# stella-cv/stella_vslam

Measured on AMD Instinct MI355X. Metric: frames/s ORB-extract+match @640x480,2k kpts, higher is better.
Workload: dtype u8

## Files before the change

include/svgpu.h:

```cpp
#ifndef SVGPU_H
#define SVGPU_H

#include <stddef.h>
#include <stdint.h>

#ifdef __cplusplus
extern "C" {
#endif

#define SVGPU_ABI_VERSION 1

typedef enum svgpu_status {
    SVGPU_OK = 0,
    SVGPU_ERR_INVALID = 1,
    SVGPU_ERR_HIP = 2,
    SVGPU_ERR_CAPACITY = 3,
    SVGPU_ERR_NOT_CONFIGURED = 4,
    SVGPU_ERR_NO_DEVICE = 5,
    SVGPU_ERR_NUMERIC = 6,
    SVGPU_STOPPED = 7
} svgpu_status;

typedef struct svgpu_ctx svgpu_ctx;

typedef struct svgpu_keypoint {
    float x, y, size, angle, response;
    int32_t octave, class_id;
} svgpu_keypoint;

int svgpu_abi_version(void);
int svgpu_device_count(void);
int svgpu_create(int device, svgpu_ctx** out);
int svgpu_create_with_priority(int device, int priority, svgpu_ctx** out);
void svgpu_destroy(svgpu_ctx* ctx);
const char* svgpu_last_error(const svgpu_ctx* ctx);
const char* svgpu_status_string(int status);
int svgpu_synchronize(svgpu_ctx* ctx);
void* svgpu_stream(svgpu_ctx* ctx);

const char* svgpu_profile_kernels(void);
int svgpu_profile_select(svgpu_ctx* ctx, const char* kernel_name);
int svgpu_profile_read(svgpu_ctx* ctx, double* total_ms, long long* launches);
int svgpu_profile_read_class(svgpu_ctx* ctx, const char* kernel_name, double* total_ms, long long* launches);
int svgpu_profile_mfma_ops(svgpu_ctx* ctx, unsigned long long* int8_ops);


int svgpu_orb_scale_tables(float scale_factor, int num_levels, float* scale_factors, float* inv_scale_factors,
                           float* level_sigma_sq, float* inv_level_sigma_sq);

int svgpu_orb_configure(svgpu_ctx* ctx, int width, int height, int max_batch, float scale_factor, int num_levels,
                        int ini_fast_thr, int min_fast_thr, unsigned min_area);

int svgpu_orb_stream_wait_stage(svgpu_ctx* ctx, int stage, void* stream);

int svgpu_orb_max_keypoints(const svgpu_ctx* ctx);
int svgpu_orb_level_size(const svgpu_ctx* ctx, int level, int* width, int* height);

int svgpu_orb_extract(svgpu_ctx* ctx, const uint8_t* img, int stride, const uint8_t* mask, int mask_stride,
                      svgpu_keypoint* kps, uint8_t* desc, int cap, int* n_out, int* level_counts);

int svgpu_orb_extract_batch_device(svgpu_ctx* ctx, const uint8_t* imgs_dev, int batch, size_t frame_stride,
                                   int row_stride, const uint8_t* mask_dev, size_t mask_frame_stride,
                                   int mask_row_stride, svgpu_keypoint* kps_dev, uint8_t* desc_dev, int cap,
                                   int32_t* counts_dev, void* stream);

int svgpu_orb_extract_batch_device_angles(svgpu_ctx* ctx, const uint8_t* imgs_dev, int batch, size_t frame_stride,
                                          int row_stride, const uint8_t* mask_dev, size_t mask_frame_stride,
                                          int mask_row_stride, svgpu_keypoint* kps_dev, uint8_t* desc_dev, int cap,
                                          int32_t* counts_dev, float* angles_dev, void* stream);

int svgpu_orb_pyramid_download(svgpu_ctx* ctx, int frame, int level, uint8_t* dst, int dst_stride);
int svgpu_orb_blurred_download(svgpu_ctx* ctx, int frame, int level, uint8_t* dst, int dst_stride);


int svgpu_hamming_distance(svgpu_ctx* ctx, const uint8_t* a, const uint8_t* b, int n, uint32_t* dist);

int svgpu_hamming_matrix(svgpu_ctx* ctx, const uint8_t* desc1, int n1, const uint8_t* desc2, int n2, uint16_t* out);

int svgpu_match_bruteforce(svgpu_ctx* ctx, const uint8_t* desc1, const float* angle1, int n1, const uint8_t* desc2,
                           const float* angle2, const uint8_t* valid2, int n2, float lowe_ratio,
                           int check_orientation, int32_t* matched_2_in_1, int* num_matches);

int svgpu_match_bruteforce_batch_device(svgpu_ctx* ctx, int pairs, const uint8_t* desc1_dev,
                                        const svgpu_keypoint* kps1_dev, const int32_t* n1_dev, int cap1,
                                        const uint8_t* desc2_dev, const svgpu_keypoint* kps2_dev,
                                        const int32_t* n2_dev, int cap2, int n_stride, const uint8_t* valid2_dev,
                                        float lowe_ratio, int check_orientation, int32_t* matched_dev,
                                        int32_t* num_dev, void* stream);

int svgpu_match_consecutive_batch_device(svgpu_ctx* ctx, int frames, const uint8_t* desc_dev, const svgpu_keypoint* kps_dev,
                                         const int32_t* n_dev, int cap, int n_stride, const uint8_t* valid_dev, float lowe_ratio,
                                         int check_orientation, int32_t* matched_dev, int32_t* num_dev, void* stream);

int svgpu_match_consecutive_batch_device_angles(svgpu_ctx* ctx, int frames, const uint8_t* desc_dev, const svgpu_keypoint* kps_dev,
                                                const float* angles_dev, const int32_t* n_dev, int cap, int n_stride, const uint8_t* valid_dev,
                                                float lowe_ratio, int check_orientation, int32_t* matched_dev, int32_t* num_dev, void* stream);

typedef enum svgpu_match_mode {
    SVGPU_MATCH_BEST_ONLY = 0,
    SVGPU_MATCH_RATIO_SAME_OCTAVE = 1,
    SVGPU_MATCH_RATIO = 2,
    SVGPU_MATCH_TRIANGULATION = 3,
    SVGPU_MATCH_AREA = 4
} svgpu_match_mode;

int svgpu_match_candidates(svgpu_ctx* ctx, const uint8_t* qdesc, int nq, const uint8_t* tdesc, const int32_t* t_octave,
                           int nt, const int32_t* cand_off, const int32_t* cand_idx, const uint8_t* cand_skip,
                           const uint8_t* q_valid, const uint8_t* occupied, const float* q_angle, const float* t_angle, int check_orientation,
                           const float* q_xright, const float* t_xright, const float* q_xr_tol, unsigned thr,
                           float lowe_ratio, int mode, int32_t* match_q, int* num_matches);

int svgpu_match_in_cells(svgpu_ctx* ctx, const uint8_t* qdesc, int nq, const float* q_xy, const float* q_margin,
                         const int32_t* q_min_level, const int32_t* q_max_level, const uint8_t* q_valid, const float* q_angle,
                         const float* q_xright, const float* q_xr_tol, const uint8_t* tdesc, const float* t_xy,
                         const int32_t* t_octave, int nt, const uint8_t* occupied, const float* t_angle, const float* t_xright,
                         float min_x, float max_x, float min_y, float max_y, int grid_cols, int grid_rows,
                         int check_orientation, unsigned thr, float lowe_ratio, int mode, int32_t* match_q, int* num_matches);

typedef enum svgpu_camera_model {
    SVGPU_CAM_PERSPECTIVE = 0,
    SVGPU_CAM_FISHEYE = 1,
    SVGPU_CAM_EQUIRECTANGULAR = 2,
    SVGPU_CAM_RADIAL_DIVISION = 3
} svgpu_camera_model;

typedef struct svgpu_camera {
    int32_t model;
    int32_t pad_;
    double cols, rows;
    double fx, fy, cx, cy;
    double dist[5];
    double focal_x_baseline;
    float min_x, max_x, min_y, max_y;
} svgpu_camera;

int svgpu_camera_image_bounds(svgpu_ctx* ctx, svgpu_camera* cam);

int svgpu_frame_observation(svgpu_ctx* ctx, const svgpu_camera* cam, const svgpu_keypoint* kps, int n, int grid_cols,
                            int grid_rows, svgpu_keypoint* undist_kps, double* bearings, int32_t* cell_off, int32_t* cell_items);

int svgpu_keypoints_to_bearings(svgpu_ctx* ctx, const svgpu_camera* cam, const svgpu_keypoint* undist_kps, int n, double* bearings);

int svgpu_reproject_landmarks(svgpu_ctx* ctx, const svgpu_camera* cam, const double* rot_cw, const double* trans_cw,
                              const double* trans_wc, int n, const double* pos_w, const double* mean_normal,
                              const float* min_valid_dist, const float* max_valid_dist, const uint8_t* skip, float ray_cos_thr,
                              int num_levels, float log_scale_factor, uint8_t* visible, double* reproj, float* x_right,
                              int32_t* pred_scale_level);

int svgpu_match_frame_and_landmarks(svgpu_ctx* ctx, const svgpu_camera* cam, const double* rot_cw, const double* trans_cw,
                                    const double* trans_wc, int n, const double* pos_w, const double* mean_normal,
                                    const float* min_valid_dist, const float* max_valid_dist, const uint8_t* skip,
                                    const uint8_t* lm_desc, float ray_cos_thr, int num_levels, const float* scale_factors,
                                    float log_scale_factor, float margin, const uint8_t* tdesc, const float* t_xy,
                                    const int32_t* t_octave, int nt, const uint8_t* occupied, const float* t_xright,
                                    int grid_cols, int grid_rows, unsigned thr, float lowe_ratio, int32_t* match_lm,
                                    int* num_matches, uint8_t* visible, double* reproj, float* x_right,
                                    int32_t* pred_scale_level);

typedef struct svgpu_frame svgpu_frame;
int svgpu_frame_create(svgpu_ctx* ctx, svgpu_frame** out);
void svgpu_frame_destroy(svgpu_frame* frame);
int svgpu_frame_size(const svgpu_frame* frame);
int svgpu_frame_adopt_extraction(svgpu_ctx* ctx, svgpu_frame* frame, const svgpu_camera* cam, int grid_cols, int grid_rows,
                                 svgpu_keypoint* undist_kps, double* bearings);
int svgpu_frame_upload(svgpu_ctx* ctx, svgpu_frame* frame, const svgpu_camera* cam, const svgpu_keypoint* undist_kps, const uint8_t* desc,
                       const float* x_right, int n, int grid_cols, int grid_rows);
int svgpu_frame_set_stereo(svgpu_ctx* ctx, svgpu_frame* frame, const float* x_right);
int svgpu_frame_bind(svgpu_ctx* ctx, const svgpu_frame* frame);
int svgpu_match_set_query_blocks(svgpu_ctx* ctx, const uint8_t* q_blocks);

typedef struct svgpu_map svgpu_map;
enum {
    SVGPU_LM_PRESENT = 1,
    SVGPU_LM_HAS_OBSERVATION = 2,
    SVGPU_LM_HAS_DESCRIPTOR = 4
};
typedef struct svgpu_landmark_record {
    double pos_w[3];
    double mean_normal[3];
    float min_valid_dist, max_valid_dist;
    uint8_t descriptor[32];
    uint32_t flags;
    uint32_t reserved;
} svgpu_landmark_record;
int svgpu_map_create(svgpu_ctx* ctx, svgpu_map** out);
void svgpu_map_destroy(svgpu_map* map);
int svgpu_map_capacity(const svgpu_map* map);
int svgpu_map_upsert(svgpu_ctx* ctx, svgpu_map* map, int n, const uint32_t* ids, const svgpu_landmark_record* records);
int svgpu_map_erase(svgpu_ctx* ctx, svgpu_map* map, int n, const uint32_t* ids);
int svgpu_map_download(svgpu_ctx* ctx, const svgpu_map* map, int n, const uint32_t* ids, svgpu_landmark_record* records);

typedef struct svgpu_tracker svgpu_tracker;
typedef struct svgpu_track_config {
    int num_levels;
    float scale_factors[16];
    float inv_level_sigma_sq[16];
    float log_scale_factor;
    int grid_cols, grid_rows;
    int is_monocular;
    float true_baseline;
    int po_num_trials_robust, po_num_trials, po_num_each_iter, po_reset_stop_flag_each_round;
} svgpu_track_config;
typedef struct svgpu_track_result {
    int n_keypoints;
    int num_matches;
    int num_valid;
    int lm_iterations;
    int num_observations;
    int num_candidates;
    int replay_sweeps;
    int reserved;
    double pose_cw[12];
} svgpu_track_result;
int svgpu_tracker_create(svgpu_ctx* ctx, svgpu_map* map, const svgpu_camera* cam, const svgpu_track_config* cfg, svgpu_tracker** out);
void svgpu_tracker_destroy(svgpu_tracker* tracker);
int svgpu_track_motion(svgpu_tracker* tracker, svgpu_frame* cur, const uint8_t* img, int stride, const svgpu_frame* last,
                       const int32_t* last_lm_ids, const double* pose_guess_cw, const double* pose_last_cw, float margin,
                       int check_orientation, svgpu_keypoint* kps, uint8_t* desc, svgpu_keypoint* undist_kps, double* bearings, int cap,
                       int32_t* match_last, uint8_t* outlier, svgpu_track_result* result);
int svgpu_tracker_observation(const svgpu_tracker* tracker, const svgpu_keypoint** kps, const uint8_t** desc, const svgpu_keypoint** undist_kps,
                              const double** bearings);
int svgpu_track_motion_stereo(svgpu_tracker* tracker, svgpu_ctx* ctx_right, svgpu_frame* cur, const uint8_t* img_left, int stride_left,
                              const uint8_t* img_right, int stride_right, const svgpu_frame* last, const int32_t* last_lm_ids,
                              const double* pose_guess_cw, const double* pose_last_cw, float margin, int check_orientation, int cap,
                              int32_t* match_last, uint8_t* outlier, svgpu_track_result* result);
int svgpu_tracker_observation_stereo(const svgpu_tracker* tracker, const float** stereo_x_right, const float** depths);
int svgpu_track_motion_rgbd(svgpu_tracker* tracker, svgpu_frame* cur, const uint8_t* img, int stride, const float* depth, int depth_stride,
                            const svgpu_frame* last, const int32_t* last_lm_ids, const double* pose_guess_cw, const double* pose_last_cw,
                            float margin, int check_orientation, int cap, int32_t* match_last, uint8_t* outlier, svgpu_track_result* result);
int svgpu_track_local_map(svgpu_tracker* tracker, const svgpu_frame* cur, const int32_t* cur_lm_ids, int n_local, const int32_t* local_ids,
                          const double* pose_cw, float margin, float lowe_ratio, float ray_cos_thr, int32_t* match_local, uint8_t* visible,
                          uint8_t* outlier, svgpu_track_result* result);
int svgpu_track_local_map_observability(svgpu_tracker* tracker, int n_local, double* reproj, float* x_right, int32_t* pred_scale_level);
int svgpu_tracker_counters(const svgpu_tracker* tracker, long long* launches, long long* host_syncs);
const unsigned long long* svgpu_tracker_debug_stamps(const svgpu_tracker* tracker);

typedef struct svgpu_ingest svgpu_ingest;
typedef enum svgpu_color_order { SVGPU_COLOR_GRAY = 0, SVGPU_COLOR_RGB = 1, SVGPU_COLOR_BGR = 2 } svgpu_color_order;
typedef enum svgpu_depth_type { SVGPU_DEPTH_NONE = 0, SVGPU_DEPTH_U16 = 1, SVGPU_DEPTH_F32 = 2 } svgpu_depth_type;
int svgpu_ingest_create(svgpu_ctx* ctx, int width, int height, int channels, int color_order, const float* map_x, const float* map_y,
                        int map_stride, svgpu_ingest** out);
void svgpu_ingest_destroy(svgpu_ingest* ingest);
int svgpu_ingest_gray(svgpu_ctx* ctx, const svgpu_ingest* ingest, const uint8_t* src, int src_stride, uint8_t* dst, int dst_stride);
int svgpu_ingest_gray_batch_device(svgpu_ctx* ctx, const svgpu_ingest* ingest, const uint8_t* src_dev, int batch, size_t src_frame_stride,
                                   int src_row_stride, uint8_t* dst_dev, size_t dst_frame_stride, int dst_row_stride, void* stream);
int svgpu_ingest_depth(svgpu_ctx* ctx, const void* src, int src_type, int src_stride, int width, int height, double depthmap_factor, float* dst,
                       int dst_stride);
int svgpu_ingest_depth_device(svgpu_ctx* ctx, const void* src_dev, int src_type, int src_stride, int width, int height, double depthmap_factor,
                              float* dst_dev, int dst_stride, void* stream);
int svgpu_tracker_set_ingest(svgpu_tracker* tracker, const svgpu_ingest* ingest_left, const svgpu_ingest* ingest_right, int depth_type,
                             double depthmap_factor);


int svgpu_reproject_to_bearing(const svgpu_camera* cam, const double* rot_cw, const double* trans_cw, const double* pos_w, double* bearing,
                               int* valid);

int svgpu_match_current_and_last_frames(svgpu_ctx* ctx, const svgpu_camera* cam, const double* rot_cw, const double* trans_cw, const double* rot_lw,
                                        const double* trans_lw, int is_monocular, float true_baseline, int n_last, const double* pos_w,
                                        const uint8_t* valid, const uint8_t* lm_desc, const int32_t* octave_last, const float* angle_last,
                                        const uint8_t* lm_has_observation, int num_levels, const float* scale_factors, float margin,
                                        const uint8_t* tdesc, const float* t_xy, const int32_t* t_octave, const float* t_angle, int nt,
                                        const uint8_t* occupied, const float* t_xright, int grid_cols, int grid_rows, int check_orientation,
                                        int32_t* match_last, int* num_matches);

int svgpu_match_frame_and_keyframe_projection(svgpu_ctx* ctx, const svgpu_camera* cam, const double* rot_cw, const double* trans_cw, int n_kf,
                                              const double* pos_w, const uint8_t* valid, const float* min_valid_dist, const float* max_valid_dist,
                                              const uint8_t* lm_desc, const float* angle_kf, int num_levels, const float* scale_factors,
                                              float log_scale_factor, float margin, unsigned hamm_dist_thr, const uint8_t* tdesc, const float* t_xy,
                                              const int32_t* t_octave, const float* t_angle, int nt, const uint8_t* occupied, int grid_cols,
                                              int grid_rows, int check_orientation, int32_t* match_kf, int* num_matches);

int svgpu_match_by_sim3_transform(svgpu_ctx* ctx, const svgpu_camera* cam, const double* sim3_cw, int n, const double* pos_w, const uint8_t* valid,
                                  const float* min_valid_dist, const float* max_valid_dist, const double* mean_normal, const uint8_t* lm_desc,
                                  int num_levels, const float* scale_factors, float log_scale_factor, float margin, const uint8_t* tdesc,
                                  const float* t_xy, const int32_t* t_octave, int nt, const uint8_t* occupied, int grid_cols, int grid_rows,
                                  int32_t* match_lm, int* num_matches);

int svgpu_match_keyframes_mutually(svgpu_ctx* ctx, const svgpu_camera* cam1, const svgpu_camera* cam2, const double* rot_1w, const double* trans_1w,
                                   const double* rot_2w, const double* trans_2w, float s_12, const double* rot_12, const double* trans_12,
                                   int n1, const double* pos_w1, const uint8_t* valid1, const float* min_valid1, const float* max_valid1,
                                   const uint8_t* lm_desc1, const uint8_t* desc1, const float* xy1, const int32_t* octave1,
                                   int n2, const double* pos_w2, const uint8_t* valid2, const float* min_valid2, const float* max_valid2,
                                   const uint8_t* lm_desc2, const uint8_t* desc2, const float* xy2, const int32_t* octave2,
                                   int num_levels, const float* scale_factors, float log_scale_factor, float margin, int grid_cols, int grid_rows,
                                   int32_t* matched_2_in_1, int32_t* matched_1_in_2, int32_t* mutual_2_in_1, int* num_matches);

int svgpu_fuse_detect_duplication(svgpu_ctx* ctx, const svgpu_camera* cam, const double* rot_cw, const double* trans_cw, int n, const double* pos_w,
                                  const uint8_t* valid, const float* min_valid_dist, const float* max_valid_dist, const double* mean_normal,
                                  const uint8_t* lm_desc, int num_levels, const float* scale_factors, const float* inv_level_sigma_sq,
                                  float log_scale_factor, float margin, int do_reprojection_matching, const uint8_t* tdesc, const float* t_xy,
                                  const int32_t* t_octave, const float* t_xright, int nt, int grid_cols, int grid_rows, int32_t* best_idx,
                                  int* num_fused);

int svgpu_match_for_triangulation(svgpu_ctx* ctx, const uint8_t* desc1, const float* angle1, const int32_t* octave1, const double* bearings1,
                                  const uint8_t* has_lm1, const float* xright1, int n1, const uint8_t* desc2, const float* angle2,
                                  const double* bearings2, const uint8_t* has_lm2, const float* xright2, int n2, const int32_t* node1,
                                  const int32_t* node2, const double* E_12, const double* epipole_in_2, int valid_epipole, const float* scale_factors,
                                  int num_levels, float residual_rad_thr, float lowe_ratio, int check_orientation, int32_t* matched_2_in_1,
                                  int* num_matches);

#define SVGPU_TRI_ACCEPTED 0
#define SVGPU_TRI_NO_MODE 1
#define SVGPU_TRI_DEPTH 2
#define SVGPU_TRI_REPROJECTION 3
#define SVGPU_TRI_SCALE 4
#define SVGPU_TRI_SKIPPED 255
int svgpu_triangulate_two_views(svgpu_ctx* ctx, const svgpu_camera* cam1, const double* pose_1w, double true_baseline_1, const float* xy1, const int32_t* octave1,
                                const double* bearings1, const float* xright1, const float* depth1, int n1, const svgpu_camera* cam2, const double* pose_2w,
                                double true_baseline_2, const float* xy2, const int32_t* octave2, const double* bearings2, const float* xright2,
                                const float* depth2, int n2, const float* scale_factors, const float* level_sigma_sq, int num_levels, float scale_factor_1,
                                float scale_factor_2, float rays_parallax_deg_thr, const int32_t* idx1, const int32_t* idx2, int num_matches, double* pos_w,
                                uint8_t* status, int* num_accepted);

typedef struct svgpu_triangulate_view {
    const svgpu_camera* cam;
    const double* pose_cw;
    double true_baseline;
    const float* xy;
    const int32_t* octave;
    const double* bearings;
    const float* xright;
    const float* depth;
    int32_t n;
    float scale_factor;
} svgpu_triangulate_view;
int svgpu_triangulate_two_views_batch(svgpu_ctx* ctx, const svgpu_triangulate_view* view1, const svgpu_triangulate_view* neighbours, int num_neighbours,
                                      const int32_t* match_off, const float* scale_factors, const float* level_sigma_sq, int num_levels,
                                      float rays_parallax_deg_thr, const int32_t* idx1, const int32_t* idx2, double* pos_w, uint8_t* status, int* num_accepted);

int svgpu_pnp_compute_pose(svgpu_ctx* ctx, int num_sets, const int32_t* set_off, const double* bearings, const double* pos_w,
                           int gauss_newton_num_iter, double* pose_cw, double* reproj_error);

int svgpu_pnp_ransac_batch(svgpu_ctx* ctx, int num_problems, const int32_t* match_off, const double* bearings, const double* pos_w,
                           const int32_t* octaves, const float* scale_factors, int num_levels, int min_num_inliers, int num_iter,
                           const uint32_t* samples, int recompute, int gauss_newton_num_iter, uint8_t* valid, double* pose_cw,
                           uint8_t* is_inlier, int32_t* best_iter, double* hyp_pose, int32_t* hyp_num_inliers, double* hyp_cost);

int svgpu_pnp_ransac(svgpu_ctx* ctx, const double* bearings, const double* pos_w, const int32_t* octaves, int num_matches,
                     const float* scale_factors, int num_levels, int min_num_inliers, int num_iter, const uint32_t* samples, int recompute,
                     int gauss_newton_num_iter, uint8_t* valid, double* pose_cw, uint8_t* is_inlier, int32_t* best_iter, double* hyp_pose,
                     int32_t* hyp_num_inliers, double* hyp_cost);

int svgpu_bow_match(svgpu_ctx* ctx, const uint8_t* desc1, const float* angle1, const uint8_t* valid1, const int32_t* node1, int n1,
                    const uint8_t* desc2, const float* angle2, const uint8_t* valid2, const int32_t* node2, int n2, const uint8_t* occupied2,
                    float lowe_ratio, int check_orientation, int32_t* match_1to2, int* num_matches);

int svgpu_landmarks_compute_descriptor(svgpu_ctx* ctx, int n, const int32_t* obs_off, const uint8_t* obs_desc, int32_t* best_obs,
                                       uint8_t* descriptor);

int svgpu_landmarks_update_geometry(svgpu_ctx* ctx, int n, const int32_t* obs_off, const double* obs_trans_wc, const double* pos_w,
                                    const double* ref_trans_wc, const float* ref_scale_factor, float inv_scale_factor_last,
                                    double* mean_normal, float* max_valid_dist, float* min_valid_dist);

typedef struct svgpu_vocabulary svgpu_vocabulary;
int svgpu_bow_vocabulary_upload(svgpu_ctx* ctx, int n_nodes, const int32_t* child_off, const int32_t* children, const uint8_t* node_desc,
                                const float* node_weight, const int32_t* word_id, svgpu_vocabulary** out);
void svgpu_bow_vocabulary_free(svgpu_vocabulary* vocab);
int svgpu_bow_transform(svgpu_ctx* ctx, const svgpu_vocabulary* vocab, const uint8_t* desc, int n, int node_level, int32_t* word_id,
                        float* weight, int32_t* node_id);
int svgpu_fbow_transform(svgpu_ctx* ctx, const svgpu_vocabulary* vocab, const uint8_t* desc, int n, int store_level, int k,
                         int32_t* word_id, float* weight, uint32_t* node_code);

#define SVGPU_BOW_SCORE_FBOW_L2 0
#define SVGPU_BOW_SCORE_DBOW2_L1 1
typedef struct svgpu_bowdb svgpu_bowdb;
int svgpu_bowdb_create(svgpu_ctx* ctx, int score_form, svgpu_bowdb** db);
void svgpu_bowdb_destroy(svgpu_bowdb* db);
int svgpu_bowdb_clear(svgpu_ctx* ctx, svgpu_bowdb* db);
int svgpu_bowdb_add(svgpu_ctx* ctx, svgpu_bowdb* db, int n_words, const uint32_t* words, const double* weights, int32_t* slot);
int svgpu_bowdb_erase(svgpu_ctx* ctx, svgpu_bowdb* db, int32_t slot);
int svgpu_bowdb_size(svgpu_bowdb* db, int* live_keyframes, long long* live_entries);
int svgpu_bowdb_diagnostics(svgpu_bowdb* db, long long* num_slots, long long* pool_capacity, long long* pool_used, long long* num_growths,
                            long long* num_compactions);
int svgpu_bowdb_query_stage_capacity(void);
int svgpu_bowdb_acquire(svgpu_ctx* ctx, svgpu_bowdb* db, int n_words, const uint32_t* words, const double* weights, float min_score, float ratio,
                        int n_reject, const int32_t* reject_slots, int cap, int32_t* out_slots, uint32_t* out_common, float* out_score, int32_t* n_out,
                        uint32_t* max_common);
int svgpu_bowdb_acquire_batch(svgpu_ctx* ctx, svgpu_bowdb* db, int num_queries, const int32_t* q_off, const uint32_t* words, const double* weights,
                              const float* min_score, float ratio, int n_reject, const int32_t* reject_slots, int cap, int32_t* out_slots,
                              uint32_t* out_common, float* out_score, int32_t* n_out, uint32_t* max_common);
int svgpu_bowdb_score(svgpu_ctx* ctx, svgpu_bowdb* db, int n_words, const uint32_t* words, const double* weights, int n, const int32_t* slots,
                      float* out_score);

int svgpu_stereo_match(svgpu_ctx* ctx_left, svgpu_ctx* ctx_right, const svgpu_keypoint* kps_left, const uint8_t* desc_left,
                       int n_left, const svgpu_keypoint* kps_right, const uint8_t* desc_right, int n_right,
                       float focal_x_baseline, float true_baseline, float* stereo_x_right, float* depths);

int svgpu_stereo_match_batch_device(svgpu_ctx* ctx_left, svgpu_ctx* ctx_right, int pairs, const svgpu_keypoint* kps_left_dev, const uint8_t* desc_left_dev,
                                    const int32_t* n_left_dev, const svgpu_keypoint* kps_right_dev, const uint8_t* desc_right_dev,
                                    const int32_t* n_right_dev, int cap, int n_stride, float focal_x_baseline, float true_baseline,
                                    float* stereo_x_right_dev, float* depths_dev, void* stream);

typedef struct svgpu_ba_problem {
    int32_t num_poses;
    int32_t num_points;
    int32_t num_obs;
    const double* pose_cw;
    const uint8_t* pose_fixed;
    const double* points;
    const uint8_t* point_fixed;
    const int32_t* obs_pose;
    const int32_t* obs_point;
    const float* obs_uvr;
    const float* obs_inv_sigma_sq;
    const float* obs_huber_delta;
    const double* intrinsics;
    int32_t num_first_iter;
    int32_t num_second_iter;
    double gain_threshold;
} svgpu_ba_problem;

typedef struct svgpu_ba_stats {
    double chi2_initial, chi2_final;
    int32_t iters_stage1, iters_stage2, stage2_entered, num_gated;
    int32_t lm_trials, cholesky_failures;
    double lambda_final;
    int32_t stopped_by_terminate_action;
    int32_t pcg_iterations;
} svgpu_ba_stats;

typedef enum svgpu_ba_solver {
    SVGPU_BA_SOLVER_AUTO = 0,
    SVGPU_BA_SOLVER_CHOLESKY = 1,
    SVGPU_BA_SOLVER_PCG = 2,
    SVGPU_BA_SOLVER_DENSE = 3,
    SVGPU_BA_SOLVER_PCG_MULTI = 4,
    SVGPU_BA_SOLVER_CHOLESKY_MFMA = 7,
    SVGPU_BA_SOLVER_ENVELOPE = 6
} svgpu_ba_solver;
int svgpu_ba_set_solver(svgpu_ctx* ctx, int solver, double pcg_tolerance, int pcg_max_iterations);

int svgpu_ba_last_envelope_plan(svgpu_ctx* ctx, int* info);

int svgpu_selftest_segmented_solve(int nP, int NB, const int* blk_ab, const double* Sblk, const double* g, int cuts, int world,
                                   double* x, int* info);

int svgpu_selftest_segmented_solve_rank(int nP, int NB, const int* blk_ab, const double* Sblk, const double* g, int cuts, int rank, int world,
                                        int (*allreduce)(void* user, double* buf, size_t count, void* stream), void* allreduce_user, double* x,
                                        int* info);

int svgpu_selftest_scan_sort(svgpu_ctx* ctx, int n, const int32_t* values, int32_t* scan_out, const uint32_t* keys, int bits, int32_t* sorted_idx);

int svgpu_local_ba(svgpu_ctx* ctx, const svgpu_ba_problem* problem, volatile uint8_t* stop, double* pose_out,
                   double* points_out, uint8_t* outlier_out, svgpu_ba_stats* stats);

int svgpu_pose_optimize(svgpu_ctx* ctx, const double* pose_cw, int n, const double* pos_w, const float* uvr,
                        const float* inv_sigma_sq, const float* huber_delta, const double* intrinsics ,
                        int num_trials_robust, int num_trials, int num_each_iter, int reset_stop_flag_each_round,
                        double* pose_out, uint8_t* outlier_flags, int* num_valid, int* lm_iterations);

int svgpu_pose_optimize_device(svgpu_ctx* ctx, const double* pose_cw, int n, const double* pos_w_dev, const float* uvr_dev,
                               const float* inv_sigma_sq_dev, const float* huber_delta_dev, const double* intrinsics, int num_trials_robust,
                               int num_trials, int num_each_iter, int reset_stop_flag_each_round, double* pose_out,
                               uint8_t* outlier_flags, int* num_valid, int* lm_iterations);

int svgpu_global_ba(svgpu_ctx* ctx, const svgpu_ba_problem* problem, volatile uint8_t* stop, double* pose_out,
                    double* points_out, svgpu_ba_stats* stats);

typedef int (*svgpu_allreduce_fn)(void* user, double* dev_buf, size_t count, void* stream);
int svgpu_local_ba_sharded(svgpu_ctx* ctx, const svgpu_ba_problem* shard, int rank, int world,
                           svgpu_allreduce_fn allreduce, void* allreduce_user, volatile uint8_t* stop, double* pose_out,
                           double* points_out, uint8_t* outlier_out, svgpu_ba_stats* stats);
int svgpu_global_ba_sharded(svgpu_ctx* ctx, const svgpu_ba_problem* shard, int rank, int world,
                            svgpu_allreduce_fn allreduce, void* allreduce_user, volatile uint8_t* stop, double* pose_out,
                            double* points_out, svgpu_ba_stats* stats);

int svgpu_ba_partition_keyframe_segments(const svgpu_ba_problem* problem, int world, int32_t* landmark_rank, int32_t* info);
int svgpu_ba_last_exchange(svgpu_ctx* ctx, int64_t* info);

int svgpu_comm_unique_id(uint8_t* id128);
int svgpu_comm_init(svgpu_ctx* ctx, int rank, int world, const uint8_t* id128);
void svgpu_comm_destroy(svgpu_ctx* ctx);
int svgpu_comm_allreduce_f64(svgpu_ctx* ctx, double* dev_buf, size_t count, void* stream);

#ifdef __cplusplus
}
#endif
#endif
```

stella_vslam_amd/csrc/orb_kernels.hip:

```cpp
#include "svgpu_internal.h"
#include "sv_trig.h"
#include <cstdlib>
#include <utility>

#pragma clang fp contract(off)

namespace {

__device__ __constant__ float c_pattern_f[1024] = {
#include "orb_pattern_i8.inc"
};

__device__ __forceinline__ int find_level(const OrbLevel* __restrict__ L, int num_levels, int idx, int OrbLevel::*first,
                                          int* local) {
    int lv = 0;
    for (int l = 0; l < num_levels; ++l) {
        const int f = L[l].*first;
        if (idx >= f) lv = l;
    }
    *local = idx - L[lv].*first;
    return lv;
}

__device__ __forceinline__ int reflect101(int p, int len) {
    if (len == 1) return 0;
    while (p < 0 || p >= len) p = p < 0 ? -p : 2 * (len - 1) - p;
    return p;
}

typedef unsigned short u16x2 __attribute__((ext_vector_type(2)));
__device__ __forceinline__ u16x2 as_u16x2(uint32_t v) { return __builtin_bit_cast(u16x2, v); }

__device__ __forceinline__ void xcd_frame_map(int per_frame, int batch, int& item, int& frame) {
    const int lin = blockIdx.x + blockIdx.y * gridDim.x;
    const int full = (batch / 8) * 8, lim = full * per_frame;
    if (lin < lim) {
        const int xcd = lin & 7, idx = lin >> 3;
        frame = (idx / per_frame) * 8 + xcd;
        item = idx % per_frame;
    }
    else {
        const int r = lin - lim;
        frame = full + r / per_frame;
        item = r % per_frame;
    }
}

__device__ __forceinline__ void sv_glds16(unsigned long long base, uint32_t voff, uint32_t lds_dst) {
    uint32_t keep;
    asm volatile("s_mov_b32 %0, m0\n\ts_mov_b32 m0, %3\n\ts_nop 2\n\tglobal_load_lds_dwordx4 %1, %2\n\ts_mov_b32 m0, %0"
                 : "=&s"(keep)
                 : "v"(voff), "s"(base), "s"(lds_dst)
                 : "memory");
}

__global__ __launch_bounds__(256) void k_resize(const uint8_t* __restrict__ src, size_t src_frame_stride, int src_pitch,
                                                int sw, uint8_t* __restrict__ dst, size_t dst_frame_stride, int dst_pitch,
                                                int dw, int dh, const short* __restrict__ xofs,
                                                const short2* __restrict__ xa, const short2* __restrict__ yofs,
                                                const short2* __restrict__ yb) {
    const int dy = blockIdx.y * 4 + threadIdx.y;
    const int dx0 = (blockIdx.x * 64 + threadIdx.x) * 4;
    if (dy >= dh || dx0 >= dw) return;
    const uint8_t* S = src + (size_t)blockIdx.z * src_frame_stride;
    const short2 yo = yofs[dy];
    const short2 bb = yb[dy];
    const uint8_t* S0 = S + (size_t)yo.x * src_pitch;
    const uint8_t* S1 = S + (size_t)yo.y * src_pitch;
    uint32_t packed = 0;
#pragma unroll
    for (int i = 0; i < 4; ++i) {
        const int dx = dx0 + i;
        if (dx < dw) {
            const int sx = xofs[dx];
            const short2 a = xa[dx];
            const int sx1 = min(sx + 1, sw - 1);
            const int r0 = S0[sx] * a.x + S0[sx1] * a.y;
            const int r1 = S1[sx] * a.x + S1[sx1] * a.y;
            const int v = ((((int)bb.x * (r0 >> 4)) >> 16) + (((int)bb.y * (r1 >> 4)) >> 16) + 2) >> 2;
            packed |= (uint32_t)(v & 255) << (8 * i);
        }
    }
    uint8_t* D = dst + (size_t)blockIdx.z * dst_frame_stride + (size_t)dy * dst_pitch + dx0;
    *reinterpret_cast<uint32_t*>(D) = packed;
}

#define PYR_THREADS 1024
#define PYR_MAXW 4096
__global__ __launch_bounds__(PYR_THREADS) void k_pyramid(const OrbLevel* __restrict__ L, int num_levels, const int2* __restrict__ band_rows,
                                                         const uint8_t* __restrict__ img0, size_t img0_frame_stride, int img0_pitch,
                                                         uint8_t* __restrict__ pyr, size_t pyr_frame_bytes,
                                                         const short* __restrict__ xofs, const short2* __restrict__ xa,
                                                         const short2* __restrict__ yofs, const short2* __restrict__ yb) {
    __shared__ short s_xo[PYR_MAXW];
    __shared__ short2 s_xa[PYR_MAXW];
    const int band = blockIdx.x, b = blockIdx.y, tid = threadIdx.x;
    uint8_t* P = pyr + (size_t)b * pyr_frame_bytes;
    for (int l = 1; l < num_levels; ++l) {
        const OrbLevel lev = L[l], prev = L[l - 1];
        const uint8_t* S = l == 1 ? img0 + (size_t)b * img0_frame_stride : P + prev.pyr_off;
        const int sp = l == 1 ? img0_pitch : prev.pitch;
        uint8_t* Dst = P + lev.pyr_off;
        const int2 rr = band_rows[band * num_levels + l];
        const int groups = (lev.w + 3) >> 2, ntask = (rr.y - rr.x) * groups;
        const bool in_lds = lev.w <= PYR_MAXW;
        if (in_lds)
            for (int x = tid; x < lev.w; x += PYR_THREADS) {
                s_xo[x] = xofs[lev.xtab_off + x];
                s_xa[x] = xa[lev.xtab_off + x];
            }
        __syncthreads();
        for (int t = tid; t < ntask; t += PYR_THREADS) {
            const int row = t / groups, g = t - row * groups;
            const int dy = rr.x + row, dx0 = g * 4;
            const short2 yo = yofs[lev.ytab_off + dy], bb = yb[lev.ytab_off + dy];
            const uint8_t* S0 = S + (size_t)yo.x * sp;
            const uint8_t* S1 = S + (size_t)yo.y * sp;
            int sx[4], sx1[4];
            short2 a[4];
#pragma unroll
            for (int i = 0; i < 4; ++i) {
                const int dx = min(dx0 + i, lev.w - 1);
                sx[i] = in_lds ? s_xo[dx] : xofs[lev.xtab_off + dx];
                a[i] = in_lds ? s_xa[dx] : xa[lev.xtab_off + dx];
                sx1[i] = min(sx[i] + 1, prev.w - 1);
            }
            int p00[4], p01[4], p10[4], p11[4];
#pragma unroll
            for (int i = 0; i < 4; ++i) {
                p00[i] = S0[sx[i]];
                p01[i] = S0[sx1[i]];
                p10[i] = S1[sx[i]];
                p11[i] = S1[sx1[i]];
            }
            uint32_t packed = 0;
#pragma unroll
            for (int i = 0; i < 4; ++i) {
                const int r0 = p00[i] * a[i].x + p01[i] * a[i].y;
                const int r1 = p10[i] * a[i].x + p11[i] * a[i].y;
                const int v = ((((int)bb.x * (r0 >> 4)) >> 16) + (((int)bb.y * (r1 >> 4)) >> 16) + 2) >> 2;
                packed |= (uint32_t)(v & 255) << (8 * i);
            }
            *reinterpret_cast<uint32_t*>(Dst + (size_t)dy * lev.pitch + dx0) = packed;
        }
        __syncthreads();
    }
}

__device__ __forceinline__ uint32_t mul_hi_u24(uint32_t a, uint32_t b) {
    uint32_t d;
    asm("v_mul_hi_u32_u24 %0, %1, %2" : "=v"(d) : "v"(a), "v"(b));
    return d;
}

__global__ __launch_bounds__(PYR_THREADS) void k_pyramid_lds(const OrbLevel* __restrict__ L, int num_levels, const int2* __restrict__ band_rows,
                                                             int bands, const uint8_t* __restrict__ img0, size_t img0_frame_stride,
                                                             int img0_pitch, uint8_t* __restrict__ pyr, size_t pyr_frame_bytes,
                                                             const uint32_t* __restrict__ xg, const short4* __restrict__ yrow) {
    extern __shared__ __attribute__((aligned(16))) uint8_t s_mem[];
    __shared__ int s_img[SV_MAX_LEVELS], s_yt[SV_MAX_LEVELS + 1];
    const int band = blockIdx.x, b = blockIdx.y, tid = threadIdx.x;
    const int2* BR = band_rows + (size_t)band * num_levels;
    if (tid == 0) {
        int size_a = 0, size_b = 0;
        for (int l = 0; l < num_levels; ++l) {
            const int bytes = (BR[l].y - BR[l].x) * ((L[l].w + 3) & ~3);
            if (l & 1) size_a = max(size_a, bytes);
            else size_b = max(size_b, bytes);
        }
        size_a = (size_a + 15) & ~15;
        size_b = (size_b + 15) & ~15;
        for (int l = 0; l < num_levels; ++l) s_img[l] = (l & 1) ? 0 : size_a;
        int off = size_a + size_b;
        s_yt[0] = off;
        for (int l = 1; l < num_levels; ++l) {
            s_yt[l] = off;
            off += (BR[l].y - BR[l].x) * 8;
        }
        s_yt[num_levels] = off;
    }
    __syncthreads();
    const uint8_t* I0 = img0 + (size_t)b * img0_frame_stride;
    {
        const int w0 = L[0].w, p0 = (w0 + 3) & ~3, lo0 = BR[0].x, n0 = BR[0].y - lo0;
        uint8_t* D0 = s_mem + s_img[0];
        if (((((size_t)I0) | (size_t)img0_pitch) & 15) == 0 && (p0 & 15) == 0) {
            const int cpr = p0 >> 4, total = n0 * cpr;
            const float inv = 1.0f / (float)cpr;
            for (int i = tid; i < total; i += PYR_THREADS) {
                const int r = (int)(((float)i + 0.5f) * inv), c = i - __mul24(r, cpr);
                reinterpret_cast<uint4*>(D0)[i] = *reinterpret_cast<const uint4*>(I0 + (__umul24(lo0 + r, img0_pitch) + 16 * c));
            }
        }
        else if (((((size_t)I0) | (size_t)img0_pitch) & 3) == 0) {
            const int wpr = p0 >> 2, total = n0 * wpr;
            const float inv = 1.0f / (float)wpr;
            for (int i = tid; i < total; i += PYR_THREADS) {
                const int r = (int)(((float)i + 0.5f) * inv), c = i - __mul24(r, wpr);
                reinterpret_cast<uint32_t*>(D0)[i] = *reinterpret_cast<const uint32_t*>(I0 + (__umul24(lo0 + r, img0_pitch) + 4 * c));
            }
        }
        else {
            const int total = n0 * p0;
            for (int i = tid; i < total; i += PYR_THREADS) {
                const int r = i / p0, c = i - r * p0;
                D0[i] = c < w0 ? I0[(size_t)(lo0 + r) * img0_pitch + c] : (uint8_t)0;
            }
        }
        const int rows = (s_yt[num_levels] - s_yt[0]) >> 3;
        for (int i = tid; i < rows; i += PYR_THREADS) {
            int l = 1;
            while (l + 1 < num_levels && s_yt[0] + 8 * i >= s_yt[l + 1]) ++l;
            const int r = i - ((s_yt[l] - s_yt[0]) >> 3);
            reinterpret_cast<short4*>(s_mem + s_yt[0])[i] = yrow[L[l].ytab_off + BR[l].x + r];
        }
    }
    __syncthreads();
    uint8_t* P = pyr + (size_t)b * pyr_frame_bytes;
    for (int l = 1; l < num_levels; ++l) {
        const OrbLevel lev = L[l];
        const int spw = ((L[l - 1].w + 3) & ~3) >> 2, dpw = ((lev.w + 3) & ~3) >> 2;
        const int src_lo = BR[l - 1].x, lo = BR[l].x, hi = BR[l].y;
        const int own_lo = (int)((long long)band * lev.h / bands), own_hi = (int)((long long)(band + 1) * lev.h / bands);
        const uint32_t* S = reinterpret_cast<const uint32_t*>(s_mem + s_img[l - 1]);
        uint32_t* Dl = reinterpret_cast<uint32_t*>(s_mem + s_img[l]);
        const short4* yt = reinterpret_cast<const short4*>(s_mem + s_yt[l]);
        uint8_t* Dg = P + lev.pyr_off;
        const int groups = (lev.w + 3) >> 2, nrows = hi - lo;
        const int chunks = max(min(PYR_THREADS / groups, nrows), 1), rc = (nrows + chunks - 1) / chunks;
        const int c = (int)(((float)tid + 0.5f) * (1.0f / (float)groups)), g = tid - __mul24(c, groups);
        const int r0 = __mul24(c, rc), r1 = min(r0 + rc, nrows);
        if (r0 < r1) {
            const uint4 e = reinterpret_cast<const uint4*>(xg)[2 * (lev.xg_off + g)];
            const uint2 e2 = reinterpret_cast<const uint2*>(xg)[4 * (lev.xg_off + g) + 2];
            const int i0 = e.x & 0xffff, i2 = e.x >> 16;
            const uint32_t coef[4] = {e.z, e.w, e2.x, e2.y};
            uint32_t sel[4];
#pragma unroll
            for (int i = 0; i < 4; ++i) sel[i] = 0x0c010c00u + ((e.y >> (8 * i)) & 255u) * 0x00010001u;
            const uint32_t* S0 = S + (i0 - __mul24(src_lo, spw));
            const int d2 = i2 - i0;
            auto hrow = [&](int sy, uint32_t (&h)[4]) {
                const uint32_t* R = S0 + __mul24(sy, spw);
                const uint32_t a0 = R[0], a1 = R[1], c0 = R[d2], c1 = R[d2 + 1];
                h[0] = __builtin_amdgcn_udot2(as_u16x2(__builtin_amdgcn_perm(a1, a0, sel[0])), as_u16x2(coef[0]), 0u, false) & ~15u;
                h[1] = __builtin_amdgcn_udot2(as_u16x2(__builtin_amdgcn_perm(a1, a0, sel[1])), as_u16x2(coef[1]), 0u, false) & ~15u;
                h[2] = __builtin_amdgcn_udot2(as_u16x2(__builtin_amdgcn_perm(c1, c0, sel[2])), as_u16x2(coef[2]), 0u, false) & ~15u;
                h[3] = __builtin_amdgcn_udot2(as_u16x2(__builtin_amdgcn_perm(c1, c0, sel[3])), as_u16x2(coef[3]), 0u, false) & ~15u;
            };
            uint32_t* dl = Dl + (__mul24(r0, dpw) + g);
            uint32_t goff = __umul24(lo + r0, lev.pitch) + 4 * g;
            const uint32_t own_n = (uint32_t)(own_hi - own_lo);
            uint32_t dyo = (uint32_t)(lo + r0 - own_lo);
            int prev = -1;
            auto step = [&](int row, uint32_t (&top)[4], uint32_t (&bot)[4]) {
                const short4 ye = yt[row];
                if (ye.x != prev) hrow(ye.x, top);
                hrow(ye.y, bot);
                prev = ye.y;
                const uint32_t b0 = (uint32_t)ye.z << 12, b1 = (uint32_t)ye.w << 12;
                uint32_t v[4];
#pragma unroll
                for (int i = 0; i < 4; ++i) v[i] = (mul_hi_u24(b0, top[i]) + mul_hi_u24(b1, bot[i]) + 2u) >> 2;
                const uint32_t packed = (v[0] & 255u) | ((v[1] & 255u) << 8) | ((v[2] & 255u) << 16) | (v[3] << 24);
                *dl = packed;
                if (dyo < own_n) *reinterpret_cast<uint32_t*>(Dg + goff) = packed;
                dl += dpw;
                goff += (uint32_t)lev.pitch;
                ++dyo;
            };
            uint32_t hX[4], hY[4] = {0, 0, 0, 0};
            int row = r0;
            for (; row + 1 < r1; row += 2) {
                step(row, hY, hX);
                step(row + 1, hX, hY);
            }
            if (row < r1) step(row, hY, hX);
        }
        __syncthreads();
    }
}

#define BLUR_EDGE_ROWS 8
struct BlurRow {
    uint32_t w0, w1, w2;
};
enum { BLUR_INTERIOR = 0, BLUR_EDGE = 1, BLUR_GATHER = 2, BLUR_LDS = 3 };
struct BlurEdge {
    bool left, hi_p1;
    uint32_t sel1, sel2;
};
__device__ __forceinline__ uint32_t blur_selector(int xbase, int lo_base, int w) {
    uint32_t s = 0;
#pragma unroll
    for (int k = 0; k < 4; ++k) {
        const int x = xbase + k, sx = x < w ? x : 2 * (w - 1) - x;
        s |= (uint32_t)min(max(sx - lo_base, 0), 7) << (8 * k);
    }
    return s;
}
__device__ __forceinline__ BlurEdge blur_edge_ctx(int x0, int w) {
    BlurEdge e;
    e.left = x0 == 0;
    e.hi_p1 = x0 + 4 < w;
    e.sel1 = blur_selector(x0, x0 - 4, w);
    e.sel2 = blur_selector(x0 + 4, e.hi_p1 ? x0 : x0 - 4, w);
    return e;
}
template <int MODE>
__device__ __forceinline__ BlurRow blur_load(const uint8_t* __restrict__ row, int x0, int w, const BlurEdge& e) {
    BlurRow r;
    if (MODE == BLUR_INTERIOR) {
        const uint32_t* p = reinterpret_cast<const uint32_t*>(row + x0 - 4);
        r.w0 = p[0];
        r.w1 = p[1];
        r.w2 = p[2];
    }
    else if (MODE == BLUR_EDGE) {
        if (e.left) {
            const uint32_t* p = reinterpret_cast<const uint32_t*>(row);
            r.w1 = p[0];
            r.w2 = p[1];
            r.w0 = __builtin_amdgcn_perm(r.w2, r.w1, 0x01020304u);
        }
        else {
            const uint32_t* p = reinterpret_cast<const uint32_t*>(row + x0 - 4);
            const uint32_t pm1 = p[0], p0 = p[1], p1 = e.hi_p1 ? p[2] : 0u;
            r.w0 = pm1;
            r.w1 = __builtin_amdgcn_perm(p0, pm1, e.sel1);
            r.w2 = e.hi_p1 ? __builtin_amdgcn_perm(p1, p0, e.sel2) : __builtin_amdgcn_perm(p0, pm1, e.sel2);
        }
    }
    else {
        uint32_t b[12];
#pragma unroll
        for (int k = 0; k < 12; ++k) b[k] = row[reflect101(x0 - 4 + k, w)];
        r.w0 = b[0] | (b[1] << 8) | (b[2] << 16) | (b[3] << 24);
        r.w1 = b[4] | (b[5] << 8) | (b[6] << 16) | (b[7] << 24);
        r.w2 = b[8] | (b[9] << 8) | (b[10] << 16) | (b[11] << 24);
    }
    return r;
}
__device__ __forceinline__ void blur_hpair(const BlurRow& a, const BlurRow& b, u16x2 (&hp)[4]) {
    u16x2 q[10];
#define SV_PK(WA, WB, K) as_u16x2(__builtin_amdgcn_perm(WB, WA, 0x0c000c00u | ((4u + K) << 16) | K))
    q[0] = SV_PK(a.w0, b.w0, 1u);
    q[1] = SV_PK(a.w0, b.w0, 2u);
    q[2] = SV_PK(a.w0, b.w0, 3u);
    q[3] = SV_PK(a.w1, b.w1, 0u);
    q[4] = SV_PK(a.w1, b.w1, 1u);
    q[5] = SV_PK(a.w1, b.w1, 2u);
    q[6] = SV_PK(a.w1, b.w1, 3u);
    q[7] = SV_PK(a.w2, b.w2, 0u);
    q[8] = SV_PK(a.w2, b.w2, 1u);
    q[9] = SV_PK(a.w2, b.w2, 2u);
#undef SV_PK
    const u16x2 t18 = {18, 18}, t34 = {34, 34}, t48 = {48, 48}, t56 = {56, 56};
#pragma unroll
    for (int j = 0; j < 4; ++j) hp[j] = t18 * (q[j] + q[j + 6]) + t34 * (q[j + 1] + q[j + 5]) + t48 * (q[j + 2] + q[j + 4]) + t56 * q[j + 3];
}
__device__ __forceinline__ uint32_t blur_dot(u16x2 h, uint32_t taps, uint32_t acc) { return __builtin_amdgcn_udot2(h, as_u16x2(taps), acc, false); }
__device__ __forceinline__ uint32_t blur_pack(const uint32_t (&acc)[4]) {
    const uint32_t lo = __builtin_amdgcn_perm(acc[1], acc[0], 0x0c0c0602u), hi = __builtin_amdgcn_perm(acc[3], acc[2], 0x06020c0cu);
    return lo | hi;
}

template <int MODE, class LoadPair>
__device__ __forceinline__ void blur_walk(LoadPair load_pair, uint8_t* __restrict__ Dp, int dpitch, int ys, int ye) {
    constexpr int AHEAD = MODE == BLUR_LDS ? 0 : 2;
    u16x2 A[4], B[4], C[4], D[4], E[4];
    BlurRow n0 = {}, n1 = {};
    {
        BlurRow r[8];
#pragma unroll
        for (int k = 0; k < 4; ++k) load_pair(ys - 4 + 2 * k, r[2 * k], r[2 * k + 1]);
        if (AHEAD) load_pair(ys + 4, n0, n1);
        if (MODE == BLUR_INTERIOR) {
#pragma unroll
            for (int k = 0; k < 8; ++k) asm volatile("" : "+v"(r[k].w0), "+v"(r[k].w1), "+v"(r[k].w2));
            asm volatile("" : "+v"(n0.w0), "+v"(n0.w1), "+v"(n0.w2), "+v"(n1.w0), "+v"(n1.w1), "+v"(n1.w2));
        }
        blur_hpair(r[0], r[1], A);
        blur_hpair(r[2], r[3], B);
        blur_hpair(r[4], r[5], C);
        blur_hpair(r[6], r[7], D);
    }
    for (int y = ys; y < ye; y += 2) {
        const BlurRow c0 = n0, c1 = n1;
        load_pair(y + 4 + AHEAD, n0, n1);
        if (AHEAD) blur_hpair(c0, c1, E);
        else blur_hpair(n0, n1, E);
        uint32_t acc[4];
#pragma unroll
        for (int j = 0; j < 4; ++j)
            acc[j] = blur_dot(D[j], 34u | (18u << 16), blur_dot(C[j], 56u | (48u << 16), blur_dot(B[j], 34u | (48u << 16), blur_dot(A[j], 18u << 16, 32768u))));
        *reinterpret_cast<uint32_t*>(Dp + __umul24(y, dpitch)) = blur_pack(acc);
        if (y + 1 < ye) {
#pragma unroll
            for (int j = 0; j < 4; ++j)
                acc[j] = blur_dot(E[j], 18u, blur_dot(D[j], 48u | (34u << 16), blur_dot(C[j], 48u | (56u << 16), blur_dot(B[j], 18u | (34u << 16), 32768u))));
            *reinterpret_cast<uint32_t*>(Dp + __umul24(y + 1, dpitch)) = blur_pack(acc);
        }
#pragma unroll
        for (int j = 0; j < 4; ++j) {
            A[j] = B[j];
            B[j] = C[j];
            C[j] = D[j];
            D[j] = E[j];
        }
    }
}
template <int MODE>
__device__ __forceinline__ void blur_strip(const uint8_t* __restrict__ src, int spitch, int w, int h, uint8_t* __restrict__ dst,
                                           int dpitch, int x0, int ys, int ye) {
    auto row_ptr = [&](int y) { return src + __umul24(reflect101(y, h), spitch); };
    BlurEdge edge = {};
    if (MODE == BLUR_EDGE) edge = blur_edge_ctx(x0, w);
    blur_walk<MODE>([&](int y, BlurRow& a, BlurRow& b) {
        a = blur_load<MODE>(row_ptr(y), x0, w, edge);
        b = blur_load<MODE>(row_ptr(y + 1), x0, w, edge);
    }, dst + x0, dpitch, ys, ye);
}

__device__ __forceinline__ void blur_locate(const OrbLevel* __restrict__ L, int num_levels, const uint8_t* __restrict__ img0,
                                            size_t img0_frame_stride, int img0_pitch, const uint8_t* __restrict__ pyr,
                                            size_t pyr_frame_bytes, uint8_t* __restrict__ blur, size_t blur_frame_bytes, OrbLevel& lev,
                                            int& tile, const uint8_t*& src, int& spitch, uint8_t*& dst,
                                            int OrbLevel::*first = &OrbLevel::btile_first) {
    int b, item;
    xcd_frame_map(gridDim.x, gridDim.y, item, b);
    const int lv = find_level(L, num_levels, item, first, &tile);
    lev = L[lv];
    if (lv == 0) {
        src = img0 + (size_t)b * img0_frame_stride;
        spitch = img0_pitch;
    }
    else {
        src = pyr + (size_t)b * pyr_frame_bytes + lev.pyr_off;
        spitch = lev.pitch;
    }
    dst = blur + (size_t)b * blur_frame_bytes + lev.blur_off;
}
__device__ __forceinline__ bool blur_streamable(const uint8_t* src, int spitch, int w) {
    return ((((size_t)src) | (size_t)spitch) & 3) == 0 && w >= 16;
}
template <int ROWS>
__global__ __launch_bounds__(256) void k_blur(const OrbLevel* __restrict__ L, int num_levels, const uint8_t* __restrict__ img0,
                                              size_t img0_frame_stride, int img0_pitch, const uint8_t* __restrict__ pyr,
                                              size_t pyr_frame_bytes, uint8_t* __restrict__ blur, size_t blur_frame_bytes) {
    OrbLevel lev;
    int tile, spitch;
    const uint8_t* src;
    uint8_t* dst;
    blur_locate(L, num_levels, img0, img0_frame_stride, img0_pitch, pyr, pyr_frame_bytes, blur, blur_frame_bytes, lev, tile, src, spitch, dst);
    if (!blur_streamable(src, spitch, lev.w)) return;
    const int main_tiles = lev.btiles_x * lev.btiles_y;
    if (tile < main_tiles) {
        const int tx = tile % lev.btiles_x, ty = tile / lev.btiles_x;
        const int rem_groups = tx == lev.btiles_x - 1 ? (min(lev.w - 6, (tx + 1) * BLUR_TW) - tx * BLUR_TW + 3) / 4 : 64;
        int g = 64;
        while (g > 1 && (g >> 1) >= rem_groups) g >>= 1;
        if (g <= 32 && rem_groups > 0) {
            const int spw = 64 / g, lane = threadIdx.x & 63;
            if (ty * spw >= lev.btiles_y) return;
            const int strip = (ty * 4 + (int)(threadIdx.x >> 6)) * spw + lane / g;
            const int x0 = tx * BLUR_TW + (lane % g) * 4, ys = strip * ROWS;
            if (x0 >= lev.w || ys >= lev.h) return;
            if (x0 >= 4 && x0 + 6 < lev.w) blur_strip<BLUR_INTERIOR>(src, spitch, lev.w, lev.h, dst, lev.pitch, x0, ys, min(ys + ROWS, lev.h));
            return;
        }
        const int x0 = tx * BLUR_TW + (threadIdx.x & 63) * 4;
        const int ys = __builtin_amdgcn_readfirstlane(ty * (4 * ROWS) + (int)(threadIdx.x >> 6) * ROWS);
        if (x0 >= lev.w || ys >= lev.h) return;
        if (x0 >= 4 && x0 + 6 < lev.w) blur_strip<BLUR_INTERIOR>(src, spitch, lev.w, lev.h, dst, lev.pitch, x0, ys, min(ys + ROWS, lev.h));
    }
    else {
        const int which = threadIdx.x & 3, strip = (tile - main_tiles) * 64 + (threadIdx.x >> 2);
        const int ys = strip * BLUR_EDGE_ROWS;
        const int last = ((lev.w - 1) >> 2) << 2;
        int x0;
        if (which == 0) x0 = 0;
        else if (which == 1) x0 = last;
        else if (which == 2) x0 = last - 4;
        else return;
        if (ys >= lev.h || x0 < 0 || (which != 0 && (x0 == 0 || x0 + 6 < lev.w))) return;
        blur_strip<BLUR_EDGE>(src, spitch, lev.w, lev.h, dst, lev.pitch, x0, ys, min(ys + BLUR_EDGE_ROWS, lev.h));
    }
}
#define BLUR_LP (16 + BLUR_SEG + 16)
#define BLUR_LDS_ROWS (BLUR_ROWS + 8)
static_assert(BLUR_SEG % 16 == 0 && BLUR_BAND_THREADS % 64 == 0 && BLUR_SEG / 4 <= BLUR_BAND_THREADS && BLUR_ROWS % 2 == 0, "blur band geometry");
static_assert(BLUR_LDS_ROWS * BLUR_LP <= 64 * 1024, "blur band exceeds the static LDS limit");
template <>
__global__ __launch_bounds__(BLUR_BAND_THREADS) void k_blur<BLUR_ROWS>(const OrbLevel* __restrict__ L, int num_levels, const uint8_t* __restrict__ img0,
                                                                       size_t img0_frame_stride, int img0_pitch, const uint8_t* __restrict__ pyr,
                                                                       size_t pyr_frame_bytes, uint8_t* __restrict__ blur, size_t blur_frame_bytes) {
    __shared__ __attribute__((aligned(16))) uint8_t s_rows[BLUR_LDS_ROWS * BLUR_LP];
    OrbLevel lev;
    int item, spitch;
    const uint8_t* src;
    uint8_t* dst;
    blur_locate(L, num_levels, img0, img0_frame_stride, img0_pitch, pyr, pyr_frame_bytes, blur, blur_frame_bytes, lev, item, src, spitch, dst,
                &OrbLevel::bband_first);
    if (!blur_streamable(src, spitch, lev.w)) return;
    const int tid = threadIdx.x, w = lev.w, h = lev.h;
    const int seg = item % lev.bband_segs, xs = seg * BLUR_SEG, sw = min(BLUR_SEG, w - xs);
    const int y0 = (item / lev.bband_segs) * BLUR_ROWS, rows = min(BLUR_ROWS, h - y0);
    const int groups = (sw + 3) >> 2, xend = xs + 4 * groups + 4;
    {
        constexpr int CPR = BLUR_LP / 16;
        const int total = (rows + 6) * CPR;
        const unsigned long long base = (unsigned long long)(uintptr_t)src;
        const uint32_t lds0 = __builtin_amdgcn_readfirstlane((uint32_t)(uintptr_t)(const __attribute__((address_space(3))) uint8_t*)s_rows) + BLUR_LP;
        for (int q0 = __builtin_amdgcn_readfirstlane(tid & ~63); q0 < total; q0 += BLUR_BAND_THREADS) {
            const int q = q0 + (tid & 63), k = q / CPR, x = xs - 16 + 16 * (q - k * CPR);
            if (q < total && x >= 0 && x < min(w, xend)) {
                const uint32_t off = __umul24(reflect101(y0 - 3 + k, h), spitch) + (uint32_t)x;
                if (x + 16 <= w) sv_glds16(base, off, lds0 + 16u * (uint32_t)q0);
                else
#pragma clang loop vectorize(disable)
                    for (int d = 0; x + 4 * d < w; ++d)
                        *reinterpret_cast<uint32_t*>(s_rows + BLUR_LP + 16 * q + 4 * d) = *reinterpret_cast<const uint32_t*>(src + off + 4 * d);
            }
        }
        asm volatile("s_waitcnt vmcnt(0)" ::: "memory");
    }
    __syncthreads();
    for (int i = tid; i < (rows + 6) * 8; i += BLUR_BAND_THREADS) {
        uint8_t* row = s_rows + ((i >> 3) + 1) * BLUR_LP + 16 - xs;
        const int j = i & 7;
        if (j == 0 && xs == 0) {
            const uint32_t* p = reinterpret_cast<const uint32_t*>(row);
            reinterpret_cast<uint32_t*>(row)[-1] = __builtin_amdgcn_perm(p[1], p[0], 0x01020304u);
        }
        const int x = w - 1 + j;
        if (j > 0 && x < xend) row[x] = row[2 * (w - 1) - x];
    }
    __syncthreads();
    const int chunks = max(min(BLUR_BAND_THREADS / groups, rows >> 1), 1), rc = ((rows + chunks - 1) / chunks + 1) & ~1;
    const int c = (int)(((float)tid + 0.5f) * (1.0f / (float)groups)), g = tid - __mul24(c, groups);
    const int r0 = __mul24(c, rc), r1 = min(r0 + rc, rows);
    if (r0 >= r1) return;
    const uint32_t* S = reinterpret_cast<const uint32_t*>(s_rows + 12 + 4 * g);
    blur_walk<BLUR_LDS>([&](int y, BlurRow& a, BlurRow& b) {
        const uint32_t* p = S + __mul24(y + 4, BLUR_LP / 4);
        a = BlurRow{p[0], p[1], p[2]};
        b = BlurRow{p[BLUR_LP / 4], p[BLUR_LP / 4 + 1], p[BLUR_LP / 4 + 2]};
    }, dst + __umul24(y0, lev.pitch) + xs + 4 * g, lev.pitch, r0, r1);
}
template <int ROWS>
__global__ __launch_bounds__(256) void k_blur_gather(const OrbLevel* __restrict__ L, int num_levels, const uint8_t* __restrict__ img0,
                                                     size_t img0_frame_stride, int img0_pitch, const uint8_t* __restrict__ pyr,
                                                     size_t pyr_frame_bytes, uint8_t* __restrict__ blur, size_t blur_frame_bytes) {
    OrbLevel lev;
    int tile, spitch;
    const uint8_t* src;
    uint8_t* dst;
    blur_locate(L, num_levels, img0, img0_frame_stride, img0_pitch, pyr, pyr_frame_bytes, blur, blur_frame_bytes, lev, tile, src, spitch, dst);
    if (blur_streamable(src, spitch, lev.w) || tile >= lev.btiles_x * lev.btiles_y) return;
    const int x0 = (tile % lev.btiles_x) * BLUR_TW + (threadIdx.x & 63) * 4;
    const int ys = (tile / lev.btiles_x) * (4 * ROWS) + (threadIdx.x >> 6) * ROWS;
    if (x0 >= lev.w || ys >= lev.h) return;
    blur_strip<BLUR_GATHER>(src, spitch, lev.w, lev.h, dst, lev.pitch, x0, ys, min(ys + ROWS, lev.h));
}

typedef short s16x2 __attribute__((ext_vector_type(2)));
__device__ __forceinline__ int arc_score16(int v, const int (&p)[16]) {
    s16x2 e[16];
#pragma unroll
    for (int k = 0; k < 16; ++k) e[k] = __builtin_bit_cast(s16x2, __mul24(p[k], -65535) + (int)0xFFFF0000);
    s16x2 m2[8], m4[8];
#pragma unroll
    for (int j = 0; j < 8; ++j) m2[j] = __builtin_elementwise_min(e[2 * j + 1], e[(2 * j + 2) & 15]);
#pragma unroll
    for (int j = 0; j < 8; ++j) m4[j] = __builtin_elementwise_min(m2[j], m2[(j + 1) & 7]);
    s16x2 best = s16x2{(short)-32768, (short)-32768};
#pragma unroll
    for (int j = 0; j < 8; ++j) {
        const s16x2 m8 = __builtin_elementwise_min(m4[j], m4[(j + 2) & 7]);
        best = __builtin_elementwise_max(best, __builtin_elementwise_min(m8, __builtin_elementwise_max(e[2 * j], e[(2 * j + 9) & 15])));
    }
    return max(max((int)best.x - v, v + 1 + (int)best.y), 0);
}

#define FAST_KT 12
#define FP 80
__global__ __launch_bounds__(256) void k_fast(const OrbLevel* __restrict__ L, int num_levels, const FastCell* __restrict__ cells, int num_cells, int cpw,
                                              const uint8_t* __restrict__ img0, size_t img0_frame_stride, int img0_pitch,
                                              const uint8_t* __restrict__ pyr, size_t pyr_frame_bytes,
                                              const unsigned short* __restrict__ gtab, unsigned long long* __restrict__ keys,
                                              int total_grid, int ini_thr, int min_thr, const uint8_t* __restrict__ mask,
                                              size_t mask_frame_stride, int mask_pitch, int mask_w, int mask_h) {
    __shared__ __attribute__((aligned(16))) uint8_t s_raw[SV_ROI_MAX * FP + 16];
    __shared__ __attribute__((aligned(16))) uint8_t s_a[SV_ROI_MAX * FP];
    __shared__ unsigned short s_q[SV_CELL * SV_CELL];
    __shared__ unsigned long long s_key[FAST_KT * FAST_KT];
    __shared__ unsigned short s_gx[SV_ROI_MAX], s_gy[SV_ROI_MAX];
    __shared__ int s_count;
    int b, grp;
    xcd_frame_map(gridDim.x, gridDim.y, grp, b);
    const int tid = threadIdx.x, lane = tid & 63;
    const int wv = __builtin_amdgcn_readfirstlane(tid >> 6);
    const uint8_t* M = mask ? mask + (size_t)b * mask_frame_stride : nullptr;
    const uint8_t* const I0 = img0 + (size_t)b * img0_frame_stride;
    const uint8_t* const PY = pyr + (size_t)b * pyr_frame_bytes;
    unsigned long long* const KF = keys + (size_t)b * total_grid;
    uint8_t* const s_img = s_raw + 3;
    unsigned short* const my_q = s_q + wv * (SV_CELL * SV_CELL / 4);
    const int qrow = lane >> 4, qk = lane & 15;
    const int x0 = 3 + 4 * qk;
    const int ly0 = 3 + 4 * (4 * qrow + wv);
    const int e0 = (ly0 << 7) | x0;
    const uint32_t* const qbase = reinterpret_cast<const uint32_t*>(s_raw + ly0 * FP + 4 * qk);

    auto load_ring = [&](const uint8_t* c, int (&p)[16]) {
        p[0] = c[3 * FP];
        p[1] = c[3 * FP + 1];
        p[2] = c[2 * FP + 2];
        p[3] = c[FP + 3];
        p[4] = c[3];
        p[5] = c[-FP + 3];
        p[6] = c[-2 * FP + 2];
        p[7] = c[-3 * FP + 1];
        p[8] = c[-3 * FP];
        p[9] = c[-3 * FP - 1];
        p[10] = c[-2 * FP - 2];
        p[11] = c[-FP - 3];
        p[12] = c[-3];
        p[13] = c[FP - 3];
        p[14] = c[2 * FP - 2];
        p[15] = c[3 * FP - 1];
    };

    const int c_first = grp * cpw, c_last = min(c_first + cpw, num_cells);
    for (int ci = c_first; ci < c_last; ++ci) {
    const FastCell cell = cells[ci];
    const OrbLevel lev = L[cell.lv];
    auto masked = [&](int y, int x) -> bool {
        int my = (int)((float)y * lev.scale), mx = (int)((float)x * lev.scale);
        my = min(my, mask_h - 1);
        mx = min(mx, mask_w - 1);
        return M[(size_t)my * mask_pitch + mx] == 0;
    };
    if (M) {
        const int y0 = cell.min_y, y1 = cell.min_y + cell.h, xa = cell.min_x, xb = cell.min_x + cell.w;
        if (masked(y0, xa) || masked(y1, xa) || masked(y0, xb) || masked(y1, xb)) continue;
    }
    const uint8_t* src;
    int spitch;
    if (cell.lv == 0) {
        src = I0;
        spitch = img0_pitch;
    }
    else {
        src = PY + lev.pyr_off;
        spitch = lev.pitch;
    }
    const int w = cell.w, h = cell.h;
    if (ci != c_first) __syncthreads();
    const uint8_t* rsrc = src + (size_t)cell.min_y * spitch + (cell.min_x - 3);
    {
        const unsigned long long rbase = (unsigned long long)(uintptr_t)rsrc;
        const uint32_t lds_raw = __builtin_amdgcn_readfirstlane((uint32_t)(uintptr_t)(const __attribute__((address_space(3))) uint8_t*)s_raw) + (uint32_t)wv * 1024u;
#pragma unroll
        for (int it = 0; it < 2; ++it) {
            const int q = tid + 256 * it, r = q / 5, c = q - 5 * r;
            if (it == 0 || wv < 2) {
                if (q < SV_ROI_MAX * (FP / 16) && r < h && 16 * c < w + 3) sv_glds16(rbase, (uint32_t)(__umul24(r, spitch) + 16 * c), lds_raw + 4096u * it);
            }
            if (q < SV_ROI_MAX * (FP / 16)) reinterpret_cast<uint4*>(s_a)[q] = make_uint4(0, 0, 0, 0);
        }
    }
    if (tid == 0) {
        s_count = 0;
    }
    if (tid < FAST_KT * FAST_KT) s_key[tid] = 0ull;
    if (tid < w) s_gx[tid] = gtab[lev.gtab_x_off + cell.min_x + tid - SV_PATCH_RADIUS];
    else if (tid >= 128 && tid - 128 < h) s_gy[tid - 128] = gtab[lev.gtab_y_off + cell.min_y + (tid - 128) - SV_PATCH_RADIUS];
    uint32_t band80 = 0;
#pragma unroll
    for (int j = 0; j < 4; ++j) band80 |= (x0 + j < w - 3) ? (0x80u << (8 * j)) : 0u;
    asm volatile("s_waitcnt vmcnt(0)" ::: "memory");
    __syncthreads();

    unsigned long long* K = KF + lev.grid_first;
    const int gx0 = s_gx[3], gy0 = s_gy[3];
    for (int pass = 0; pass < 2; ++pass) {
    const int t = pass == 0 ? ini_thr : min_thr, tq = t;
    int wq = 0;
#if defined(FAST_ABLATE) && FAST_ABLATE >= 2
    if (mask_h == -12345)
#endif
    {
        const uint32_t tqq = (uint32_t)(tq + 1) * 0x10001u;
        uint32_t m = 0;
#pragma unroll
        for (int g = 0; g < 4; ++g) {
            const uint32_t* const rc = qbase + g * (FP / 4);
            const uint32_t w0 = rc[0], w1 = rc[1], w2 = rc[2], w3 = rc[3];
            const uint32_t d1 = rc[3 * (FP / 4) + 1], d2 = rc[3 * (FP / 4) + 2], u1 = rc[-3 * (FP / 4) + 1], u2 = rc[-3 * (FP / 4) + 2];
            auto pk = [](uint32_t hi, uint32_t lo, uint32_t sel) { return __builtin_bit_cast(s16x2, __builtin_amdgcn_perm(hi, lo, sel)); };
            uint32_t e2[2];
#pragma unroll
            for (int half = 0; half < 2; ++half) {
                const s16x2 v = pk(w2, w1, half ? 0x0c050c04u : 0x0c030c02u);
                const s16x2 p0 = pk(d2, d1, half ? 0x0c050c04u : 0x0c030c02u);
                const s16x2 p8 = pk(u2, u1, half ? 0x0c050c04u : 0x0c030c02u);
                const s16x2 p12 = pk(w1, w0, half ? 0x0c060c05u : 0x0c040c03u);
                const s16x2 p4 = pk(w3, w2, half ? 0x0c040c03u : 0x0c020c01u);
                const s16x2 up = __builtin_elementwise_min(__builtin_elementwise_max(p0, p8), __builtin_elementwise_max(p4, p12));
                const s16x2 dn = __builtin_elementwise_max(__builtin_elementwise_min(p0, p8), __builtin_elementwise_min(p4, p12));
                const s16x2 mm = __builtin_elementwise_max(up - v, v - dn);
                e2[half] = __builtin_bit_cast(uint32_t, mm - __builtin_bit_cast(s16x2, tqq));
            }
            const uint32_t sgn = __builtin_amdgcn_perm(e2[1], e2[0], 0x07050301u);
            m = (m >> 1) | (~sgn & (ly0 + g < h - 3 ? band80 : 0u));
        }
        const int cnt = __popc(m);
        int incl = cnt;
        incl += __builtin_amdgcn_update_dpp(0, incl, 0x111, 0xF, 0xF, false);
        incl += __builtin_amdgcn_update_dpp(0, incl, 0x112, 0xF, 0xF, false);
        incl += __builtin_amdgcn_update_dpp(0, incl, 0x114, 0xF, 0xF, false);
        incl += __builtin_amdgcn_update_dpp(0, incl, 0x118, 0xF, 0xF, false);
        incl += __builtin_amdgcn_update_dpp(0, incl, 0x142, 0xA, 0xF, false);
        incl += __builtin_amdgcn_update_dpp(0, incl, 0x143, 0xC, 0xF, false);
        wq = __builtin_amdgcn_readlane(incl, 63);
        int pos = incl - cnt;
        while (m) {
            const int bit = __ffs((int)m) - 1;
            m &= m - 1;
            my_q[pos++] = (unsigned short)(e0 + (((bit & 7) - 4) << 7) + (bit >> 3));
        }
    }
#if defined(FAST_ABLATE) && FAST_ABLATE >= 1
    if (mask_h != -12345) wq = 0;
#endif
    __builtin_amdgcn_fence(__ATOMIC_RELEASE, "wavefront");
    __builtin_amdgcn_wave_barrier();
    __builtin_amdgcn_fence(__ATOMIC_ACQUIRE, "wavefront");
    for (int i = lane; i < wq; i += 64) {
        const int e = my_q[i], ly = e >> 7, qx = e & 127;
        const uint8_t* c = &s_img[ly * FP + qx];
        int p[16];
        load_ring(c, p);
        s_a[ly * FP + qx] = (uint8_t)arc_score16(c[0], p);
    }
    __syncthreads();

    {
        int found = 0;
        for (int i = lane; i < wq; i += 64) {
            const int e = my_q[i], ly = e >> 7, qx = e & 127;
            const uint8_t* a = &s_a[ly * FP + qx];
            const int A = a[0];
            if (A <= t) continue;
            const int s = A - 1;
            const int n0 = max(max((int)a[-FP - 1], (int)a[-FP]), (int)a[-FP + 1]);
            const int n1 = max(max((int)a[-1], (int)a[1]), (int)a[FP - 1]);
            const int n2 = max(max((int)a[FP], (int)a[FP + 1]), n0);
            const bool keep = A > 1 && max(n1, n2) < A;
            if (!keep) continue;
            ++found;
            const int x_level = cell.min_x + qx, y_level = cell.min_y + ly;
            if (M && masked(y_level, x_level)) continue;
            const int gx = s_gx[qx], gy = s_gy[ly];
            const uint32_t order = (uint32_t)cell.order_base | ((uint32_t)ly << 7) | (uint32_t)qx;
            const unsigned long long key = ((unsigned long long)(uint32_t)s << 32) | (0xFFFFFFFFu - order);
            const int kx = gx - gx0, ky = gy - gy0;
            if ((unsigned)kx < FAST_KT && (unsigned)ky < FAST_KT) atomicMax(&s_key[ky * FAST_KT + kx], key);
            else atomicMax(&K[gy * lev.grid_x + gx], key);
        }
        if (found) atomicAdd(&s_count, found);
        __syncthreads();
        if (s_count > 0) break;
        __syncthreads();
    }
    }
    if (tid < FAST_KT * FAST_KT) {
        const unsigned long long key = s_key[tid];
        if (key) atomicMax(&K[(gy0 + tid / FAST_KT) * lev.grid_x + gx0 + tid % FAST_KT], key);
    }
    }
}

__global__ __launch_bounds__(1024) void k_select(const OrbLevel* __restrict__ L, int num_levels, unsigned long long* __restrict__ keys,
                                                 int total_grid, int4* __restrict__ sel, int32_t* __restrict__ counts, int32_t* __restrict__ cellpos) {
    __shared__ int s_wave[16], s_lvcnt[SV_MAX_LEVELS];
    const int b = blockIdx.x, tid = threadIdx.x, lane = tid & 63, wave = tid >> 6;
    unsigned long long* K = keys + (size_t)b * total_grid;
    int4* S = sel + (size_t)b * total_grid;
    if (tid < SV_MAX_LEVELS) s_lvcnt[tid] = 0;
    int running = 0;
    for (int base = 0; base < total_grid; base += 1024) {
        const int idx = base + tid;
        unsigned long long key = 0;
        if (idx < total_grid) {
            key = K[idx];
            if (key) K[idx] = 0;
        }
        const unsigned long long bal = __ballot(key != 0);
        const int before = __popcll(bal & ((1ull << lane) - 1ull));
        __syncthreads();
        if (lane == 0) s_wave[wave] = __popcll(bal);
        __syncthreads();
        int woff = 0, total = 0;
#pragma unroll
        for (int k = 0; k < 16; ++k) {
            if (k < wave) woff += s_wave[k];
            total += s_wave[k];
        }
        if (cellpos && idx < total_grid) cellpos[(size_t)b * (total_grid + 1) + idx] = running + woff + before;
        if (key) {
            int lv = 0;
            while (lv + 1 < num_levels && idx >= L[lv + 1].grid_first) ++lv;
            const uint32_t order = 0xFFFFFFFFu - (uint32_t)(key & 0xFFFFFFFFu);
            const int lx = order & 127, ly = (order >> 7) & 127, cid = order >> 14;
            const int cells_x = L[lv].cells_x;
            const int ci = cid / cells_x, cj = cid - ci * cells_x;
            int4 r;
            r.x = SV_PATCH_RADIUS + cj * SV_CELL + lx;
            r.y = SV_PATCH_RADIUS + ci * SV_CELL + ly;
            r.z = lv;
            r.w = (int)(key >> 32);
            S[running + woff + before] = r;
            atomicAdd(&s_lvcnt[lv], 1);
        }
        running += total;
    }
    __syncthreads();
    if (tid < num_levels) counts[b * (1 + num_levels) + 1 + tid] = s_lvcnt[tid];
    if (tid == 0) {
        counts[b * (1 + num_levels)] = running;
        if (cellpos) cellpos[(size_t)b * (total_grid + 1) + total_grid] = running;
    }
}

__device__ __forceinline__ float dev_fast_atan2(float y, float x) {
    const float p1 = 0.9997878412794807f * (float)(180 / 3.1415926535897932384626433832795);
    const float p3 = -0.3258083974640975f * (float)(180 / 3.1415926535897932384626433832795);
    const float p5 = 0.1555786518463281f * (float)(180 / 3.1415926535897932384626433832795);
    const float p7 = -0.04432655554792128f * (float)(180 / 3.1415926535897932384626433832795);
    const float eps = (float)2.2204460492503131e-16;
    const float ax = fabsf(x), ay = fabsf(y);
    float a, c, c2;
    if (ax >= ay) {
        c = ay / (ax + eps);
        c2 = c * c;
        a = (((p7 * c2 + p5) * c2 + p3) * c2 + p1) * c;
    }
    else {
        c = ax / (ay + eps);
        c2 = c * c;
        a = 90.f - (((p7 * c2 + p5) * c2 + p3) * c2 + p1) * c;
    }
    if (x < 0) a = 180.f - a;
    if (y < 0) a = 360.f - a;
    return a;
}

__device__ __forceinline__ float dev_util_cos(float v) { return sv_util_cos(v); }
__device__ __forceinline__ float dev_util_sin(float v) { return sv_util_sin(v); }

__device__ __forceinline__ int wave_sum(int v) {
    v += __builtin_amdgcn_update_dpp(0, v, 0x111, 0xF, 0xF, false);
    v += __builtin_amdgcn_update_dpp(0, v, 0x112, 0xF, 0xF, false);
    v += __builtin_amdgcn_update_dpp(0, v, 0x114, 0xF, 0xF, false);
    v += __builtin_amdgcn_update_dpp(0, v, 0x118, 0xF, 0xF, false);
    v += __builtin_amdgcn_update_dpp(0, v, 0x142, 0xA, 0xF, false);
    v += __builtin_amdgcn_update_dpp(0, v, 0x143, 0xC, 0xF, false);
    return __builtin_amdgcn_readlane(v, 63);
}

#ifndef DESC_KPW
#define DESC_KPW 5
#endif
#define DESC_IP 32
#define DESC_BP 40
#define DESC_R 18
#define DESC_SLAB (DESC_KPW * 37 * DESC_BP + 16)
struct IcWeights {
    uint32_t w1[256], wu[256];
};
constexpr IcWeights make_ic_weights() {
    constexpr int umax[16] = {15, 15, 15, 15, 14, 14, 14, 13, 13, 12, 11, 10, 9, 8, 6, 3};
    IcWeights t{};
    for (int row = 0; row < 31; ++row)
        for (int j = 0; j < 8; ++j) {
            uint32_t w1 = 0, wu = 0;
            const int v = row - 15, av = v < 0 ? -v : v;
            for (int k = 0; k < 4; ++k) {
                const int col = 4 * j + k, u = col - 15, au = u < 0 ? -u : u;
                if (col < 31 && au <= umax[av]) {
                    w1 |= 1u << (8 * k);
                    wu |= (uint32_t)(u + 15) << (8 * k);
                }
            }
            t.w1[row * 8 + j] = w1;
            t.wu[row * 8 + j] = wu;
        }
    return t;
}
__device__ __constant__ IcWeights c_icw = make_ic_weights();

__global__ __launch_bounds__(256) void k_describe(const OrbLevel* __restrict__ L, int num_levels, const int4* __restrict__ sel,
                                                  int total_grid, const int32_t* __restrict__ counts,
                                                  const uint8_t* __restrict__ img0, size_t img0_frame_stride, int img0_pitch,
                                                  const uint8_t* __restrict__ pyr, size_t pyr_frame_bytes,
                                                  const uint8_t* __restrict__ blur, size_t blur_frame_bytes,
                                                  svgpu_keypoint* __restrict__ kps, uint8_t* __restrict__ desc, int cap, float* __restrict__ angles) {
    __shared__ __attribute__((aligned(16))) uint8_t s_slab[4][DESC_SLAB];
    int b, blk;
    xcd_frame_map(gridDim.x, gridDim.y, blk, b);
    const int lane = threadIdx.x & 63, wave = __builtin_amdgcn_readfirstlane(threadIdx.x >> 6);
    const int n = min(counts[b * (1 + num_levels)], cap);
    const int i0 = (blk * 4 + wave) * DESC_KPW;
    if (i0 >= n) return;
    uint8_t* const slab = s_slab[wave];
    float px0[4], py0[4], px1[4], py1[4];
#pragma unroll
    for (int r = 0; r < 4; ++r) {
        const float4 q = reinterpret_cast<const float4*>(c_pattern_f)[r * 64 + lane];
        px0[r] = q.x;
        py0[r] = q.y;
        px1[r] = q.z;
        py1[r] = q.w;
    }
    uint32_t w1[4], wu[4];
    int rowv[4];
#pragma unroll
    for (int m = 0; m < 4; ++m) {
        const int item = lane + 64 * m;
        w1[m] = c_icw.w1[item];
        wu[m] = c_icw.wu[item];
        rowv[m] = (item >> 3) - 15;
    }
    const int nk = min(DESC_KPW, n - i0);
    const int4* const S = sel + (size_t)b * total_grid + i0;
    const uint8_t* const I0 = img0 + (size_t)b * img0_frame_stride;
    const uint8_t* const PY = pyr + (size_t)b * pyr_frame_bytes;
    const uint8_t* const BL = blur + (size_t)b * blur_frame_bytes;
    const int part = lane & 3, prow = lane >> 2;
    const int br = lane / 5, bpart = lane - 5 * br;
    int4 sv[DESC_KPW];
#pragma unroll
    for (int kk = 0; kk < DESC_KPW; ++kk) sv[kk] = S[kk];
    const uint8_t* gi[DESC_KPW];
    const uint8_t* gbl[DESC_KPW];
    int pit_i[DESC_KPW], pit_b[DESC_KPW];
#pragma unroll
    for (int kk = 0; kk < DESC_KPW; ++kk) {
        const int lv = kk < nk ? sv[kk].z : 0;
        pit_b[kk] = L[lv].pitch;
        pit_i[kk] = lv == 0 ? img0_pitch : pit_b[kk];
        gi[kk] = (lv == 0 ? I0 : PY + L[lv].pyr_off) + (size_t)(sv[kk].y - 15) * pit_i[kk] + (sv[kk].x - 15);
        gbl[kk] = BL + L[lv].blur_off + (size_t)(sv[kk].y - DESC_R) * pit_b[kk] + (sv[kk].x - DESC_R);
    }
    uint2 vi[DESC_KPW][2];
#pragma unroll
    for (int kk = 0; kk < DESC_KPW; ++kk)
        if (kk < nk) {
#pragma unroll
            for (int h = 0; h < 2; ++h)
                if (16 * h + prow < 31) __builtin_memcpy(&vi[kk][h], gi[kk] + (__umul24(16 * h + prow, pit_i[kk]) + 8 * part), 8);
        }
#pragma unroll
    for (int kk = 0; kk < DESC_KPW; ++kk)
        if (kk < nk) {
#pragma unroll
            for (int h = 0; h < 2; ++h)
                if (16 * h + prow < 31) *reinterpret_cast<uint2*>(slab + kk * (31 * DESC_IP) + (16 * h + prow) * DESC_IP + 8 * part) = vi[kk][h];
        }
    __builtin_amdgcn_fence(__ATOMIC_RELEASE, "wavefront");
    __builtin_amdgcn_wave_barrier();
    __builtin_amdgcn_fence(__ATOMIC_ACQUIRE, "wavefront");
    uint2 vb[DESC_KPW][4];
#pragma unroll
    for (int kk = 0; kk < DESC_KPW; ++kk)
        if (kk < nk) {
#pragma unroll
            for (int h = 0; h < 4; ++h)
                if (br < 12 && 12 * h + br < 37) __builtin_memcpy(&vb[kk][h], gbl[kk] + (__umul24(12 * h + br, pit_b[kk]) + 8 * bpart), 8);
        }
    int my10 = 0, my01 = 0;
#pragma unroll
    for (int kk = 0; kk < DESC_KPW; ++kk)
        if (kk < nk) {
            int m10 = 0, m01 = 0;
#pragma unroll
            for (int m = 0; m < 4; ++m) {
                const int item = lane + 64 * m;
                const uint32_t px = item < 248 ? reinterpret_cast<const uint32_t*>(slab + kk * (31 * DESC_IP))[item] : 0u;
                const int s1 = (int)__builtin_amdgcn_udot4(px, w1[m], 0u, false), su = (int)__builtin_amdgcn_udot4(px, wu[m], 0u, false);
                m10 += su - __mul24(15, s1);
                m01 += __mul24(rowv[m], s1);
            }
            m10 = wave_sum(m10);
            m01 = wave_sum(m01);
            if (lane == kk) {
                my10 = m10;
                my01 = m01;
            }
        }
    const float angle = dev_fast_atan2((float)my01, (float)my10);
    const float rad = (float)((double)angle * 3.14159265358979323846 / 180.0);
    const float ca_l = dev_util_cos(rad), sa_l = dev_util_sin(rad);
    __builtin_amdgcn_fence(__ATOMIC_RELEASE, "wavefront");
    __builtin_amdgcn_wave_barrier();
#pragma unroll
    for (int kk = 0; kk < DESC_KPW; ++kk)
        if (kk < nk) {
#pragma unroll
            for (int h = 0; h < 4; ++h)
                if (br < 12 && 12 * h + br < 37) *reinterpret_cast<uint2*>(slab + kk * (37 * DESC_BP) + __mul24(12 * h + br, DESC_BP) + 8 * bpart) = vb[kk][h];
        }
    __builtin_amdgcn_fence(__ATOMIC_RELEASE, "wavefront");
    __builtin_amdgcn_wave_barrier();
    __builtin_amdgcn_fence(__ATOMIC_ACQUIRE, "wavefront");
#pragma unroll
    for (int kk = 0; kk < DESC_KPW; ++kk)
        if (kk < nk) {
            const float ca = __int_as_float(__builtin_amdgcn_readlane(__float_as_int(ca_l), kk));
            const float sa = __int_as_float(__builtin_amdgcn_readlane(__float_as_int(sa_l), kk));
            const uint8_t* B = slab + kk * (37 * DESC_BP) + DESC_R * DESC_BP + DESC_R;
            unsigned long long bits[4];
#pragma unroll
            for (int r = 0; r < 4; ++r) {
                const float x0 = px0[r], y0 = py0[r], x1 = px1[r], y1 = py1[r];
                constexpr float RN = 12582912.0f;
                constexpr int RK = 0x400000 * DESC_BP + 0x4B400000;
                typedef float f32x2 __attribute__((ext_vector_type(2)));
                const f32x2 sc = {sa, ca}, cs = {ca, -sa}, rn = {RN, RN};
                const f32x2 q0 = (f32x2{x0, x0} * sc + f32x2{y0, y0} * cs) + rn;
                const f32x2 q1 = (f32x2{x1, x1} * sc + f32x2{y1, y1} * cs) + rn;
                const int r0 = __float_as_int(q0.x), c0 = __float_as_int(q0.y);
                const int r1 = __float_as_int(q1.x), c1 = __float_as_int(q1.y);
                const int a = B[__mul24(r0, DESC_BP) + c0 - RK];
                const int bb = B[__mul24(r1, DESC_BP) + c1 - RK];
                bits[r] = __builtin_amdgcn_ballot_w64(a < bb);
            }
            uint8_t* D = desc + ((size_t)b * cap + i0 + kk) * 32;
            if (lane < 4) reinterpret_cast<unsigned long long*>(D)[lane] = lane == 0 ? bits[0] : lane == 1 ? bits[1] : lane == 2 ? bits[2] : bits[3];
        }
    if (lane < nk) {
        const int4 s = S[lane];
        const int lv = s.z;
        svgpu_keypoint k;
        k.x = (float)s.x;
        k.y = (float)s.y;
        if (lv != 0) {
            k.x = k.x * L[lv].scale;
            k.y = k.y * L[lv].scale;
        }
        k.size = L[lv].kp_size;
        k.angle = angle;
        k.response = (float)s.w;
        k.octave = lv;
        k.class_id = -1;
        kps[(size_t)b * cap + i0 + lane] = k;
        if (angles) angles[(size_t)b * cap + i0 + lane] = angle;
    }
}


#ifndef DB_THREADS
#define DB_THREADS 512
#endif
#define DB_WAVES (DB_THREADS / 64)
#define DB_MAX_KP 128
struct IcWeights3 {
    uint32_t w1[256], wu[256], wv[256];
};
constexpr IcWeights3 make_ic_weights3() {
    constexpr int umax[16] = {15, 15, 15, 15, 14, 14, 14, 13, 13, 12, 11, 10, 9, 8, 6, 3};
    IcWeights3 t{};
    for (int row = 0; row < 31; ++row)
        for (int j = 0; j < 8; ++j) {
            uint32_t w1 = 0, wu = 0, wv = 0;
            const int v = row - 15, av = v < 0 ? -v : v;
            for (int k = 0; k < 4; ++k) {
                const int col = 4 * j + k, u = col - 15, au = u < 0 ? -u : u;
                if (col < 31 && au <= umax[av]) {
                    w1 |= 1u << (8 * k);
                    wu |= (uint32_t)(u + 15) << (8 * k);
                    wv |= (uint32_t)row << (8 * k);
                }
            }
            t.w1[row * 8 + j] = w1;
            t.wu[row * 8 + j] = wu;
            t.wv[row * 8 + j] = wv;
        }
    return t;
}
__device__ __constant__ IcWeights3 c_icw3 = make_ic_weights3();

template <int LANE>
__device__ __forceinline__ void sv_writelane8(uint32_t& lo, uint32_t& hi, const unsigned long long (&m)[4]) {
    asm("s_nop 1\n\tv_writelane_b32 %0, %2, %10\n\tv_writelane_b32 %1, %3, %10\n\tv_writelane_b32 %0, %4, %11\n\tv_writelane_b32 %1, %5, %11\n\t"
        "v_writelane_b32 %0, %6, %12\n\tv_writelane_b32 %1, %7, %12\n\tv_writelane_b32 %0, %8, %13\n\tv_writelane_b32 %1, %9, %13"
        : "+v"(lo), "+v"(hi)
        : "s"((uint32_t)m[0]), "s"((uint32_t)(m[0] >> 32)), "s"((uint32_t)m[1]), "s"((uint32_t)(m[1] >> 32)), "s"((uint32_t)m[2]), "s"((uint32_t)(m[2] >> 32)),
          "s"((uint32_t)m[3]), "s"((uint32_t)(m[3] >> 32)), "n"(LANE), "n"(LANE + 1), "n"(LANE + 2), "n"(LANE + 3));
}

__device__ __forceinline__ void db_stage_rows(const uint8_t* img, int gp, int y0, int nrows, int cpr, uint32_t lds0, int lane, int wave) {
    const int rpi = 64 / cpr;
    const int rsub = lane / cpr, csub = lane - rsub * cpr;
    const uint32_t voff = (uint32_t)(rsub * gp + csub * 16);
    const int groups = (nrows + rpi - 1) / rpi;
    const unsigned long long base = (unsigned long long)(uintptr_t)(img + (size_t)y0 * gp);
    if (rsub < rpi)
        for (int g = wave; g < groups; g += DB_WAVES)
            if (g * rpi + rsub < nrows) sv_glds16(base + (unsigned long long)(g * rpi) * (unsigned)gp, voff, lds0 + (uint32_t)(g * rpi * cpr) * 16);
}
__device__ __forceinline__ void db_stage_rows_wide(const uint8_t* img, int gp, int y0, int nrows, int cpr, uint32_t lds0, int lane, int wave) {
    const int total = nrows * cpr;
    int q = wave * 64 + lane;
    int row = q / cpr, c = q - row * cpr;
    const int drow = (DB_WAVES * 64) / cpr, dc = (DB_WAVES * 64) - drow * cpr;
    const unsigned long long base = (unsigned long long)(uintptr_t)(img + (size_t)y0 * gp);
    uint32_t dst = lds0 + wave * 1024;
    for (int i = wave * 64; i < total; i += DB_WAVES * 64) {
        if (q < total) sv_glds16(base, (uint32_t)(row * gp + c * 16), dst);
        q += DB_WAVES * 64;
        row += drow;
        c += dc;
        if (c >= cpr) {
            c -= cpr;
            ++row;
        }
        dst += DB_WAVES * 1024;
    }
}

__global__ __launch_bounds__(DB_THREADS) void k_describe_bands(const OrbLevel* __restrict__ L, int num_levels, const DescBand* __restrict__ bands, int num_bands,
                                                               const int4* __restrict__ sel, int total_grid, const int32_t* __restrict__ cellpos,
                                                               const int32_t* __restrict__ counts,
                                                               const uint8_t* __restrict__ img0, size_t img0_frame_stride, int img0_pitch,
                                                               const uint8_t* __restrict__ pyr, size_t pyr_frame_bytes,
                                                               const uint8_t* __restrict__ blur, size_t blur_frame_bytes,
                                                               svgpu_keypoint* __restrict__ kps, uint8_t* __restrict__ desc, int cap, float* __restrict__ angles) {
    extern __shared__ __attribute__((aligned(16))) uint8_t s_band[];
    int b, bi;
    xcd_frame_map(gridDim.x, gridDim.y, bi, b);
    const DescBand bd = bands[bi];
    const int tid = threadIdx.x, lane = tid & 63, wave = __builtin_amdgcn_readfirstlane(tid >> 6);
    const int32_t* const P = cellpos + (size_t)b * (total_grid + 1);
    const int n = min(counts[b * (1 + num_levels)], cap);
    const int p0 = P[bd.cell0], nkp = min(P[bd.cell1], n) - p0;
    if (nkp <= 0) return;
    const int lv = bd.lv, lp = bd.lp, cpr = lp >> 4;
    int2* const s_xy = reinterpret_cast<int2*>(s_band + bd.img_bytes);
    int2* const s_aux = s_xy + DB_MAX_KP;
    const uint32_t lds0 = __builtin_amdgcn_readfirstlane((uint32_t)(uintptr_t)(const __attribute__((address_space(3))) uint8_t*)s_band);
    const int4* const S = sel + (size_t)b * total_grid + p0;
    int4 sv = make_int4(0, 0, 0, 0);
    if (tid < nkp) {
        sv = S[tid];
        s_xy[tid] = make_int2(sv.x, sv.y);
    }
    uint32_t w1[4], wu[4], wv[4];
#pragma unroll
    for (int m = 0; m < 4; ++m) {
        const int item = lane + 64 * m;
        w1[m] = c_icw3.w1[item];
        wu[m] = c_icw3.wu[item];
        wv[m] = c_icw3.wv[item];
    }
    float px0[4], py0[4], px1[4], py1[4];
#pragma unroll
    for (int r = 0; r < 4; ++r) {
        const float4 q = reinterpret_cast<const float4*>(c_pattern_f)[r * 64 + lane];
        px0[r] = q.x;
        py0[r] = q.y;
        px1[r] = q.z;
        py1[r] = q.w;
    }
    {
        const uint8_t* img = lv == 0 ? img0 + (size_t)b * img0_frame_stride : pyr + (size_t)b * pyr_frame_bytes + L[lv].pyr_off;
        asm volatile("s_waitcnt vmcnt(0) lgkmcnt(0)" ::: "memory");
        if (cpr <= 64) db_stage_rows(img, lv == 0 ? img0_pitch : L[lv].pitch, bd.yu0, bd.nru, cpr, lds0, lane, wave);
        else db_stage_rows_wide(img, lv == 0 ? img0_pitch : L[lv].pitch, bd.yu0, bd.nru, cpr, lds0, lane, wave);
        asm volatile("s_waitcnt vmcnt(0)" ::: "memory");
    }
    __syncthreads();
    {
        const int lane_off = (lane >> 3) * lp + 4 * (lane & 7), step = 8 * lp;
        for (int j = wave; j < nkp; j += DB_WAVES) {
            const int2 xy = s_xy[j];
            const int x = __builtin_amdgcn_readfirstlane(xy.x), y = __builtin_amdgcn_readfirstlane(xy.y);
            const int org = (y - 15 - bd.yu0) * lp + (x - 15);
            const uint32_t* U = reinterpret_cast<const uint32_t*>(s_band + ((org & ~3) + lane_off));
            const uint32_t sh = (org & 3) * 8;
            uint32_t s1 = 0, su = 0, sw = 0;
#pragma unroll
            for (int m = 0; m < 4; ++m) {
                const uint32_t lo = U[m * (step >> 2)], hi = U[m * (step >> 2) + 1];
                const uint32_t px = __builtin_amdgcn_alignbit(hi, lo, sh);
                s1 = __builtin_amdgcn_udot4(px, w1[m], s1, false);
                su = __builtin_amdgcn_udot4(px, wu[m], su, false);
                sw = __builtin_amdgcn_udot4(px, wv[m], sw, false);
            }
            const int m10 = wave_sum((int)su - __mul24(15, (int)s1)), m01 = wave_sum((int)sw - __mul24(15, (int)s1));
            if (lane == 0) s_aux[j] = make_int2(m10, m01);
        }
    }
    __syncthreads();
    if (cpr <= 64) db_stage_rows(blur + (size_t)b * blur_frame_bytes + L[lv].blur_off, L[lv].pitch, bd.yb0, bd.nrb, cpr, lds0, lane, wave);
    else db_stage_rows_wide(blur + (size_t)b * blur_frame_bytes + L[lv].blur_off, L[lv].pitch, bd.yb0, bd.nrb, cpr, lds0, lane, wave);
    if (tid < nkp) {
        const int2 mm = s_aux[tid];
        const float angle = dev_fast_atan2((float)mm.y, (float)mm.x);
        const float rad = (float)((double)angle * 3.14159265358979323846 / 180.0);
        s_aux[tid] = make_int2(__float_as_int(dev_util_cos(rad)), __float_as_int(dev_util_sin(rad)));
        svgpu_keypoint k;
        k.x = (float)sv.x;
        k.y = (float)sv.y;
        if (lv != 0) {
            k.x = k.x * L[lv].scale;
            k.y = k.y * L[lv].scale;
        }
        k.size = L[lv].kp_size;
        k.angle = angle;
        k.response = (float)sv.w;
        k.octave = lv;
        k.class_id = -1;
        kps[(size_t)b * cap + p0 + tid] = k;
        if (angles) angles[(size_t)b * cap + p0 + tid] = angle;
    }
    asm volatile("s_waitcnt vmcnt(0)" ::: "memory");
    __syncthreads();
    {
        constexpr float RN = 12582912.0f;
        const int rk = 0x400000 * lp + 0x4B400000;
        for (int j = wave; j < nkp; j += DB_WAVES) {
            const int2 xy = s_xy[j], cs2 = s_aux[j];
            const int x = __builtin_amdgcn_readfirstlane(xy.x), y = __builtin_amdgcn_readfirstlane(xy.y);
            const float ca = __int_as_float(__builtin_amdgcn_readfirstlane(cs2.x)), sa = __int_as_float(__builtin_amdgcn_readfirstlane(cs2.y));
            const uint8_t* B = s_band + ((y - bd.yb0) * lp + x - rk);
            unsigned long long bits[4];
#pragma unroll
            for (int r = 0; r < 4; ++r) {
                typedef float f32x2 __attribute__((ext_vector_type(2)));
                const f32x2 sc = {sa, ca}, cs = {ca, -sa}, rn = {RN, RN};
                const f32x2 q0 = (f32x2{px0[r], px0[r]} * sc + f32x2{py0[r], py0[r]} * cs) + rn;
                const f32x2 q1 = (f32x2{px1[r], px1[r]} * sc + f32x2{py1[r], py1[r]} * cs) + rn;
                const int a = B[__mul24(__float_as_int(q0.x), lp) + __float_as_int(q0.y)];
                const int bb = B[__mul24(__float_as_int(q1.x), lp) + __float_as_int(q1.y)];
                bits[r] = __builtin_amdgcn_ballot_w64(a < bb);
            }
            uint32_t d_lo = 0, d_hi = 0;
            sv_writelane8<0>(d_lo, d_hi, bits);
            if (lane < 4) reinterpret_cast<uint2*>(desc + ((size_t)b * cap + p0 + j) * 32)[lane] = make_uint2(d_lo, d_hi);
        }
    }
}

}

void sv_launch_resize(hipStream_t s, const uint8_t* src, size_t src_frame_stride, int src_pitch, int sw, int sh,
                      uint8_t* dst, size_t dst_frame_stride, int dst_pitch, int dw, int dh, const short* xofs,
                      const short2* xa, const short2* yofs, const short2* yb, int batch) {
    (void)sh;
    dim3 block(64, 4), grid((dw + 255) / 256, (dh + 3) / 4, batch);
    hipLaunchKernelGGL(k_resize, grid, block, 0, s, src, src_frame_stride, src_pitch, sw, dst, dst_frame_stride, dst_pitch, dw,
                       dh, xofs, xa, yofs, yb);
}

hipError_t sv_pyramid_prepare() {
    return sv_allow_dynamic_lds(reinterpret_cast<const void*>(k_pyramid_lds), SV_PYR_LDS_MAX);
}
void sv_launch_pyramid(hipStream_t s, const OrbLevel* levels, int num_levels, const int2* band_rows, int bands, const uint8_t* img0,
                       size_t img0_frame_stride, int img0_pitch, uint8_t* pyr, size_t pyr_frame_bytes, const short* xofs,
                       const short2* xa, const short2* yofs, const short2* yb, const uint32_t* xg, const short4* yrow, int batch, size_t lds_bytes) {
    if (lds_bytes > 0) {
        hipLaunchKernelGGL(k_pyramid_lds, dim3(bands, batch), dim3(PYR_THREADS), lds_bytes, s, levels, num_levels, band_rows, bands, img0,
                           img0_frame_stride, img0_pitch, pyr, pyr_frame_bytes, xg, yrow);
        return;
    }
    hipLaunchKernelGGL(k_pyramid, dim3(bands, batch), dim3(PYR_THREADS), 0, s, levels, num_levels, band_rows, img0, img0_frame_stride,
                       img0_pitch, pyr, pyr_frame_bytes, xofs, xa, yofs, yb);
}

void sv_launch_blur(hipStream_t s, const OrbLevel* levels, int num_levels, int total_tiles, int total_bands, const uint8_t* img0,
                    size_t img0_frame_stride, int img0_pitch, const uint8_t* pyr, size_t pyr_frame_bytes, uint8_t* blur,
                    size_t blur_frame_bytes, int batch, bool need_gather, int rows) {
    const dim3 grid(total_tiles, batch), block(256);
    if (rows == BLUR_ROWS_SMALL) {
        hipLaunchKernelGGL(k_blur<BLUR_ROWS_SMALL>, grid, block, 0, s, levels, num_levels, img0, img0_frame_stride, img0_pitch, pyr, pyr_frame_bytes, blur, blur_frame_bytes);
        if (need_gather)
            hipLaunchKernelGGL(k_blur_gather<BLUR_ROWS_SMALL>, grid, block, 0, s, levels, num_levels, img0, img0_frame_stride, img0_pitch, pyr, pyr_frame_bytes, blur, blur_frame_bytes);
    }
    else {
        hipLaunchKernelGGL(k_blur<BLUR_ROWS>, dim3(total_bands, batch), dim3(BLUR_BAND_THREADS), 0, s, levels, num_levels, img0, img0_frame_stride, img0_pitch, pyr,
                           pyr_frame_bytes, blur, blur_frame_bytes);
        if (need_gather)
            hipLaunchKernelGGL(k_blur_gather<BLUR_ROWS>, grid, block, 0, s, levels, num_levels, img0, img0_frame_stride, img0_pitch, pyr, pyr_frame_bytes, blur, blur_frame_bytes);
    }
}

void sv_launch_fast(hipStream_t s, const OrbLevel* levels, int num_levels, const FastCell* cells, int num_cells,
                    const uint8_t* img0, size_t img0_frame_stride, int img0_pitch, const uint8_t* pyr,
                    size_t pyr_frame_bytes, const unsigned short* gtab, unsigned long long* keys, int total_grid,
                    int ini_thr, int min_thr, const uint8_t* mask, size_t mask_frame_stride, int mask_pitch, int mask_w,
                    int mask_h, int batch) {
    if (num_cells == 0) return;
    int cpw = (long long)num_cells * batch >= 16384 ? 4 : 1;
    if (const char* e = getenv("SVGPU_FAST_CPW")) cpw = std::max(1, atoi(e));
    hipLaunchKernelGGL(k_fast, dim3((num_cells + cpw - 1) / cpw, batch), dim3(256), 0, s, levels, num_levels, cells, num_cells, cpw, img0, img0_frame_stride,
                       img0_pitch, pyr, pyr_frame_bytes, gtab, keys, total_grid, ini_thr, min_thr, mask, mask_frame_stride,
                       mask_pitch, mask_w, mask_h);
}

void sv_launch_select(hipStream_t s, const OrbLevel* levels, int num_levels, unsigned long long* keys, int total_grid,
                      int4* sel, int32_t* counts, int32_t* cellpos, int batch) {
    hipLaunchKernelGGL(k_select, dim3(batch), dim3(1024), 0, s, levels, num_levels, keys, total_grid, sel, counts, cellpos);
}

void sv_launch_describe(hipStream_t s, const OrbLevel* levels, int num_levels, const int4* sel, int total_grid,
                        const int32_t* counts, const uint8_t* img0, size_t img0_frame_stride, int img0_pitch,
                        const uint8_t* pyr, size_t pyr_frame_bytes, const uint8_t* blur, size_t blur_frame_bytes,
                        svgpu_keypoint* kps, uint8_t* desc, int cap, int batch, float* angles) {
    if (total_grid == 0) return;
    hipLaunchKernelGGL(k_describe, dim3((total_grid + 4 * DESC_KPW - 1) / (4 * DESC_KPW), batch), dim3(256), 0, s, levels, num_levels, sel, total_grid,
                       counts, img0, img0_frame_stride, img0_pitch, pyr, pyr_frame_bytes, blur, blur_frame_bytes, kps, desc, cap, angles);
}

hipError_t sv_describe_bands_prepare(size_t lds_bytes) {
    return sv_allow_dynamic_lds(reinterpret_cast<const void*>(k_describe_bands), lds_bytes);
}
void sv_launch_describe_bands(hipStream_t s, const OrbLevel* levels, int num_levels, const DescBand* bands, int num_bands, size_t lds_bytes,
                              const int4* sel, int total_grid, const int32_t* cellpos, const int32_t* counts, const uint8_t* img0,
                              size_t img0_frame_stride, int img0_pitch, const uint8_t* pyr, size_t pyr_frame_bytes, const uint8_t* blur,
                              size_t blur_frame_bytes, svgpu_keypoint* kps, uint8_t* desc, int cap, int batch, float* angles) {
    if (num_bands == 0) return;
    hipLaunchKernelGGL(k_describe_bands, dim3(num_bands, batch), dim3(DB_THREADS), lds_bytes, s, levels, num_levels, bands, num_bands, sel, total_grid,
                       cellpos, counts, img0, img0_frame_stride, img0_pitch, pyr, pyr_frame_bytes, blur, blur_frame_bytes, kps, desc, cap, angles);
}
```

stella_vslam_amd/csrc/svgpu_internal.h:

```cpp
#pragma once
#include <hip/hip_runtime.h>

#include <cstdint>
#include <cstdio>
#include <cstring>
#include <map>
#include <mutex>
#include <string>
#include <vector>

#include "svgpu.h"
#include "sv_arena.h"

#define SV_MAX_LEVELS 16
#define SV_PATCH_RADIUS 19
#define SV_CELL 64
#define SV_OVERLAP 6
#define SV_ROI_MAX 70
#ifndef BLUR_ROWS
#define BLUR_ROWS 48
#endif
#ifndef BLUR_SEG
#define BLUR_SEG 320
#endif
#ifndef BLUR_BAND_THREADS
#define BLUR_BAND_THREADS 256
#endif
#define BLUR_ROWS_SMALL 16
#define BLUR_SMALL_BATCH 4
#define BLUR_TW 256

struct OrbLevel {
    int w, h;
    int pitch;
    int has_cells;
    long long pyr_off;
    long long blur_off;
    int xtab_off, ytab_off;
    int xg_off;
    int cell_first, cell_count;
    int cells_x;
    int grid_x, grid_y, grid_first;
    int gtab_x_off, gtab_y_off;
    int btile_first, btiles_x, btiles_y;
    int bband_first, bband_segs;
    float scale;
    float kp_size;
};

struct FastCell {
    short min_x, min_y;
    short w, h;
    short lv, cj;
    int order_base;
};

struct DescBand {
    int cell0, cell1;
    int img_bytes;
    short lv, lp;
    short yu0, nru;
    short yb0, nrb;
};

struct OrbConfig {
    int width = 0, height = 0, max_batch = 0, num_levels = 0;
    float scale_factor = 0;
    int ini_thr = 0, min_thr = 0;
    unsigned min_area_sqrt = 0;
    float scale_factors[SV_MAX_LEVELS];
    OrbLevel levels[SV_MAX_LEVELS];
    std::vector<FastCell> cells;
    int total_grid = 0;
    int total_btiles = 0, total_bbands = 0;
    int blur_rows = BLUR_ROWS;
    size_t pyr_frame_bytes = 0, blur_frame_bytes = 0;
    std::vector<DescBand> dbands;
    size_t dband_lds_bytes = 0;
    bool configured = false;
};

struct SvProfClass {
    std::vector<hipEvent_t> ev;
    size_t used = 0;
    double total_ms = 0;
    long long launches = 0;
};
struct SvProf {
    std::string name;
    std::map<std::string, SvProfClass> cls;
    unsigned long long* d_counter = nullptr;
};

struct svgpu_frame {
    int device = 0;
    int n = 0, cap = 0;
    int grid_cols = 0, grid_rows = 0, cells_cap = 0;
    float min_x = 0, max_x = 0, min_y = 0, max_y = 0;
    bool has_xright = false;
    char* slab = nullptr;
    size_t slab_bytes = 0;
    svgpu_keypoint* kps_raw = nullptr;
    uint8_t* desc = nullptr;
    svgpu_keypoint* undist = nullptr;
    double* bearings = nullptr;
    float* xy = nullptr;
    int32_t* octave = nullptr;
    float* angle = nullptr;
    float* xright = nullptr;
    float* depth = nullptr;
    int32_t* cell_of = nullptr;
    int32_t* cell_items = nullptr;
    int32_t* counts = nullptr;
    int32_t* cell_off = nullptr;
    int32_t* dummy = nullptr;
};

struct svgpu_map {
    int device = 0;
    int cap = 0;
    svgpu_landmark_record* rec = nullptr;
    std::mutex mtx;
    hipEvent_t ev_write = nullptr;
    bool wrote = false;
    std::vector<hipEvent_t> reads_pending, reads_pool;
};
int sv_map_reader_begin(svgpu_ctx* ctx, svgpu_map* map, hipStream_t s);
int sv_map_reader_end(svgpu_ctx* ctx, svgpu_map* map, hipStream_t s);
struct SvMapReadScope {
    svgpu_ctx* ctx;
    svgpu_map* map;
    hipStream_t s;
    bool open = false;
    SvMapReadScope(svgpu_ctx* c, svgpu_map* m, hipStream_t st) : ctx(c), map(m), s(st) {}
    int begin() {
        const int rc = sv_map_reader_begin(ctx, map, s);
        open = rc == 0;
        return rc;
    }
    int end() {
        open = false;
        return sv_map_reader_end(ctx, map, s);
    }
    ~SvMapReadScope() {
        if (open) {
            (void)sv_map_reader_end(ctx, map, s);
            (void)hipStreamSynchronize(s);
        }
    }
    SvMapReadScope(const SvMapReadScope&) = delete;
    SvMapReadScope& operator=(const SvMapReadScope&) = delete;
};

struct svgpu_ingest {
    int device = 0;
    int width = 0, height = 0, channels = 0, color_order = 0;
    uint2* d_map = nullptr;
    int map_pitch = 0;
};

struct svgpu_ctx {
    int device = 0;
    hipStream_t stream = nullptr;
    hipStream_t stream_aux = nullptr;
    hipEvent_t ev_fork = nullptr, ev_join = nullptr;
    hipEvent_t ev_stage[2] = {nullptr, nullptr};
    bool stage_recorded = false;
    std::string last_error;
    SvProf prof;
    OrbConfig orb;
    OrbLevel* d_levels = nullptr;
    FastCell* d_cells = nullptr;
    short* d_xofs = nullptr;
    short2* d_xa = nullptr;
    short2* d_yofs = nullptr;
    short2* d_yb = nullptr;
    uint32_t* d_xg = nullptr;
    short4* d_yrow = nullptr;
    int2* d_band_rows = nullptr;
    int pyr_bands = 0;
    size_t pyr_lds_bytes = 0;
    unsigned short* d_gtab = nullptr;
    uint8_t* d_pyr = nullptr;
    uint8_t* d_blur = nullptr;
    unsigned long long* d_keys = nullptr;
    int4* d_sel = nullptr;
    int32_t* d_cellpos = nullptr;
    DescBand* d_dbands = nullptr;
    uint8_t* d_img = nullptr;
    uint8_t* d_mask = nullptr;
    svgpu_keypoint* d_kps = nullptr;
    uint8_t* d_desc = nullptr;
    int32_t* d_counts = nullptr;
    int last_batch = 0;
    int last_extract_n = -1;
    const svgpu_frame* bound_frame = nullptr;
    size_t cand_cap_hint = 0;
    const uint8_t* next_q_blocks = nullptr;
    const uint8_t* last_imgs = nullptr;
    size_t last_frame_stride = 0;
    int last_row_stride = 0;
    void* d_scratch = nullptr;
    double* h_pinned = nullptr;
    size_t pinned_doubles = 0;
    char* h_stage = nullptr;
    size_t stage_bytes = 0;
    size_t scratch_bytes = 0;
    hipStream_t ba_copy_stream = nullptr;
    hipEvent_t ev_ba_copy = nullptr;
    hipEvent_t ev_ba = nullptr;
    int ba_solver = 0;
    double pcg_tol = 1e-10;
    int pcg_max_it = 0;
    void* comm = nullptr;
    void* ba_sky = nullptr;
    svgpu_allreduce_fn ba_ar_fn = nullptr;
    void* ba_ar_user = nullptr;
    long long ba_xch[10] = {0};
    int comm_rank = 0, comm_world = 1;
};
void sv_comm_release(svgpu_ctx* ctx);

int sv_set_error(svgpu_ctx* ctx, int status, const char* what, hipError_t e = hipSuccess);
void sv_prof_begin(svgpu_ctx* ctx, hipStream_t s, const char* name);
void sv_prof_end(svgpu_ctx* ctx, hipStream_t s, const char* name);
unsigned long long* sv_prof_counter(svgpu_ctx* ctx, const char* name);
struct SvProfScope {
    svgpu_ctx* c;
    hipStream_t s;
    const char* n;
    SvProfScope(svgpu_ctx* ctx, hipStream_t st, const char* name) : c(ctx), s(st), n(name) {
        if (!c->prof.name.empty()) sv_prof_begin(c, s, n);
    }
    ~SvProfScope() {
        if (!c->prof.name.empty()) sv_prof_end(c, s, n);
    }
};
int sv_ensure_scratch(svgpu_ctx* ctx, size_t bytes);
void sv_sky_release(svgpu_ctx* ctx);
int sv_ensure_stage(svgpu_ctx* ctx, size_t bytes);
template <class Layout>
int sv_scratch_layout(svgpu_ctx* ctx, const char* overflow_msg, Layout&& layout) {
    const int rc = sv_ensure_scratch(ctx, arena_measure(layout));
    if (rc) return rc;
    Arena A(ctx->d_scratch, ctx->scratch_bytes);
    layout(A);
    return A.overflow ? sv_set_error(ctx, SVGPU_ERR_INVALID, overflow_msg) : SVGPU_OK;
}
hipError_t sv_allow_dynamic_lds(const void* kernel, size_t bytes);
void sv_orb_release(svgpu_ctx* ctx);
int sv_frame_reserve(svgpu_ctx* ctx, svgpu_frame* f, int n, int ncell);

#define SV_HIP(ctx, call)                                                   \
    do {                                                                    \
        hipError_t _e = (call);                                             \
        if (_e != hipSuccess) return sv_set_error((ctx), SVGPU_ERR_HIP, #call, _e); \
    } while (0)

void sv_launch_resize(hipStream_t s, const uint8_t* src, size_t src_frame_stride, int src_pitch, int sw, int sh,
                      uint8_t* dst, size_t dst_frame_stride, int dst_pitch, int dw, int dh, const short* xofs,
                      const short2* xa, const short2* yofs, const short2* yb, int batch);
#define SV_PYR_LDS_MAX (156 * 1024)
#define SV_PYR_LDS_HALF (78 * 1024)
hipError_t sv_pyramid_prepare();
void sv_launch_pyramid(hipStream_t s, const OrbLevel* levels, int num_levels, const int2* band_rows, int bands, const uint8_t* img0,
                       size_t img0_frame_stride, int img0_pitch, uint8_t* pyr, size_t pyr_frame_bytes, const short* xofs,
                       const short2* xa, const short2* yofs, const short2* yb, const uint32_t* xg, const short4* yrow, int batch, size_t lds_bytes);
void sv_launch_blur(hipStream_t s, const OrbLevel* levels, int num_levels, int total_tiles, int total_bands, const uint8_t* img0,
                    size_t img0_frame_stride, int img0_pitch, const uint8_t* pyr, size_t pyr_frame_bytes, uint8_t* blur,
                    size_t blur_frame_bytes, int batch, bool need_gather, int rows);
void sv_launch_fast(hipStream_t s, const OrbLevel* levels, int num_levels, const FastCell* cells, int num_cells,
                    const uint8_t* img0, size_t img0_frame_stride, int img0_pitch, const uint8_t* pyr,
                    size_t pyr_frame_bytes, const unsigned short* gtab, unsigned long long* keys, int total_grid,
                    int ini_thr, int min_thr, const uint8_t* mask, size_t mask_frame_stride, int mask_pitch, int mask_w,
                    int mask_h, int batch);
void sv_launch_select(hipStream_t s, const OrbLevel* levels, int num_levels, unsigned long long* keys, int total_grid,
                      int4* sel, int32_t* counts, int32_t* cellpos, int batch);
hipError_t sv_describe_bands_prepare(size_t lds_bytes);
void sv_launch_describe_bands(hipStream_t s, const OrbLevel* levels, int num_levels, const DescBand* bands, int num_bands, size_t lds_bytes,
                              const int4* sel, int total_grid, const int32_t* cellpos, const int32_t* counts, const uint8_t* img0,
                              size_t img0_frame_stride, int img0_pitch, const uint8_t* pyr, size_t pyr_frame_bytes, const uint8_t* blur,
                              size_t blur_frame_bytes, svgpu_keypoint* kps, uint8_t* desc, int cap, int batch, float* angles);
void sv_launch_describe(hipStream_t s, const OrbLevel* levels, int num_levels, const int4* sel, int total_grid,
                        const int32_t* counts, const uint8_t* img0, size_t img0_frame_stride, int img0_pitch,
                        const uint8_t* pyr, size_t pyr_frame_bytes, const uint8_t* blur, size_t blur_frame_bytes,
                        svgpu_keypoint* kps, uint8_t* desc, int cap, int batch, float* angles);
```

stella_vslam_amd/csrc/svgpu_orb.hip:

```cpp
#include <algorithm>
#include <cmath>
#include <cstdlib>

#include "svgpu_internal.h"

#pragma clang fp contract(off)
#pragma STDC FP_CONTRACT OFF

namespace {

inline int cv_floor_f(float v) {
    int i = (int)v;
    return i - (i > v);
}
inline int cv_round_f(float v) { return (int)lrintf(v); }
inline size_t align_up(size_t v, size_t a) { return (v + a - 1) / a * a; }

template <class T>
int upload(svgpu_ctx* ctx, T** dptr, const std::vector<T>& v) {
    if (*dptr) {
        SV_HIP(ctx, hipFree(*dptr));
        *dptr = nullptr;
    }
    const size_t n = v.empty() ? 1 : v.size();
    SV_HIP(ctx, hipMalloc((void**)dptr, n * sizeof(T)));
    if (!v.empty()) SV_HIP(ctx, hipMemcpy(*dptr, v.data(), v.size() * sizeof(T), hipMemcpyHostToDevice));
    return SVGPU_OK;
}

template <class T>
void free_dev(T*& p) {
    if (p) (void)hipFree(p);
    p = nullptr;
}

}

void sv_orb_release(svgpu_ctx* ctx) {
    free_dev(ctx->d_levels);
    free_dev(ctx->d_cells);
    free_dev(ctx->d_xofs);
    free_dev(ctx->d_xa);
    free_dev(ctx->d_yofs);
    free_dev(ctx->d_yb);
    free_dev(ctx->d_xg);
    free_dev(ctx->d_yrow);
    free_dev(ctx->d_band_rows);
    free_dev(ctx->d_gtab);
    free_dev(ctx->d_pyr);
    free_dev(ctx->d_blur);
    free_dev(ctx->d_keys);
    free_dev(ctx->d_sel);
    free_dev(ctx->d_cellpos);
    free_dev(ctx->d_dbands);
    free_dev(ctx->d_img);
    free_dev(ctx->d_mask);
    free_dev(ctx->d_kps);
    free_dev(ctx->d_desc);
    free_dev(ctx->d_counts);
    ctx->orb.configured = false;
    ctx->last_extract_n = -1;
    ctx->last_batch = 0;
}

extern "C" {

int svgpu_orb_scale_tables(float scale_factor, int num_levels, float* scale_factors, float* inv_scale_factors,
                           float* level_sigma_sq, float* inv_level_sigma_sq) {
    if (num_levels < 1) return SVGPU_ERR_INVALID;
    float s = 1.0f, inv = 1.0f;
    for (int l = 0; l < num_levels; ++l) {
        if (l > 0) {
            s = scale_factor * s;
            inv = (1.0f / scale_factor) * inv;
        }
        if (scale_factors) scale_factors[l] = s;
        if (inv_scale_factors) inv_scale_factors[l] = inv;
        if (level_sigma_sq) level_sigma_sq[l] = l == 0 ? 1.0f : s * s;
        if (inv_level_sigma_sq) inv_level_sigma_sq[l] = l == 0 ? 1.0f : 1.0f / (s * s);
    }
    return SVGPU_OK;
}

int svgpu_orb_configure(svgpu_ctx* ctx, int width, int height, int max_batch, float scale_factor, int num_levels,
                        int ini_fast_thr, int min_fast_thr, unsigned min_area) {
    if (!ctx) return SVGPU_ERR_INVALID;
    if (width < 8 || height < 8 || width > 16384 || height > 16384 || max_batch < 1 || num_levels < 1
        || num_levels > SV_MAX_LEVELS || !(scale_factor > 1.0f))
        return sv_set_error(ctx, SVGPU_ERR_INVALID, "svgpu_orb_configure: bad geometry/parameters");
    SV_HIP(ctx, hipSetDevice(ctx->device));
    SV_HIP(ctx, hipStreamSynchronize(ctx->stream));
    sv_orb_release(ctx);
    OrbConfig& C = ctx->orb;
    C = OrbConfig();
    C.width = width;
    C.height = height;
    C.max_batch = max_batch;
    C.blur_rows = max_batch <= BLUR_SMALL_BATCH ? BLUR_ROWS_SMALL : BLUR_ROWS;
    C.num_levels = num_levels;
    C.scale_factor = scale_factor;
    C.ini_thr = ini_fast_thr < 0 ? 0 : (ini_fast_thr > 255 ? 255 : ini_fast_thr);
    C.min_thr = min_fast_thr < 0 ? 0 : (min_fast_thr > 255 ? 255 : min_fast_thr);
    C.min_area_sqrt = (unsigned)std::sqrt((double)min_area);
    svgpu_orb_scale_tables(scale_factor, num_levels, C.scale_factors, nullptr, nullptr, nullptr);

    std::vector<short> xofs;
    std::vector<short2> xa, yofs, yb;
    std::vector<unsigned short> gtab;
    std::vector<uint32_t> xg;
    std::vector<short4> yrow;
    bool xg_ok = true;
    size_t pyr_off = 0, blur_off = 0;
    int grid_first = 0, btile_first = 0, bband_first = 0;
    std::vector<std::pair<int, int>> grid_rows[SV_MAX_LEVELS];
    for (int l = 0; l < num_levels; ++l) {
        OrbLevel& L = C.levels[l];
        memset(&L, 0, sizeof(L));
        const float s = C.scale_factors[l];
        if (l == 0) {
            L.w = width;
            L.h = height;
        }
        else {
            const double scale = (double)s;
            L.w = (int)std::round(width * 1.0 / scale);
            L.h = (int)std::round(height * 1.0 / scale);
        }
        if (L.w < 2 || L.h < 2) return sv_set_error(ctx, SVGPU_ERR_INVALID, "pyramid level smaller than 2 px");
        L.pitch = (int)align_up(L.w, 64);
        L.scale = s;
        L.kp_size = (float)(unsigned)(31u * s);
        L.blur_off = (long long)blur_off;
        blur_off += align_up((size_t)L.pitch * L.h, 256);
        if (l > 0) {
            L.pyr_off = (long long)pyr_off;
            pyr_off += align_up((size_t)L.pitch * L.h, 256);
            const OrbLevel& P = C.levels[l - 1];
            const double inv_scale_x = (double)L.w / P.w, inv_scale_y = (double)L.h / P.h;
            const double scale_x = 1. / inv_scale_x, scale_y = 1. / inv_scale_y;
            L.xtab_off = (int)xofs.size();
            L.ytab_off = (int)yofs.size();
            for (int dx = 0; dx < L.w; ++dx) {
                float fx = (float)((dx + 0.5) * scale_x - 0.5);
                int sx = cv_floor_f(fx);
                fx -= sx;
                if (sx < 0) {
                    fx = 0;
                    sx = 0;
                }
                if (sx >= P.w - 1) {
                    fx = 0;
                    sx = P.w - 1;
                }
                xofs.push_back((short)sx);
                short2 a;
                a.x = (short)cv_round_f((1.f - fx) * 2048);
                a.y = (short)cv_round_f(fx * 2048);
                xa.push_back(a);
            }
            for (int dy = 0; dy < L.h; ++dy) {
                float fy = (float)((dy + 0.5) * scale_y - 0.5);
                int sy = cv_floor_f(fy);
                fy -= sy;
                short2 o, bb;
                o.x = (short)(sy < 0 ? 0 : (sy > P.h - 1 ? P.h - 1 : sy));
                o.y = (short)(sy + 1 < 0 ? 0 : (sy + 1 > P.h - 1 ? P.h - 1 : sy + 1));
                bb.x = (short)cv_round_f((1.f - fy) * 2048);
                bb.y = (short)cv_round_f(fy * 2048);
                yofs.push_back(o);
                yb.push_back(bb);
            }
            L.xg_off = (int)(xg.size() / 8);
            for (int c = 0; c < L.w; c += 4) {
                int sxs[4];
                for (int i = 0; i < 4; ++i) sxs[i] = xofs[L.xtab_off + std::min(c + i, L.w - 1)];
                const int base0 = sxs[0] >> 2, base2 = sxs[2] >> 2;
                const int k[4] = {sxs[0] - 4 * base0, sxs[1] - 4 * base0, sxs[2] - 4 * base2, sxs[3] - 4 * base2};
                for (int i = 0; i < 4; ++i) xg_ok = xg_ok && k[i] >= 0 && k[i] <= 6;
                xg.push_back((uint32_t)base0 | ((uint32_t)base2 << 16));
                xg.push_back((uint32_t)(k[0] & 255) | ((uint32_t)(k[1] & 255) << 8) | ((uint32_t)(k[2] & 255) << 16) | ((uint32_t)(k[3] & 255) << 24));
                for (int i = 0; i < 4; ++i) {
                    const short2 a = xa[L.xtab_off + std::min(c + i, L.w - 1)];
                    xg_ok = xg_ok && a.x >= 0 && a.y >= 0;
                    xg.push_back((uint32_t)(unsigned short)a.x | ((uint32_t)(unsigned short)a.y << 16));
                }
                xg.push_back(0);
                xg.push_back(0);
            }
            for (int dy = 0; dy < L.h; ++dy) {
                const short2 o = yofs[L.ytab_off + dy], c = yb[L.ytab_off + dy];
                xg_ok = xg_ok && c.x >= 0 && c.y >= 0;
                yrow.push_back(make_short4(o.x, o.y, c.x, c.y));
            }
        }
        L.btile_first = btile_first;
        L.btiles_x = (L.w + BLUR_TW - 1) / BLUR_TW;
        L.btiles_y = (L.h + 4 * C.blur_rows - 1) / (4 * C.blur_rows);
        btile_first += L.btiles_x * L.btiles_y + ((L.h + 7) / 8 + 63) / 64;
        L.bband_first = bband_first;
        L.bband_segs = (L.w + BLUR_SEG - 1) / BLUR_SEG;
        bband_first += L.bband_segs * ((L.h + BLUR_ROWS - 1) / BLUR_ROWS);
        L.cell_first = (int)C.cells.size();
        L.grid_first = grid_first;
        L.gtab_x_off = L.gtab_y_off = (int)gtab.size();
        if (L.w > 2 * SV_PATCH_RADIUS && L.h > 2 * SV_PATCH_RADIUS) {
            L.has_cells = 1;
            const unsigned min_bx = SV_PATCH_RADIUS, min_by = SV_PATCH_RADIUS;
            const unsigned max_bx = L.w - SV_PATCH_RADIUS, max_by = L.h - SV_PATCH_RADIUS;
            const unsigned rw = max_bx - min_bx, rh = max_by - min_by;
            const unsigned num_cols = rw / SV_CELL + 1, num_rows = rh / SV_CELL + 1;
            L.cells_x = (int)num_cols;
            for (unsigned i = 0; i < num_rows; ++i) {
                const unsigned min_y = min_by + i * SV_CELL;
                if (max_by - SV_OVERLAP <= min_y) continue;
                unsigned max_y = min_y + SV_CELL + SV_OVERLAP;
                if (max_by < max_y) max_y = max_by;
                for (unsigned j = 0; j < num_cols; ++j) {
                    const unsigned min_x = min_bx + j * SV_CELL;
                    if (max_bx - SV_OVERLAP <= min_x) continue;
                    unsigned max_x = min_x + SV_CELL + SV_OVERLAP;
                    if (max_bx < max_x) max_x = max_bx;
                    FastCell c;
                    c.min_x = (short)min_x;
                    c.min_y = (short)min_y;
                    c.w = (short)(max_x - min_x);
                    c.h = (short)(max_y - min_y);
                    c.lv = (short)l;
                    c.cj = (short)j;
                    c.order_base = (int)((i * num_cols + j) << 14);
                    C.cells.push_back(c);
                }
            }
            const double scaled_min_area_sqrt = C.min_area_sqrt / s;
            const unsigned gx = (unsigned)std::ceil((int)rw / scaled_min_area_sqrt);
            const unsigned gy = (unsigned)std::ceil((int)rh / scaled_min_area_sqrt);
            const double delta_x = (double)(int)rw / gx, delta_y = (double)(int)rh / gy;
            L.grid_x = (int)gx;
            L.grid_y = (int)gy;
            L.gtab_x_off = (int)gtab.size();
            for (unsigned x = 0; x < rw; ++x) {
                unsigned ix = (unsigned)((float)x / delta_x);
                gtab.push_back((unsigned short)(ix < gx ? ix : gx - 1));
            }
            L.gtab_y_off = (int)gtab.size();
            grid_rows[l].assign(gy, std::make_pair(1 << 30, -1));
            for (unsigned y = 0; y < rh; ++y) {
                unsigned iy = (unsigned)((float)y / delta_y);
                iy = iy < gy ? iy : gy - 1;
                gtab.push_back((unsigned short)iy);
                grid_rows[l][iy].first = std::min(grid_rows[l][iy].first, (int)(min_by + y));
                grid_rows[l][iy].second = std::max(grid_rows[l][iy].second, (int)(min_by + y));
            }
            grid_first += (int)(gx * gy);
        }
        L.cell_count = (int)C.cells.size() - L.cell_first;
    }
    C.total_grid = grid_first;
    C.total_btiles = btile_first;
    C.total_bbands = bband_first;
    {
        C.dbands.clear();
        C.dband_lds_bytes = 0;
        size_t budget = 48 * 1024;
        if (const char* e = getenv("SVGPU_DESC_BAND_KB")) budget = (size_t)std::max(1, atoi(e)) * 1024;
        const size_t hard_limit = 80 * 1024;
        bool ok = C.total_grid > 0 && getenv("SVGPU_DESCRIBE_LEGACY") == nullptr;
        for (int l = 0; l < num_levels && ok; ++l) {
            const OrbLevel& L = C.levels[l];
            if (!L.has_cells) continue;
            int lp = (L.w + 15) / 16 * 16;
            while (lp % 64 != 32) lp += 16;
            if (lp > 32000) ok = false;
            const int gy = L.grid_y, gx = L.grid_x;
            auto band_bytes = [&](int g0, int g1, DescBand* out) {
                int y0 = 1 << 30, y1 = -1;
                for (int g = g0; g < g1; ++g)
                    if (grid_rows[l][g].second >= 0) {
                        y0 = std::min(y0, grid_rows[l][g].first);
                        y1 = std::max(y1, grid_rows[l][g].second);
                    }
                if (y1 < 0) y0 = y1 = SV_PATCH_RADIUS;
                const int nru = y1 - y0 + 32, nrb = y1 - y0 + 37;
                const int rpi = std::max(1, 64 / (lp / 16));
                const size_t bytes = (size_t)((std::max(nru, nrb) + rpi - 1) / rpi * rpi) * lp;
                if (out) {
                    out->lv = (short)l;
                    out->lp = (short)lp;
                    out->yu0 = (short)(y0 - 15);
                    out->nru = (short)nru;
                    out->yb0 = (short)(y0 - 18);
                    out->nrb = (short)nrb;
                    out->img_bytes = (int)bytes;
                    out->cell0 = L.grid_first + g0 * gx;
                    out->cell1 = L.grid_first + g1 * gx;
                }
                return bytes;
            };
            if (gx > 128) ok = false;
            for (int g0 = 0; g0 < gy && ok;) {
                int g1 = g0 + 1;
                if (band_bytes(g0, g1, nullptr) > hard_limit) ok = false;
                while (g1 < gy && (g1 + 1 - g0) * gx <= 128 && band_bytes(g0, g1 + 1, nullptr) <= budget) ++g1;
                DescBand bd;
                C.dband_lds_bytes = std::max(C.dband_lds_bytes, band_bytes(g0, g1, &bd));
                C.dbands.push_back(bd);
                g0 = g1;
            }
        }
        if (!ok) C.dbands.clear();
        std::stable_sort(C.dbands.begin(), C.dbands.end(), [](const DescBand& a, const DescBand& b) { return a.img_bytes > b.img_bytes; });
        if (!C.dbands.empty()) C.dband_lds_bytes += 2 * 128 * sizeof(int2);
    }
    C.pyr_frame_bytes = pyr_off ? pyr_off : 256;
    C.blur_frame_bytes = blur_off;

    auto make_bands = [&](int bands, std::vector<int2>& band_rows) -> size_t {
        band_rows.assign((size_t)bands * num_levels, int2{0, 0});
        size_t worst = 0;
        for (int k = 0; k < bands; ++k) {
            int need_lo = 0, need_hi = 0;
            for (int l = num_levels - 1; l >= 1; --l) {
                const OrbLevel& Lv = C.levels[l];
                int lo = (int)((long long)k * Lv.h / bands), hi = (int)((long long)(k + 1) * Lv.h / bands);
                if (l < num_levels - 1 && need_hi > need_lo) {
                    lo = std::min(lo, need_lo);
                    hi = std::max(hi, need_hi);
                }
                band_rows[(size_t)k * num_levels + l] = int2{lo, hi};
                need_lo = 1 << 30;
                need_hi = 0;
                for (int dy = lo; dy < hi; ++dy) {
                    const short2 o = yofs[Lv.ytab_off + dy];
                    need_lo = std::min(need_lo, (int)o.x);
                    need_hi = std::max(need_hi, (int)o.y + 1);
                }
            }
            if (need_hi > need_lo) band_rows[(size_t)k * num_levels] = int2{need_lo, need_hi};
            size_t size_a = 0, size_b = 0;
            for (int l = 0; l < num_levels; ++l) {
                const int2 r = band_rows[(size_t)k * num_levels + l];
                const size_t b = (size_t)(r.y - r.x) * (size_t)((C.levels[l].w + 3) & ~3);
                if (l & 1) size_a = std::max(size_a, b);
                else size_b = std::max(size_b, b);
            }
            size_a = (size_a + 15) & ~(size_t)15;
            size_b = (size_b + 15) & ~(size_t)15;
            size_t bytes = size_a + size_b;
            for (int l = 1; l < num_levels; ++l) {
                const int2 r = band_rows[(size_t)k * num_levels + l];
                bytes += (size_t)(r.y - r.x) * 8;
            }
            worst = std::max(worst, bytes);
        }
        return worst;
    };
    std::vector<int2> band_rows;
    int bands = std::max(8, std::min(32, (512 + max_batch - 1) / std::max(max_batch, 1)));
    bool forced = false;
    if (const char* e = getenv("SVGPU_PYR_BANDS")) {
        bands = std::max(1, atoi(e));
        forced = true;
    }
    xg_ok = xg_ok && (num_levels < 2 || C.levels[1].w <= 4 * 1024);
    size_t lds = 0;
    if (!forced && xg_ok) {
        std::vector<int2> trial;
        for (int k = bands; k <= 32; k += 2)
            if (make_bands(k, trial) <= SV_PYR_LDS_HALF) {
                bands = k;
                break;
            }
    }
    for (;; bands += 2) {
        lds = make_bands(bands, band_rows);
        if (lds <= SV_PYR_LDS_MAX && xg_ok) break;
        if (bands >= 256 || !xg_ok) {
            bands = 16;
            make_bands(bands, band_rows);
            lds = 0;
            break;
        }
    }
    ctx->pyr_bands = bands;
    ctx->pyr_lds_bytes = lds;
    if (lds) SV_HIP(ctx, sv_pyramid_prepare());
    {
        int rcb;
        if ((rcb = upload(ctx, &ctx->d_band_rows, band_rows))) return rcb;
    }
    std::vector<OrbLevel> lv(C.levels, C.levels + num_levels);
    int rc;
    if ((rc = upload(ctx, &ctx->d_levels, lv))) return rc;
    if ((rc = upload(ctx, &ctx->d_cells, C.cells))) return rc;
    if ((rc = upload(ctx, &ctx->d_xofs, xofs))) return rc;
    if ((rc = upload(ctx, &ctx->d_xa, xa))) return rc;
    if ((rc = upload(ctx, &ctx->d_yofs, yofs))) return rc;
    if ((rc = upload(ctx, &ctx->d_yb, yb))) return rc;
    if ((rc = upload(ctx, &ctx->d_xg, xg))) return rc;
    if ((rc = upload(ctx, &ctx->d_yrow, yrow))) return rc;
    if ((rc = upload(ctx, &ctx->d_gtab, gtab))) return rc;
    if (!C.dbands.empty()) {
        if ((rc = upload(ctx, &ctx->d_dbands, C.dbands))) return rc;
        SV_HIP(ctx, sv_describe_bands_prepare(C.dband_lds_bytes));
    }
    const size_t B = (size_t)max_batch, G = (size_t)(C.total_grid > 0 ? C.total_grid : 1);
    SV_HIP(ctx, hipMalloc((void**)&ctx->d_pyr, B * C.pyr_frame_bytes + 256));
    SV_HIP(ctx, hipMalloc((void**)&ctx->d_blur, B * C.blur_frame_bytes + 4096));
    SV_HIP(ctx, hipMalloc((void**)&ctx->d_cellpos, B * (G + 1) * sizeof(int32_t)));
    SV_HIP(ctx, hipMalloc((void**)&ctx->d_keys, B * G * sizeof(unsigned long long)));
    SV_HIP(ctx, hipMemset(ctx->d_keys, 0, B * G * sizeof(unsigned long long)));
    SV_HIP(ctx, hipMalloc((void**)&ctx->d_sel, (B * G + 8) * sizeof(int4)));
    SV_HIP(ctx, hipMalloc((void**)&ctx->d_img, (size_t)C.levels[0].pitch * height));
    SV_HIP(ctx, hipMalloc((void**)&ctx->d_mask, (size_t)C.levels[0].pitch * height));
    SV_HIP(ctx, hipMalloc((void**)&ctx->d_kps, G * sizeof(svgpu_keypoint)));
    SV_HIP(ctx, hipMalloc((void**)&ctx->d_desc, G * 32));
    SV_HIP(ctx, hipMalloc((void**)&ctx->d_counts, (1 + SV_MAX_LEVELS) * sizeof(int32_t)));
    C.configured = true;
    return SVGPU_OK;
}

int svgpu_orb_max_keypoints(const svgpu_ctx* ctx) { return (ctx && ctx->orb.configured) ? ctx->orb.total_grid : -1; }

int svgpu_orb_level_size(const svgpu_ctx* ctx, int level, int* width, int* height) {
    if (!ctx || !ctx->orb.configured) return SVGPU_ERR_NOT_CONFIGURED;
    if (level < 0 || level >= ctx->orb.num_levels) return SVGPU_ERR_INVALID;
    if (width) *width = ctx->orb.levels[level].w;
    if (height) *height = ctx->orb.levels[level].h;
    return SVGPU_OK;
}

int svgpu_orb_extract_batch_device(svgpu_ctx* ctx, const uint8_t* imgs_dev, int batch, size_t frame_stride,
                                   int row_stride, const uint8_t* mask_dev, size_t mask_frame_stride,
                                   int mask_row_stride, svgpu_keypoint* kps_dev, uint8_t* desc_dev, int cap,
                                   int32_t* counts_dev, void* stream) {
    return svgpu_orb_extract_batch_device_angles(ctx, imgs_dev, batch, frame_stride, row_stride, mask_dev, mask_frame_stride, mask_row_stride, kps_dev, desc_dev, cap,
                                                 counts_dev, nullptr, stream);
}

int svgpu_orb_extract_batch_device_angles(svgpu_ctx* ctx, const uint8_t* imgs_dev, int batch, size_t frame_stride,
                                          int row_stride, const uint8_t* mask_dev, size_t mask_frame_stride,
                                          int mask_row_stride, svgpu_keypoint* kps_dev, uint8_t* desc_dev, int cap,
                                          int32_t* counts_dev, float* angles_dev, void* stream) {
    if (!ctx) return SVGPU_ERR_INVALID;
    OrbConfig& C = ctx->orb;
    if (!C.configured) return sv_set_error(ctx, SVGPU_ERR_NOT_CONFIGURED, "svgpu_orb_configure has not been called");
    if (!imgs_dev || !kps_dev || !desc_dev || !counts_dev || batch < 1 || batch > C.max_batch || cap < 1
        || row_stride < C.width)
        return sv_set_error(ctx, SVGPU_ERR_INVALID, "svgpu_orb_extract_batch_device: bad arguments");
    SV_HIP(ctx, hipSetDevice(ctx->device));
    hipStream_t s = stream ? (hipStream_t)stream : ctx->stream;
    ctx->last_extract_n = -1;
    const int Lc = C.num_levels;
    if (Lc > 1) {
        SvProfScope ps(ctx, s, "k_resize");
        sv_launch_pyramid(s, ctx->d_levels, Lc, ctx->d_band_rows, ctx->pyr_bands, imgs_dev, frame_stride, row_stride, ctx->d_pyr,
                          C.pyr_frame_bytes, ctx->d_xofs, ctx->d_xa, ctx->d_yofs, ctx->d_yb, ctx->d_xg, ctx->d_yrow, batch, ctx->pyr_lds_bytes);
    }
    static const bool fork_blur = getenv("SVGPU_FORK_BLUR") != nullptr;
    hipStream_t sb = (ctx->stream_aux && fork_blur) ? ctx->stream_aux : s;
    if (sb != s) {
        SV_HIP(ctx, hipEventRecord(ctx->ev_fork, s));
        SV_HIP(ctx, hipStreamWaitEvent(sb, ctx->ev_fork, 0));
    }
    {
        SvProfScope ps(ctx, sb, "k_blur");
        bool need_gather = (((size_t)imgs_dev | (size_t)frame_stride | (size_t)row_stride) & 3) != 0;
        for (int l = 0; l < Lc; ++l) need_gather = need_gather || C.levels[l].w < 16;
        sv_launch_blur(sb, ctx->d_levels, Lc, C.total_btiles, C.total_bbands, imgs_dev, frame_stride, row_stride, ctx->d_pyr, C.pyr_frame_bytes,
                       ctx->d_blur, C.blur_frame_bytes, batch, need_gather, C.blur_rows);
    }
    if (sb != s) SV_HIP(ctx, hipEventRecord(ctx->ev_join, sb));
    SV_HIP(ctx, hipEventRecord(ctx->ev_stage[0], s));
    {
        SvProfScope ps(ctx, s, "k_fast");
        sv_launch_fast(s, ctx->d_levels, Lc, ctx->d_cells, (int)C.cells.size(), imgs_dev, frame_stride, row_stride, ctx->d_pyr,
                   C.pyr_frame_bytes, ctx->d_gtab, ctx->d_keys, C.total_grid, C.ini_thr, C.min_thr, mask_dev,
                       mask_frame_stride, mask_row_stride, C.width, C.height, batch);
    }
    {
        SvProfScope ps(ctx, s, "k_select");
        sv_launch_select(s, ctx->d_levels, Lc, ctx->d_keys, C.total_grid, ctx->d_sel, counts_dev, C.dbands.empty() ? nullptr : ctx->d_cellpos, batch);
    }
    if (sb != s) SV_HIP(ctx, hipStreamWaitEvent(s, ctx->ev_join, 0));
    SV_HIP(ctx, hipEventRecord(ctx->ev_stage[1], s));
    ctx->stage_recorded = true;
    SvProfScope ps(ctx, s, "k_describe");
    const bool bands = !C.dbands.empty() && ((long long)batch * C.total_grid >= 32768 || getenv("SVGPU_DESCRIBE_BANDS") != nullptr);
    if (bands)
        sv_launch_describe_bands(s, ctx->d_levels, Lc, ctx->d_dbands, (int)C.dbands.size(), C.dband_lds_bytes, ctx->d_sel, C.total_grid, ctx->d_cellpos,
                                 counts_dev, imgs_dev, frame_stride, row_stride, ctx->d_pyr, C.pyr_frame_bytes, ctx->d_blur, C.blur_frame_bytes,
                                 kps_dev, desc_dev, cap, batch, angles_dev);
    else
        sv_launch_describe(s, ctx->d_levels, Lc, ctx->d_sel, C.total_grid, counts_dev, imgs_dev, frame_stride, row_stride,
                           ctx->d_pyr, C.pyr_frame_bytes, ctx->d_blur, C.blur_frame_bytes, kps_dev, desc_dev, cap, batch, angles_dev);
    SV_HIP(ctx, hipGetLastError());
    ctx->last_batch = batch;
    ctx->last_imgs = imgs_dev;
    ctx->last_frame_stride = frame_stride;
    ctx->last_row_stride = row_stride;
    return SVGPU_OK;
}

int svgpu_orb_stream_wait_stage(svgpu_ctx* ctx, int stage, void* stream) {
    if (!ctx || stage < 0 || stage > 1 || !stream) return sv_set_error(ctx, SVGPU_ERR_INVALID, "svgpu_orb_stream_wait_stage: bad arguments");
    if (!ctx->stage_recorded) return SVGPU_OK;
    SV_HIP(ctx, hipSetDevice(ctx->device));
    SV_HIP(ctx, hipStreamWaitEvent((hipStream_t)stream, ctx->ev_stage[stage], 0));
    return SVGPU_OK;
}

int svgpu_orb_extract(svgpu_ctx* ctx, const uint8_t* img, int stride, const uint8_t* mask, int mask_stride,
                      svgpu_keypoint* kps, uint8_t* desc, int cap, int* n_out, int* level_counts) {
    if (!ctx) return SVGPU_ERR_INVALID;
    OrbConfig& C = ctx->orb;
    if (!C.configured) return sv_set_error(ctx, SVGPU_ERR_NOT_CONFIGURED, "svgpu_orb_configure has not been called");
    if (!img || !n_out || stride < C.width || cap < 0 || (cap > 0 && (!kps || !desc)) || (mask && mask_stride < C.width))
        return sv_set_error(ctx, SVGPU_ERR_INVALID, "svgpu_orb_extract: bad arguments");
    SV_HIP(ctx, hipSetDevice(ctx->device));
    hipStream_t s = ctx->stream;
    const int pitch = C.levels[0].pitch;
    SV_HIP(ctx, hipMemcpy2DAsync(ctx->d_img, pitch, img, stride, C.width, C.height, hipMemcpyHostToDevice, s));
    if (mask) SV_HIP(ctx, hipMemcpy2DAsync(ctx->d_mask, pitch, mask, mask_stride, C.width, C.height, hipMemcpyHostToDevice, s));
    const int icap = C.total_grid > 0 ? C.total_grid : 1;
    int rc = svgpu_orb_extract_batch_device(ctx, ctx->d_img, 1, (size_t)pitch * C.height, pitch, mask ? ctx->d_mask : nullptr, 0,
                                            pitch, ctx->d_kps, ctx->d_desc, icap, ctx->d_counts, s);
    if (rc) return rc;
    int32_t counts[1 + SV_MAX_LEVELS];
    SV_HIP(ctx, hipMemcpyAsync(counts, ctx->d_counts, (1 + C.num_levels) * sizeof(int32_t), hipMemcpyDeviceToHost, s));
    SV_HIP(ctx, hipStreamSynchronize(s));
    const int n = counts[0];
    *n_out = n;
    ctx->last_extract_n = n < icap ? n : icap;
    if (level_counts)
        for (int l = 0; l < C.num_levels; ++l) level_counts[l] = counts[1 + l];
    const int m = n < cap ? n : cap;
    if (m > 0) {
        SV_HIP(ctx, hipMemcpyAsync(kps, ctx->d_kps, (size_t)m * sizeof(svgpu_keypoint), hipMemcpyDeviceToHost, s));
        SV_HIP(ctx, hipMemcpyAsync(desc, ctx->d_desc, (size_t)m * 32, hipMemcpyDeviceToHost, s));
        SV_HIP(ctx, hipStreamSynchronize(s));
    }
    return n > cap ? sv_set_error(ctx, SVGPU_ERR_CAPACITY, "svgpu_orb_extract: more keypoints than cap") : SVGPU_OK;
}

static int download_level(svgpu_ctx* ctx, const uint8_t* base, size_t frame_bytes, long long off, int frame, int level,
                          uint8_t* dst, int dst_stride) {
    OrbConfig& C = ctx->orb;
    const OrbLevel& L = C.levels[level];
    if (!dst || dst_stride < L.w) return sv_set_error(ctx, SVGPU_ERR_INVALID, "download: bad destination");
    SV_HIP(ctx, hipSetDevice(ctx->device));
    SV_HIP(ctx, hipStreamSynchronize(ctx->stream));
    SV_HIP(ctx, hipMemcpy2D(dst, dst_stride, base + (size_t)frame * frame_bytes + off, L.pitch, L.w, L.h, hipMemcpyDeviceToHost));
    return SVGPU_OK;
}

int svgpu_orb_pyramid_download(svgpu_ctx* ctx, int frame, int level, uint8_t* dst, int dst_stride) {
    if (!ctx) return SVGPU_ERR_INVALID;
    OrbConfig& C = ctx->orb;
    if (!C.configured || ctx->last_batch == 0) return sv_set_error(ctx, SVGPU_ERR_NOT_CONFIGURED, "no extract call yet");
    if (frame < 0 || frame >= ctx->last_batch || level < 0 || level >= C.num_levels)
        return sv_set_error(ctx, SVGPU_ERR_INVALID, "pyramid_download: bad frame/level");
    if (level == 0) {
        if (!dst || dst_stride < C.width) return sv_set_error(ctx, SVGPU_ERR_INVALID, "download: bad destination");
        SV_HIP(ctx, hipSetDevice(ctx->device));
        SV_HIP(ctx, hipStreamSynchronize(ctx->stream));
        SV_HIP(ctx, hipMemcpy2D(dst, dst_stride, ctx->last_imgs + (size_t)frame * ctx->last_frame_stride, ctx->last_row_stride,
                                C.width, C.height, hipMemcpyDeviceToHost));
        return SVGPU_OK;
    }
    return download_level(ctx, ctx->d_pyr, C.pyr_frame_bytes, C.levels[level].pyr_off, frame, level, dst, dst_stride);
}

int svgpu_orb_blurred_download(svgpu_ctx* ctx, int frame, int level, uint8_t* dst, int dst_stride) {
    if (!ctx) return SVGPU_ERR_INVALID;
    OrbConfig& C = ctx->orb;
    if (!C.configured || ctx->last_batch == 0) return sv_set_error(ctx, SVGPU_ERR_NOT_CONFIGURED, "no extract call yet");
    if (frame < 0 || frame >= ctx->last_batch || level < 0 || level >= C.num_levels)
        return sv_set_error(ctx, SVGPU_ERR_INVALID, "blurred_download: bad frame/level");
    return download_level(ctx, ctx->d_blur, C.blur_frame_bytes, C.levels[level].blur_off, frame, level, dst, dst_stride);
}

}
```

Baseline: 278,000.

## Precompute per-band pyramid work plans with cost-modeled chunking and wave-uniform fast path

Adds a host-side planner that picks pyramid band counts and a per-band, per-level plan: row chunk size, lanes per chunk, a magic multiplier for the division, and owned-row bounds. The plan is chosen with an instruction-cost model of wavefronts. The kernel reads this plan instead of computing the float division and integer divides at runtime. When a chunk is wave-uniform, it uses a specialized path that hoists the y-table entries into scalar registers via readfirstlane and uses SGPR-operand multiplies. The aim is less per-lane VALU and LDS work and better load balance in the resize kernel. In exchange it adds host complexity and a new public planning API, and correctness depends on the planner's uniformity flag being right.

```diff
diff --git a/include/svgpu.h b/include/svgpu.h
--- a/include/svgpu.h
+++ b/include/svgpu.h
@@ -50,6 +50,10 @@
 
 int svgpu_orb_configure(svgpu_ctx* ctx, int width, int height, int max_batch, float scale_factor, int num_levels,
                         int ini_fast_thr, int min_fast_thr, unsigned min_area);
+
+#define SVGPU_PYR_PLAN_INTS 10
+int svgpu_orb_pyramid_plan(int width, int height, int max_batch, float scale_factor, int num_levels, int* bands,
+                           int* entries, int entries_cap, long long* model);
 
 int svgpu_orb_stream_wait_stage(svgpu_ctx* ctx, int stage, void* stream);
 
diff --git a/stella_vslam_amd/csrc/orb_kernels.hip b/stella_vslam_amd/csrc/orb_kernels.hip
--- a/stella_vslam_amd/csrc/orb_kernels.hip
+++ b/stella_vslam_amd/csrc/orb_kernels.hip
@@ -1,6 +1,7 @@
 #include "svgpu_internal.h"
 #include "sv_trig.h"
 #include <cstdlib>
+#include <type_traits>
 #include <utility>
 
 #pragma clang fp contract(off)
@@ -153,14 +154,21 @@
     return d;
 }
 
+__device__ __forceinline__ uint32_t mul_hi_u24_s(uint32_t a, uint32_t b) {
+    uint32_t d;
+    asm("v_mul_hi_u32_u24 %0, %1, %2" : "=v"(d) : "s"(a), "v"(b));
+    return d;
+}
+
 __global__ __launch_bounds__(PYR_THREADS) void k_pyramid_lds(const OrbLevel* __restrict__ L, int num_levels, const int2* __restrict__ band_rows,
-                                                             int bands, const uint8_t* __restrict__ img0, size_t img0_frame_stride,
+                                                             const PyrPlan* __restrict__ plan, const uint8_t* __restrict__ img0, size_t img0_frame_stride,
                                                              int img0_pitch, uint8_t* __restrict__ pyr, size_t pyr_frame_bytes,
                                                              const uint32_t* __restrict__ xg, const short4* __restrict__ yrow) {
     extern __shared__ __attribute__((aligned(16))) uint8_t s_mem[];
     __shared__ int s_img[SV_MAX_LEVELS], s_yt[SV_MAX_LEVELS + 1];
     const int band = blockIdx.x, b = blockIdx.y, tid = threadIdx.x;
     const int2* BR = band_rows + (size_t)band * num_levels;
+    const PyrPlan* PL = plan + (size_t)band * num_levels;
     if (tid == 0) {
         int size_a = 0, size_b = 0;
         for (int l = 0; l < num_levels; ++l) {
@@ -219,64 +227,86 @@
     uint8_t* P = pyr + (size_t)b * pyr_frame_bytes;
     for (int l = 1; l < num_levels; ++l) {
         const OrbLevel lev = L[l];
+        const PyrPlan pl = PL[l];
         const int spw = ((L[l - 1].w + 3) & ~3) >> 2, dpw = ((lev.w + 3) & ~3) >> 2;
         const int src_lo = BR[l - 1].x, lo = BR[l].x, hi = BR[l].y;
-        const int own_lo = (int)((long long)band * lev.h / bands), own_hi = (int)((long long)(band + 1) * lev.h / bands);
         const uint32_t* S = reinterpret_cast<const uint32_t*>(s_mem + s_img[l - 1]);
         uint32_t* Dl = reinterpret_cast<uint32_t*>(s_mem + s_img[l]);
         const short4* yt = reinterpret_cast<const short4*>(s_mem + s_yt[l]);
         uint8_t* Dg = P + lev.pyr_off;
         const int groups = (lev.w + 3) >> 2, nrows = hi - lo;
-        const int chunks = max(min(PYR_THREADS / groups, nrows), 1), rc = (nrows + chunks - 1) / chunks;
-        const int c = (int)(((float)tid + 0.5f) * (1.0f / (float)groups)), g = tid - __mul24(c, groups);
-        const int r0 = __mul24(c, rc), r1 = min(r0 + rc, nrows);
-        if (r0 < r1) {
-            const uint4 e = reinterpret_cast<const uint4*>(xg)[2 * (lev.xg_off + g)];
-            const uint2 e2 = reinterpret_cast<const uint2*>(xg)[4 * (lev.xg_off + g) + 2];
-            const int i0 = e.x & 0xffff, i2 = e.x >> 16;
-            const uint32_t coef[4] = {e.z, e.w, e2.x, e2.y};
-            uint32_t sel[4];
-#pragma unroll
-            for (int i = 0; i < 4; ++i) sel[i] = 0x0c010c00u + ((e.y >> (8 * i)) & 255u) * 0x00010001u;
-            const uint32_t* S0 = S + (i0 - __mul24(src_lo, spw));
-            const int d2 = i2 - i0;
-            auto hrow = [&](int sy, uint32_t (&h)[4]) {
-                const uint32_t* R = S0 + __mul24(sy, spw);
-                const uint32_t a0 = R[0], a1 = R[1], c0 = R[d2], c1 = R[d2 + 1];
-                h[0] = __builtin_amdgcn_udot2(as_u16x2(__builtin_amdgcn_perm(a1, a0, sel[0])), as_u16x2(coef[0]), 0u, false) & ~15u;
-                h[1] = __builtin_amdgcn_udot2(as_u16x2(__builtin_amdgcn_perm(a1, a0, sel[1])), as_u16x2(coef[1]), 0u, false) & ~15u;
-                h[2] = __builtin_amdgcn_udot2(as_u16x2(__builtin_amdgcn_perm(c1, c0, sel[2])), as_u16x2(coef[2]), 0u, false) & ~15u;
-                h[3] = __builtin_amdgcn_udot2(as_u16x2(__builtin_amdgcn_perm(c1, c0, sel[3])), as_u16x2(coef[3]), 0u, false) & ~15u;
-            };
-            uint32_t* dl = Dl + (__mul24(r0, dpw) + g);
-            uint32_t goff = __umul24(lo + r0, lev.pitch) + 4 * g;
-            const uint32_t own_n = (uint32_t)(own_hi - own_lo);
-            uint32_t dyo = (uint32_t)(lo + r0 - own_lo);
-            int prev = -1;
-            auto step = [&](int row, uint32_t (&top)[4], uint32_t (&bot)[4]) {
-                const short4 ye = yt[row];
-                if (ye.x != prev) hrow(ye.x, top);
-                hrow(ye.y, bot);
-                prev = ye.y;
-                const uint32_t b0 = (uint32_t)ye.z << 12, b1 = (uint32_t)ye.w << 12;
-                uint32_t v[4];
-#pragma unroll
-                for (int i = 0; i < 4; ++i) v[i] = (mul_hi_u24(b0, top[i]) + mul_hi_u24(b1, bot[i]) + 2u) >> 2;
-                const uint32_t packed = (v[0] & 255u) | ((v[1] & 255u) << 8) | ((v[2] & 255u) << 16) | (v[3] << 24);
-                *dl = packed;
-                if (dyo < own_n) *reinterpret_cast<uint32_t*>(Dg + goff) = packed;
-                dl += dpw;
-                goff += (uint32_t)lev.pitch;
-                ++dyo;
-            };
-            uint32_t hX[4], hY[4] = {0, 0, 0, 0};
-            int row = r0;
-            for (; row + 1 < r1; row += 2) {
-                step(row, hY, hX);
-                step(row + 1, hX, hY);
-            }
-            if (row < r1) step(row, hY, hX);
-        }
+        auto level = [&](auto uni) {
+            constexpr bool U = decltype(uni)::value;
+            int c = (int)(((uint32_t)tid * (uint32_t)pl.magic) >> 20);
+            if (U) c = __builtin_amdgcn_readfirstlane(c);
+            const int g = tid - __mul24(c, pl.lpc);
+            const int r0 = __mul24(c, pl.rc), r1 = min(r0 + pl.rc, nrows);
+            if (g < groups && r0 < r1) {
+                const uint4 e = reinterpret_cast<const uint4*>(xg)[2 * (lev.xg_off + g)];
+                const uint2 e2 = reinterpret_cast<const uint2*>(xg)[4 * (lev.xg_off + g) + 2];
+                const int i0 = e.x & 0xffff, i2 = e.x >> 16;
+                const uint32_t coef[4] = {e.z, e.w, e2.x, e2.y};
+                uint32_t sel[4];
+#pragma unroll
+                for (int i = 0; i < 4; ++i) sel[i] = 0x0c010c00u + ((e.y >> (8 * i)) & 255u) * 0x00010001u;
+                const uint32_t* S0 = S + (i0 - __mul24(src_lo, spw));
+                const int d2 = i2 - i0;
+                auto hrow = [&](int sy, uint32_t (&h)[4]) {
+                    const uint32_t* R = S0 + __mul24(sy, spw);
+                    const uint32_t a0 = R[0], a1 = R[1], c0 = R[d2], c1 = R[d2 + 1];
+                    h[0] = __builtin_amdgcn_udot2(as_u16x2(__builtin_amdgcn_perm(a1, a0, sel[0])), as_u16x2(coef[0]), 0u, false) & ~15u;
+                    h[1] = __builtin_amdgcn_udot2(as_u16x2(__builtin_amdgcn_perm(a1, a0, sel[1])), as_u16x2(coef[1]), 0u, false) & ~15u;
+                    h[2] = __builtin_amdgcn_udot2(as_u16x2(__builtin_amdgcn_perm(c1, c0, sel[2])), as_u16x2(coef[2]), 0u, false) & ~15u;
+                    h[3] = __builtin_amdgcn_udot2(as_u16x2(__builtin_amdgcn_perm(c1, c0, sel[3])), as_u16x2(coef[3]), 0u, false) & ~15u;
+                };
+                uint32_t* dl = Dl + (__mul24(r0, dpw) + g);
+                uint32_t goff = __umul24(lo + r0, lev.pitch) + 4 * g;
+                const uint32_t own_n = (uint32_t)(pl.own_hi - pl.own_lo);
+                uint32_t dyo = (uint32_t)(lo + r0 - pl.own_lo);
+                int prev = -1;
+                auto step = [&](int row, uint32_t (&top)[4], uint32_t (&bot)[4]) {
+                    int sy0, sy1;
+                    uint32_t b0, b1;
+                    if constexpr (U) {
+                        const uint2 q = reinterpret_cast<const uint2*>(yt)[row];
+                        const uint32_t q0 = __builtin_amdgcn_readfirstlane(q.x), q1 = __builtin_amdgcn_readfirstlane(q.y);
+                        sy0 = (int)(short)(q0 & 0xffffu);
+                        sy1 = (int)q0 >> 16;
+                        b0 = (q1 & 0xffffu) << 12;
+                        b1 = (q1 >> 16) << 12;
+                    }
+                    else {
+                        const short4 ye = yt[row];
+                        sy0 = ye.x;
+                        sy1 = ye.y;
+                        b0 = (uint32_t)ye.z << 12;
+                        b1 = (uint32_t)ye.w << 12;
+                    }
+                    if (sy0 != prev) hrow(sy0, top);
+                    hrow(sy1, bot);
+                    prev = sy1;
+                    uint32_t v[4];
+#pragma unroll
+                    for (int i = 0; i < 4; ++i)
+                        v[i] = ((U ? mul_hi_u24_s(b0, top[i]) : mul_hi_u24(b0, top[i])) + (U ? mul_hi_u24_s(b1, bot[i]) : mul_hi_u24(b1, bot[i])) + 2u) >> 2;
+                    const uint32_t packed = (v[0] & 255u) | ((v[1] & 255u) << 8) | ((v[2] & 255u) << 16) | (v[3] << 24);
+                    *dl = packed;
+                    if (dyo < own_n) *reinterpret_cast<uint32_t*>(Dg + goff) = packed;
+                    dl += dpw;
+                    goff += (uint32_t)lev.pitch;
+                    ++dyo;
+                };
+                uint32_t hX[4], hY[4] = {0, 0, 0, 0};
+                int row = r0;
+                for (; row + 1 < r1; row += 2) {
+                    step(row, hY, hX);
+                    step(row + 1, hX, hY);
+                }
+                if (row < r1) step(row, hY, hX);
+            }
+        };
+        if (pl.uniform) level(std::true_type{});
+        else level(std::false_type{});
         __syncthreads();
     }
 }
@@ -1269,11 +1299,11 @@
 hipError_t sv_pyramid_prepare() {
     return sv_allow_dynamic_lds(reinterpret_cast<const void*>(k_pyramid_lds), SV_PYR_LDS_MAX);
 }
-void sv_launch_pyramid(hipStream_t s, const OrbLevel* levels, int num_levels, const int2* band_rows, int bands, const uint8_t* img0,
+void sv_launch_pyramid(hipStream_t s, const OrbLevel* levels, int num_levels, const int2* band_rows, const PyrPlan* plan, int bands, const uint8_t* img0,
                        size_t img0_frame_stride, int img0_pitch, uint8_t* pyr, size_t pyr_frame_bytes, const short* xofs,
                        const short2* xa, const short2* yofs, const short2* yb, const uint32_t* xg, const short4* yrow, int batch, size_t lds_bytes) {
     if (lds_bytes > 0) {
-        hipLaunchKernelGGL(k_pyramid_lds, dim3(bands, batch), dim3(PYR_THREADS), lds_bytes, s, levels, num_levels, band_rows, bands, img0,
+        hipLaunchKernelGGL(k_pyramid_lds, dim3(bands, batch), dim3(PYR_THREADS), lds_bytes, s, levels, num_levels, band_rows, plan, img0,
                            img0_frame_stride, img0_pitch, pyr, pyr_frame_bytes, xg, yrow);
         return;
     }
diff --git a/stella_vslam_amd/csrc/svgpu_internal.h b/stella_vslam_amd/csrc/svgpu_internal.h
--- a/stella_vslam_amd/csrc/svgpu_internal.h
+++ b/stella_vslam_amd/csrc/svgpu_internal.h
@@ -53,6 +53,15 @@
     short w, h;
     short lv, cj;
     int order_base;
+};
+
+struct PyrPlan {
+    int rc, chunks;
+    int lpc;
+    int magic;
+    int uniform;
+    int own_lo, own_hi;
+    int reserved;
 };
 
 struct DescBand {
@@ -178,6 +187,7 @@
     uint32_t* d_xg = nullptr;
     short4* d_yrow = nullptr;
     int2* d_band_rows = nullptr;
+    PyrPlan* d_pyr_plan = nullptr;
     int pyr_bands = 0;
     size_t pyr_lds_bytes = 0;
     unsigned short* d_gtab = nullptr;
@@ -263,7 +273,7 @@
 #define SV_PYR_LDS_MAX (156 * 1024)
 #define SV_PYR_LDS_HALF (78 * 1024)
 hipError_t sv_pyramid_prepare();
-void sv_launch_pyramid(hipStream_t s, const OrbLevel* levels, int num_levels, const int2* band_rows, int bands, const uint8_t* img0,
+void sv_launch_pyramid(hipStream_t s, const OrbLevel* levels, int num_levels, const int2* band_rows, const PyrPlan* plan, int bands, const uint8_t* img0,
                        size_t img0_frame_stride, int img0_pitch, uint8_t* pyr, size_t pyr_frame_bytes, const short* xofs,
                        const short2* xa, const short2* yofs, const short2* yb, const uint32_t* xg, const short4* yrow, int batch, size_t lds_bytes);
 void sv_launch_blur(hipStream_t s, const OrbLevel* levels, int num_levels, int total_tiles, int total_bands, const uint8_t* img0,
diff --git a/stella_vslam_amd/csrc/svgpu_orb.hip b/stella_vslam_amd/csrc/svgpu_orb.hip
--- a/stella_vslam_amd/csrc/svgpu_orb.hip
+++ b/stella_vslam_amd/csrc/svgpu_orb.hip
@@ -34,6 +34,324 @@
     p = nullptr;
 }
 
+bool pyr_level_size(int width, int height, float s, int l, int* w, int* h) {
+    if (l == 0) {
+        *w = width;
+        *h = height;
+    }
+    else {
+        const double scale = (double)s;
+        *w = (int)std::round(width * 1.0 / scale);
+        *h = (int)std::round(height * 1.0 / scale);
+    }
+    return *w >= 2 && *h >= 2;
+}
+
+struct PyrTables {
+    std::vector<short> xofs;
+    std::vector<short2> xa, yofs, yb;
+    std::vector<uint32_t> xg;
+    std::vector<short4> yrow;
+    bool xg_ok = true;
+};
+
+void pyr_level_tables(const OrbLevel& P, OrbLevel& L, PyrTables& T) {
+    std::vector<short>& xofs = T.xofs;
+    std::vector<short2>&xa = T.xa, &yofs = T.yofs, &yb = T.yb;
+    std::vector<uint32_t>& xg = T.xg;
+    bool& xg_ok = T.xg_ok;
+    const double inv_scale_x = (double)L.w / P.w, inv_scale_y = (double)L.h / P.h;
+    const double scale_x = 1. / inv_scale_x, scale_y = 1. / inv_scale_y;
+    L.xtab_off = (int)xofs.size();
+    L.ytab_off = (int)yofs.size();
+    for (int dx = 0; dx < L.w; ++dx) {
+        float fx = (float)((dx + 0.5) * scale_x - 0.5);
+        int sx = cv_floor_f(fx);
+        fx -= sx;
+        if (sx < 0) {
+            fx = 0;
+            sx = 0;
+        }
+        if (sx >= P.w - 1) {
+            fx = 0;
+            sx = P.w - 1;
+        }
+        xofs.push_back((short)sx);
+        short2 a;
+        a.x = (short)cv_round_f((1.f - fx) * 2048);
+        a.y = (short)cv_round_f(fx * 2048);
+        xa.push_back(a);
+    }
+    for (int dy = 0; dy < L.h; ++dy) {
+        float fy = (float)((dy + 0.5) * scale_y - 0.5);
+        int sy = cv_floor_f(fy);
+        fy -= sy;
+        short2 o, bb;
+        o.x = (short)(sy < 0 ? 0 : (sy > P.h - 1 ? P.h - 1 : sy));
+        o.y = (short)(sy + 1 < 0 ? 0 : (sy + 1 > P.h - 1 ? P.h - 1 : sy + 1));
+        bb.x = (short)cv_round_f((1.f - fy) * 2048);
+        bb.y = (short)cv_round_f(fy * 2048);
+        yofs.push_back(o);
+        yb.push_back(bb);
+    }
+    L.xg_off = (int)(xg.size() / 8);
+    for (int c = 0; c < L.w; c += 4) {
+        int sxs[4];
+        for (int i = 0; i < 4; ++i) sxs[i] = xofs[L.xtab_off + std::min(c + i, L.w - 1)];
+        const int base0 = sxs[0] >> 2, base2 = sxs[2] >> 2;
+        const int k[4] = {sxs[0] - 4 * base0, sxs[1] - 4 * base0, sxs[2] - 4 * base2, sxs[3] - 4 * base2};
+        for (int i = 0; i < 4; ++i) xg_ok = xg_ok && k[i] >= 0 && k[i] <= 6;
+        xg.push_back((uint32_t)base0 | ((uint32_t)base2 << 16));
+        xg.push_back((uint32_t)(k[0] & 255) | ((uint32_t)(k[1] & 255) << 8) | ((uint32_t)(k[2] & 255) << 16) | ((uint32_t)(k[3] & 255) << 24));
+        for (int i = 0; i < 4; ++i) {
+            const short2 a = xa[L.xtab_off + std::min(c + i, L.w - 1)];
+            xg_ok = xg_ok && a.x >= 0 && a.y >= 0;
+            xg.push_back((uint32_t)(unsigned short)a.x | ((uint32_t)(unsigned short)a.y << 16));
+        }
+        xg.push_back(0);
+        xg.push_back(0);
+    }
+    for (int dy = 0; dy < L.h; ++dy) {
+        const short2 o = yofs[L.ytab_off + dy], c = yb[L.ytab_off + dy];
+        xg_ok = xg_ok && c.x >= 0 && c.y >= 0;
+        T.yrow.push_back(make_short4(o.x, o.y, c.x, c.y));
+    }
+}
+
+struct PyrModel {
+    int H, V, setup_all, setup_rows;
+};
+const PyrModel PYR_MODEL_PARENT = {15, 32, 28, 54}, PYR_MODEL_PACKED = {15, 32, 5, 53}, PYR_MODEL_ALIGNED = {14, 25, 5, 23};
+struct PyrCost {
+    long long insts = 0;
+    long long longest = 0;
+};
+PyrCost pyr_plan_cost(const PyrModel& M, int groups, int nrows, const short4* yr, int rc, int lpc) {
+    PyrCost out;
+    for (int w = 0; w < 1024 / 64; ++w) {
+        long long cost = M.setup_all;
+        int cs[64], nc = 0;
+        for (int c = (64 * w) / lpc; c <= (64 * w + 63) / lpc; ++c) {
+            const int first = std::max(64 * w, c * lpc), last = std::min(64 * w + 63, c * lpc + groups - 1);
+            if (first <= last && c * rc < nrows) cs[nc++] = c;
+        }
+        if (nc) {
+            cost += M.setup_rows;
+            for (int s = 0; s < rc; ++s) {
+                bool any = false, top = false;
+                for (int i = 0; i < nc; ++i) {
+                    const int row = cs[i] * rc + s;
+                    if (row >= std::min(cs[i] * rc + rc, nrows)) continue;
+                    any = true;
+                    top = top || s == 0 || yr[row].x != yr[row - 1].y;
+                }
+                if (any) cost += M.V + M.H + (top ? M.H : 0);
+            }
+        }
+        out.insts += cost;
+        out.longest = std::max(out.longest, cost);
+    }
+    return out;
+}
+
+void pyr_parent_mapping(int groups, int nrows, int* rc, int* lpc) {
+    const int chunks = std::max(std::min(1024 / groups, nrows), 1);
+    *rc = (nrows + chunks - 1) / chunks;
+    *lpc = groups;
+}
+
+#define PYR_LONGEST_CAP 2
+PyrPlan plan_pyramid_lanes(int groups, int nrows, const short4* yr, PyrCost* parent_cost, PyrCost* plan_cost) {
+    PyrPlan best;
+    memset(&best, 0, sizeof(best));
+    if (nrows < 1) {
+        best.rc = 1;
+        best.lpc = groups;
+        best.magic = ((1 << 20) + groups - 1) / groups;
+        PyrCost none;
+        none.longest = PYR_MODEL_PARENT.setup_all;
+        none.insts = 16 * none.longest;
+        if (parent_cost) *parent_cost = none;
+        none.longest = PYR_MODEL_PACKED.setup_all;
+        none.insts = 16 * none.longest;
+        if (plan_cost) *plan_cost = none;
+        return best;
+    }
+    int prc, plpc;
+    pyr_parent_mapping(groups, nrows, &prc, &plpc);
+    const PyrCost pc = pyr_plan_cost(PYR_MODEL_PARENT, groups, nrows, yr, prc, plpc);
+    PyrCost bc;
+    bool have = false;
+    for (int aligned = 0; aligned < 2; ++aligned) {
+        const int lpc = aligned ? (groups + 63) / 64 * 64 : groups;
+        const int max_chunks = (1024 - groups) / lpc + 1;
+        for (int rc = 1; rc <= nrows; ++rc) {
+            const int chunks = (nrows + rc - 1) / rc;
+            if (chunks > max_chunks) continue;
+            const PyrCost c = pyr_plan_cost(aligned ? PYR_MODEL_ALIGNED : PYR_MODEL_PACKED, groups, nrows, yr, rc, lpc);
+            if (c.longest > PYR_LONGEST_CAP * pc.longest) continue;
+            if (!have || c.insts < bc.insts || (c.insts == bc.insts && c.longest < bc.longest)) {
+                have = true;
+                bc = c;
+                best.rc = rc;
+                best.chunks = chunks;
+                best.lpc = lpc;
+                best.uniform = aligned;
+            }
+        }
+    }
+    if (!have) {
+        best.rc = prc;
+        best.lpc = plpc;
+        best.chunks = (nrows + prc - 1) / prc;
+        best.uniform = 0;
+        bc = pyr_plan_cost(PYR_MODEL_PACKED, groups, nrows, yr, prc, plpc);
+    }
+    best.magic = ((1 << 20) + best.lpc - 1) / best.lpc;
+    if (parent_cost) *parent_cost = pc;
+    if (plan_cost) *plan_cost = bc;
+    return best;
+}
+
+struct PyrBands {
+    int bands = 0;
+    size_t lds = 0;
+    std::vector<int2> rows;
+    std::vector<PyrPlan> plan;
+    std::vector<PyrCost> parent_cost, plan_cost;
+};
+
+PyrBands plan_pyramid(const OrbLevel* levels, int num_levels, int max_batch, const PyrTables& T) {
+    const std::vector<short2>& yofs = T.yofs;
+    bool xg_ok = T.xg_ok;
+    auto make_bands = [&](int bands, std::vector<int2>& band_rows) -> size_t {
+        band_rows.assign((size_t)bands * num_levels, int2{0, 0});
+        size_t worst = 0;
+        for (int k = 0; k < bands; ++k) {
+            int need_lo = 0, need_hi = 0;
+            for (int l = num_levels - 1; l >= 1; --l) {
+                const OrbLevel& Lv = levels[l];
+                int lo = (int)((long long)k * Lv.h / bands), hi = (int)((long long)(k + 1) * Lv.h / bands);
+                if (l < num_levels - 1 && need_hi > need_lo) {
+                    lo = std::min(lo, need_lo);
+                    hi = std::max(hi, need_hi);
+                }
+                band_rows[(size_t)k * num_levels + l] = int2{lo, hi};
+                need_lo = 1 << 30;
+                need_hi = 0;
+                for (int dy = lo; dy < hi; ++dy) {
+                    const short2 o = yofs[Lv.ytab_off + dy];
+                    need_lo = std::min(need_lo, (int)o.x);
+                    need_hi = std::max(need_hi, (int)o.y + 1);
+                }
+            }
+            if (need_hi > need_lo) band_rows[(size_t)k * num_levels] = int2{need_lo, need_hi};
+            size_t size_a = 0, size_b = 0;
+            for (int l = 0; l < num_levels; ++l) {
+                const int2 r = band_rows[(size_t)k * num_levels + l];
+                const size_t b = (size_t)(r.y - r.x) * (size_t)((levels[l].w + 3) & ~3);
+                if (l & 1) size_a = std::max(size_a, b);
+                else size_b = std::max(size_b, b);
+            }
+            size_a = (size_a + 15) & ~(size_t)15;
+            size_b = (size_b + 15) & ~(size_t)15;
+            size_t bytes = size_a + size_b;
+            for (int l = 1; l < num_levels; ++l) {
+                const int2 r = band_rows[(size_t)k * num_levels + l];
+                bytes += (size_t)(r.y - r.x) * 8;
+            }
+            worst = std::max(worst, bytes);
+        }
+        return worst;
+    };
+    std::vector<int2> band_rows;
+    int bands = std::max(8, std::min(32, (512 + max_batch - 1) / std::max(max_batch, 1)));
+    bool forced = false;
+    if (const char* e = getenv("SVGPU_PYR_BANDS")) {
+        bands = std::max(1, atoi(e));
+        forced = true;
+    }
+    xg_ok = xg_ok && (num_levels < 2 || levels[1].w <= 4 * 1024);
+    size_t lds = 0;
+    if (!forced && xg_ok) {
+        std::vector<int2> trial;
+        for (int k = bands; k <= 32; k += 2)
+            if (make_bands(k, trial) <= SV_PYR_LDS_HALF) {
+                bands = k;
+                break;
+            }
+    }
+    for (;; bands += 2) {
+        lds = make_bands(bands, band_rows);
+        if (lds <= SV_PYR_LDS_MAX && xg_ok) break;
+        if (bands >= 256 || !xg_ok) {
+            bands = 16;
+            make_bands(bands, band_rows);
+            lds = 0;
+            break;
+        }
+    }
+    PyrBands out;
+    out.bands = bands;
+    out.lds = lds;
+    out.plan.assign((size_t)bands * num_levels, PyrPlan{});
+    out.parent_cost.assign((size_t)bands * num_levels, PyrCost{});
+    out.plan_cost.assign((size_t)bands * num_levels, PyrCost{});
+    if (lds)
+        for (int k = 0; k < bands; ++k)
+            for (int l = 1; l < num_levels; ++l) {
+                const size_t i = (size_t)k * num_levels + l;
+                const int2 r = band_rows[i];
+                PyrPlan p = plan_pyramid_lanes((levels[l].w + 3) >> 2, r.y - r.x, T.yrow.data() + levels[l].ytab_off + r.x, &out.parent_cost[i], &out.plan_cost[i]);
+                p.own_lo = (int)((long long)k * levels[l].h / bands);
+                p.own_hi = (int)((long long)(k + 1) * levels[l].h / bands);
+                out.plan[i] = p;
+            }
+    out.rows = std::move(band_rows);
+    return out;
+}
+
+}
+
+extern "C" int svgpu_orb_pyramid_plan(int width, int height, int max_batch, float scale_factor, int num_levels, int* bands_out,
+                                      int* entries, int entries_cap, long long* model) {
+    if (width < 8 || height < 8 || width > 16384 || height > 16384 || max_batch < 1 || num_levels < 1 || num_levels > SV_MAX_LEVELS
+        || !(scale_factor > 1.0f) || !bands_out)
+        return SVGPU_ERR_INVALID;
+    float sf[SV_MAX_LEVELS];
+    svgpu_orb_scale_tables(scale_factor, num_levels, sf, nullptr, nullptr, nullptr);
+    OrbLevel lv[SV_MAX_LEVELS];
+    PyrTables T;
+    for (int l = 0; l < num_levels; ++l) {
+        memset(&lv[l], 0, sizeof(OrbLevel));
+        if (!pyr_level_size(width, height, sf[l], l, &lv[l].w, &lv[l].h)) return SVGPU_ERR_INVALID;
+        if (l > 0) pyr_level_tables(lv[l - 1], lv[l], T);
+    }
+    const PyrBands PB = plan_pyramid(lv, num_levels, max_batch, T);
+    *bands_out = PB.lds ? PB.bands : 0;
+    if (!PB.lds) return SVGPU_OK;
+    const int n = PB.bands * num_levels;
+    if (entries) {
+        if (entries_cap < n) return SVGPU_ERR_CAPACITY;
+        for (int i = 0; i < n; ++i) {
+            const PyrPlan& p = PB.plan[i];
+            const int v[SVGPU_PYR_PLAN_INTS] = {PB.rows[i].x, PB.rows[i].y, (lv[i % num_levels].w + 3) >> 2, p.rc, p.chunks, p.lpc, p.magic, p.uniform, p.own_lo, p.own_hi};
+            memcpy(entries + (size_t)i * SVGPU_PYR_PLAN_INTS, v, sizeof(v));
+        }
+    }
+    if (model)
+        for (int l = 0; l < num_levels; ++l) {
+            long long m[4] = {0, 0, 0, 0};
+            for (int k = 0; k < PB.bands; ++k) {
+                const size_t i = (size_t)k * num_levels + l;
+                m[0] += PB.parent_cost[i].insts;
+                m[1] += PB.plan_cost[i].insts;
+                m[2] = std::max(m[2], PB.parent_cost[i].longest);
+                m[3] = std::max(m[3], PB.plan_cost[i].longest);
+            }
+            memcpy(model + 4 * l, m, sizeof(m));
+        }
+    return SVGPU_OK;
 }
 
 void sv_orb_release(svgpu_ctx* ctx) {
@@ -46,6 +364,7 @@
     free_dev(ctx->d_xg);
     free_dev(ctx->d_yrow);
     free_dev(ctx->d_band_rows);
+    free_dev(ctx->d_pyr_plan);
     free_dev(ctx->d_gtab);
     free_dev(ctx->d_pyr);
     free_dev(ctx->d_blur);
@@ -104,12 +423,8 @@
     C.min_area_sqrt = (unsigned)std::sqrt((double)min_area);
     svgpu_orb_scale_tables(scale_factor, num_levels, C.scale_factors, nullptr, nullptr, nullptr);
 
-    std::vector<short> xofs;
-    std::vector<short2> xa, yofs, yb;
     std::vector<unsigned short> gtab;
-    std::vector<uint32_t> xg;
-    std::vector<short4> yrow;
-    bool xg_ok = true;
+    PyrTables T;
     size_t pyr_off = 0, blur_off = 0;
     int grid_first = 0, btile_first = 0, bband_first = 0;
     std::vector<std::pair<int, int>> grid_rows[SV_MAX_LEVELS];
@@ -117,16 +432,7 @@
         OrbLevel& L = C.levels[l];
         memset(&L, 0, sizeof(L));
         const float s = C.scale_factors[l];
-        if (l == 0) {
-            L.w = width;
-            L.h = height;
-        }
-        else {
-            const double scale = (double)s;
-            L.w = (int)std::round(width * 1.0 / scale);
-            L.h = (int)std::round(height * 1.0 / scale);
-        }
-        if (L.w < 2 || L.h < 2) return sv_set_error(ctx, SVGPU_ERR_INVALID, "pyramid level smaller than 2 px");
+        if (!pyr_level_size(width, height, s, l, &L.w, &L.h)) return sv_set_error(ctx, SVGPU_ERR_INVALID, "pyramid level smaller than 2 px");
         L.pitch = (int)align_up(L.w, 64);
         L.scale = s;
         L.kp_size = (float)(unsigned)(31u * s);
@@ -135,63 +441,7 @@
         if (l > 0) {
             L.pyr_off = (long long)pyr_off;
             pyr_off += align_up((size_t)L.pitch * L.h, 256);
-            const OrbLevel& P = C.levels[l - 1];
-            const double inv_scale_x = (double)L.w / P.w, inv_scale_y = (double)L.h / P.h;
-            const double scale_x = 1. / inv_scale_x, scale_y = 1. / inv_scale_y;
-            L.xtab_off = (int)xofs.size();
-            L.ytab_off = (int)yofs.size();
-            for (int dx = 0; dx < L.w; ++dx) {
-                float fx = (float)((dx + 0.5) * scale_x - 0.5);
-                int sx = cv_floor_f(fx);
-                fx -= sx;
-                if (sx < 0) {
-                    fx = 0;
-                    sx = 0;
-                }
-                if (sx >= P.w - 1) {
-                    fx = 0;
-                    sx = P.w - 1;
-                }
-                xofs.push_back((short)sx);
-                short2 a;
-                a.x = (short)cv_round_f((1.f - fx) * 2048);
-                a.y = (short)cv_round_f(fx * 2048);
-                xa.push_back(a);
-            }
-            for (int dy = 0; dy < L.h; ++dy) {
-                float fy = (float)((dy + 0.5) * scale_y - 0.5);
-                int sy = cv_floor_f(fy);
-                fy -= sy;
-                short2 o, bb;
-                o.x = (short)(sy < 0 ? 0 : (sy > P.h - 1 ? P.h - 1 : sy));
-                o.y = (short)(sy + 1 < 0 ? 0 : (sy + 1 > P.h - 1 ? P.h - 1 : sy + 1));
-                bb.x = (short)cv_round_f((1.f - fy) * 2048);
-                bb.y = (short)cv_round_f(fy * 2048);
-                yofs.push_back(o);
-                yb.push_back(bb);
-            }
-            L.xg_off = (int)(xg.size() / 8);
-            for (int c = 0; c < L.w; c += 4) {
-                int sxs[4];
-                for (int i = 0; i < 4; ++i) sxs[i] = xofs[L.xtab_off + std::min(c + i, L.w - 1)];
-                const int base0 = sxs[0] >> 2, base2 = sxs[2] >> 2;
-                const int k[4] = {sxs[0] - 4 * base0, sxs[1] - 4 * base0, sxs[2] - 4 * base2, sxs[3] - 4 * base2};
-                for (int i = 0; i < 4; ++i) xg_ok = xg_ok && k[i] >= 0 && k[i] <= 6;
-                xg.push_back((uint32_t)base0 | ((uint32_t)base2 << 16));
-                xg.push_back((uint32_t)(k[0] & 255) | ((uint32_t)(k[1] & 255) << 8) | ((uint32_t)(k[2] & 255) << 16) | ((uint32_t)(k[3] & 255) << 24));
-                for (int i = 0; i < 4; ++i) {
-                    const short2 a = xa[L.xtab_off + std::min(c + i, L.w - 1)];
-                    xg_ok = xg_ok && a.x >= 0 && a.y >= 0;
-                    xg.push_back((uint32_t)(unsigned short)a.x | ((uint32_t)(unsigned short)a.y << 16));
-                }
-                xg.push_back(0);
-                xg.push_back(0);
-            }
-            for (int dy = 0; dy < L.h; ++dy) {
-                const short2 o = yofs[L.ytab_off + dy], c = yb[L.ytab_off + dy];
-                xg_ok = xg_ok && c.x >= 0 && c.y >= 0;
-                yrow.push_back(make_short4(o.x, o.y, c.x, c.y));
-            }
+            pyr_level_tables(C.levels[l - 1], L, T);
         }
         L.btile_first = btile_first;
         L.btiles_x = (L.w + BLUR_TW - 1) / BLUR_TW;
@@ -314,90 +564,25 @@
     C.pyr_frame_bytes = pyr_off ? pyr_off : 256;
     C.blur_frame_bytes = blur_off;
 
-    auto make_bands = [&](int bands, std::vector<int2>& band_rows) -> size_t {
-        band_rows.assign((size_t)bands * num_levels, int2{0, 0});
-        size_t worst = 0;
-        for (int k = 0; k < bands; ++k) {
-            int need_lo = 0, need_hi = 0;
-            for (int l = num_levels - 1; l >= 1; --l) {
-                const OrbLevel& Lv = C.levels[l];
-                int lo = (int)((long long)k * Lv.h / bands), hi = (int)((long long)(k + 1) * Lv.h / bands);
-                if (l < num_levels - 1 && need_hi > need_lo) {
-                    lo = std::min(lo, need_lo);
-                    hi = std::max(hi, need_hi);
-                }
-                band_rows[(size_t)k * num_levels + l] = int2{lo, hi};
-                need_lo = 1 << 30;
-                need_hi = 0;
-                for (int dy = lo; dy < hi; ++dy) {
-                    const short2 o = yofs[Lv.ytab_off + dy];
-                    need_lo = std::min(need_lo, (int)o.x);
-                    need_hi = std::max(need_hi, (int)o.y + 1);
-                }
-            }
-            if (need_hi > need_lo) band_rows[(size_t)k * num_levels] = int2{need_lo, need_hi};
-            size_t size_a = 0, size_b = 0;
-            for (int l = 0; l < num_levels; ++l) {
-                const int2 r = band_rows[(size_t)k * num_levels + l];
-                const size_t b = (size_t)(r.y - r.x) * (size_t)((C.levels[l].w + 3) & ~3);
-                if (l & 1) size_a = std::max(size_a, b);
-                else size_b = std::max(size_b, b);
-            }
-            size_a = (size_a + 15) & ~(size_t)15;
-            size_b = (size_b + 15) & ~(size_t)15;
-            size_t bytes = size_a + size_b;
-            for (int l = 1; l < num_levels; ++l) {
-                const int2 r = band_rows[(size_t)k * num_levels + l];
-                bytes += (size_t)(r.y - r.x) * 8;
-            }
-            worst = std::max(worst, bytes);
-        }
-        return worst;
-    };
-    std::vector<int2> band_rows;
-    int bands = std::max(8, std::min(32, (512 + max_batch - 1) / std::max(max_batch, 1)));
-    bool forced = false;
-    if (const char* e = getenv("SVGPU_PYR_BANDS")) {
-        bands = std::max(1, atoi(e));
-        forced = true;
-    }
-    xg_ok = xg_ok && (num_levels < 2 || C.levels[1].w <= 4 * 1024);
-    size_t lds = 0;
-    if (!forced && xg_ok) {
-        std::vector<int2> trial;
-        for (int k = bands; k <= 32; k += 2)
-            if (make_bands(k, trial) <= SV_PYR_LDS_HALF) {
-                bands = k;
-                break;
-            }
-    }
-    for (;; bands += 2) {
-        lds = make_bands(bands, band_rows);
-        if (lds <= SV_PYR_LDS_MAX && xg_ok) break;
-        if (bands >= 256 || !xg_ok) {
-            bands = 16;
-            make_bands(bands, band_rows);
-            lds = 0;
-            break;
-        }
-    }
-    ctx->pyr_bands = bands;
-    ctx->pyr_lds_bytes = lds;
-    if (lds) SV_HIP(ctx, sv_pyramid_prepare());
+    const PyrBands PB = plan_pyramid(C.levels, num_levels, max_batch, T);
+    ctx->pyr_bands = PB.bands;
+    ctx->pyr_lds_bytes = PB.lds;
+    if (PB.lds) SV_HIP(ctx, sv_pyramid_prepare());
     {
         int rcb;
-        if ((rcb = upload(ctx, &ctx->d_band_rows, band_rows))) return rcb;
+        if ((rcb = upload(ctx, &ctx->d_band_rows, PB.rows))) return rcb;
+        if ((rcb = upload(ctx, &ctx->d_pyr_plan, PB.plan))) return rcb;
     }
     std::vector<OrbLevel> lv(C.levels, C.levels + num_levels);
     int rc;
     if ((rc = upload(ctx, &ctx->d_levels, lv))) return rc;
     if ((rc = upload(ctx, &ctx->d_cells, C.cells))) return rc;
-    if ((rc = upload(ctx, &ctx->d_xofs, xofs))) return rc;
-    if ((rc = upload(ctx, &ctx->d_xa, xa))) return rc;
-    if ((rc = upload(ctx, &ctx->d_yofs, yofs))) return rc;
-    if ((rc = upload(ctx, &ctx->d_yb, yb))) return rc;
-    if ((rc = upload(ctx, &ctx->d_xg, xg))) return rc;
-    if ((rc = upload(ctx, &ctx->d_yrow, yrow))) return rc;
+    if ((rc = upload(ctx, &ctx->d_xofs, T.xofs))) return rc;
+    if ((rc = upload(ctx, &ctx->d_xa, T.xa))) return rc;
+    if ((rc = upload(ctx, &ctx->d_yofs, T.yofs))) return rc;
+    if ((rc = upload(ctx, &ctx->d_yb, T.yb))) return rc;
+    if ((rc = upload(ctx, &ctx->d_xg, T.xg))) return rc;
+    if ((rc = upload(ctx, &ctx->d_yrow, T.yrow))) return rc;
     if ((rc = upload(ctx, &ctx->d_gtab, gtab))) return rc;
     if (!C.dbands.empty()) {
         if ((rc = upload(ctx, &ctx->d_dbands, C.dbands))) return rc;
@@ -453,7 +638,7 @@
     const int Lc = C.num_levels;
     if (Lc > 1) {
         SvProfScope ps(ctx, s, "k_resize");
-        sv_launch_pyramid(s, ctx->d_levels, Lc, ctx->d_band_rows, ctx->pyr_bands, imgs_dev, frame_stride, row_stride, ctx->d_pyr,
+        sv_launch_pyramid(s, ctx->d_levels, Lc, ctx->d_band_rows, ctx->d_pyr_plan, ctx->pyr_bands, imgs_dev, frame_stride, row_stride, ctx->d_pyr,
                           C.pyr_frame_bytes, ctx->d_xofs, ctx->d_xa, ctx->d_yofs, ctx->d_yb, ctx->d_xg, ctx->d_yrow, batch, ctx->pyr_lds_bytes);
     }
     static const bool fork_blur = getenv("SVGPU_FORK_BLUR") != nullptr;
```

Result: no change. 279,500 (median of 6 runs) (+0.6%).
